# matthieugomez/LeastSquaresOptim.jl

Measured on AMD Instinct MI355X. Metric: lm_lsmr_outer_iterations_per_sec, higher is better.
Workload: dtype f64

## Files before the change

include/lsqhip.h:

```cpp
#ifndef LSQHIP_H
#define LSQHIP_H
#include <stddef.h>
#ifdef __cplusplus
extern "C" {
#endif

typedef enum {
    LSQ_OK = 0,
    LSQ_EDIM = 1,
    LSQ_ENOTPD = 2,
    LSQ_ERANK = 3,
    LSQ_ENONFINITE = 4,
    LSQ_EBOUNDS = 5,
    LSQ_EHIP = 6,
    LSQ_EARG = 7,
    LSQ_ECALLBACK = 8,
    LSQ_ERCCL = 9
} lsq_status;

typedef struct lsq_ctx lsq_ctx;
typedef struct lsq_mat lsq_mat;
typedef struct lsq_solver lsq_solver;
typedef struct lsq_model lsq_model;

// ... 16 lines not shown
int lsq_host_free(lsq_ctx *ctx, void *h_ptr);

int lsq_dense_create(lsq_ctx *ctx, int m, int n, lsq_mat **out);
int lsq_csc_create(lsq_ctx *ctx, int m, int n, const int *h_colptr, const int *h_rowval, lsq_mat **out);
int lsq_blockdiag_create(lsq_ctx *ctx, int nblocks, int mb, int nb, lsq_mat **out);
int lsq_mat_blockdiag_info(const lsq_mat *J, int *nblocks, int *mb, int *nb);
int lsq_blockdiag_bordered_create(lsq_ctx *ctx, int nblocks, int mb, int nb, int ng, lsq_mat **out);
int lsq_mat_bordered_info(const lsq_mat *J, int *nblocks, int *mb, int *nb, int *ng);
int lsq_mat_destroy(lsq_mat *J);
int lsq_mat_size(const lsq_mat *J, int *m, int *n, long long *nnz);
int lsq_mat_set_values(lsq_mat *J, const double *h_values);
int lsq_mat_get_values(const lsq_mat *J, double *h_values);
int lsq_mat_set_values_async(lsq_mat *J, const double *h_pinned_values);
int lsq_mat_upload_wait(lsq_mat *J);
double *lsq_mat_values(lsq_mat *J);
int lsq_mat_refresh(lsq_mat *J);

int lsq_mat_set_colscale(lsq_mat *J, const double *d_s);
int lsq_mat_colscale_changed(lsq_mat *J);

typedef int (*lsq_op_mul_callback)(int trans, const double *d_x, double *d_out, void *user);
typedef int (*lsq_op_colsum_callback)(double *d_out, void *user);
int lsq_op_create(lsq_ctx *ctx, int m, int n, lsq_op_mul_callback mul, lsq_op_colsum_callback colsumabs2,
                  void *user, lsq_mat **out);

int lsq_mul(lsq_mat *J, int trans, double alpha, const double *d_x, double beta, double *d_y);
int lsq_colsumabs2(lsq_mat *J, double *d_out);
int lsq_rowsumabs2(lsq_mat *J, double *d_out);

int lsq_axpy(lsq_ctx *ctx, int n, double a, const double *d_x, double *d_y);
int lsq_scal(lsq_ctx *ctx, int n, double a, double *d_x);
int lsq_copy(lsq_ctx *ctx, int n, const double *d_x, double *d_y);
int lsq_fill(lsq_ctx *ctx, int n, double a, double *d_x);
int lsq_sumsq(lsq_ctx *ctx, int n, const double *d_x, double *h_out);
int lsq_sum(lsq_ctx *ctx, int n, const double *d_x, double *h_out);
int lsq_dot(lsq_ctx *ctx, int n, const double *d_x, const double *d_y, double *h_out);
int lsq_emul(lsq_ctx *ctx, int n, const double *d_x, const double *d_y, double *d_out);
int lsq_nrm2(lsq_ctx *ctx, int n, const double *d_x, double *h_out);
int lsq_wdot(lsq_ctx *ctx, int n, const double *d_x, const double *d_y, const double *d_w,
             double *h_out);
int lsq_amax(lsq_ctx *ctx, int n, const double *d_x, double *h_out);
int lsq_amax_projected(lsq_ctx *ctx, int n, const double *d_g, const double *d_x,
                       const double *d_lower, const double *d_upper, double *h_out);
int lsq_clamp(lsq_ctx *ctx, int n, double lo, double hi, double *d_x);
int lsq_ediv(lsq_ctx *ctx, int n, const double *d_x, const double *d_y, double *d_out);
int lsq_box_clip(lsq_ctx *ctx, int n, double *d_dx, const double *d_x, const double *d_lower,
                 const double *d_upper);
int lsq_first_nonfinite(lsq_ctx *ctx, int n, const double *d_x, int *h_index);

int lsq_solver_create(lsq_ctx *ctx, lsq_mat *J, int solver_kind, int for_lm, lsq_solver **out);
int lsq_solver_destroy(lsq_solver *s);
int lsq_ldiv(lsq_solver *s, lsq_mat *J, const double *d_y, double *d_x, int *nmul);
int lsq_ldiv_damped(lsq_solver *s, lsq_mat *J, const double *d_y, double *d_damp, double *d_x,
                    int *nmul);
typedef int (*lsq_precond_callback)(double *d_P, lsq_mat *J, const double *d_damp, void *user);
int lsq_solver_set_preconditioner(lsq_solver *s, lsq_precond_callback cb, void *user);
typedef int (*lsq_precond_update_callback)(lsq_mat *J, const double *d_damp, void *user);
typedef int (*lsq_precond_ldiv_callback)(double *d_out, const double *d_in, void *user);
int lsq_solver_set_general_preconditioner(lsq_solver *s, lsq_precond_update_callback update, lsq_precond_ldiv_callback ldiv,
                                          void *user);
typedef int (*lsq_device_allreduce_callback)(double *d_buf, int count, void *hip_stream, void *user);

int lsq_solver_set_row_allreduce(lsq_solver *s, lsq_device_allreduce_callback cb, void *user, long long global_rows);
int lsq_solver_info(const lsq_solver *s, int *lsmr_iter, int *lsmr_istop, int *qr_rank);
int lsq_solver_qr_path(const lsq_solver *s, int *path);
int lsq_solver_qr_panel(const lsq_solver *s, int *kind);
int lsq_solver_chol_path(const lsq_solver *s, int *path);
int lsq_solver_lsmr_path(const lsq_solver *s, int *path);
int lsq_solver_blockdiag_path(const lsq_solver *s, int *path, int *block);
int lsq_solver_blockdiag_ranks(const lsq_solver *s, int *h_ranks);
int lsq_solver_covariance(lsq_solver *s, lsq_mat *J, const double *d_f, double *d_cov, double *d_stderr, int *h_info);
int lsq_dense_covariance(lsq_solver *s, lsq_mat *J, const double *d_f, double *d_cov, double *d_stderr, int *h_info);
int lsq_dense_qr_covariance(lsq_solver *s, lsq_mat *J, const double *d_f, double *d_cov, double *d_stderr, int *h_info);

int lsq_solver_stats(const lsq_solver *s, int h_giveups[4], int h_paused[4]);
int lsq_ctx_fallback_stats(const lsq_ctx *ctx, int h_giveups[4]);
int lsq_ctx_device_info(const lsq_ctx *ctx, int *num_cus, int *num_xcds, char *arch_name, int name_cap);

int lsq_ctx_tail_stats(const lsq_ctx *ctx, long long h_out[2]);
int lsq_ctx_commit_step_stats(const lsq_ctx *ctx, long long h_out[2]);

typedef int (*lsq_f_callback)(double *d_out, const double *d_x, void *user);
typedef int (*lsq_g_callback)(lsq_mat *J, const double *d_x, void *user);
typedef int (*lsq_allreduce_callback)(double *h_vals, int count, void *user);

typedef struct {
    double x_tol, f_tol, g_tol;
    int iterations;
    double delta;
    const double *h_lower;
    const double *h_upper;
    lsq_allreduce_callback allreduce;
    void *allreduce_user;
    int trace_cap;
    double *trace_ssr, *trace_gnorm, *trace_delta, *trace_rho;
    int *trace_inner, *trace_accept;
    double *trace_x;
    lsq_precond_callback preconditioner;
    void *preconditioner_user;
    lsq_device_allreduce_callback row_allreduce;
    void *row_allreduce_user;
    long long global_rows;
    lsq_precond_update_callback precond_update;
    lsq_precond_ldiv_callback precond_ldiv;
    void *precond_general_user;
} lsq_options;

typedef struct {
    int optimizer;
    double ssr;
    int iterations;
    int converged, x_converged, f_converged, g_converged;
    int f_calls, g_calls, mul_calls;
    int status;
    int bad_index;
    double seconds;
    long long lsmr_iterations;
    double ssr0;
} lsq_result;

void lsq_options_default(lsq_options *opt);
int lsq_optimize(lsq_ctx *ctx, int optimizer, int solver_kind, lsq_mat *J, double *d_x,
                 double *d_fcur, lsq_f_callback f, lsq_g_callback g, void *user,
                 const lsq_options *opt, lsq_result *res);
int lsq_fd_jacobian(lsq_ctx *ctx, lsq_mat *J, const double *d_x, lsq_f_callback f, void *user);

int lsq_csc_greedy_colouring(int m, int n, const int *h_colptr, const int *h_rowval, int *h_colour, int *h_ncolours);
int lsq_mat_set_fd_colouring(lsq_mat *J, const int *h_colour_or_null, int *h_ncolours);
int lsq_mat_fd_colouring(const lsq_mat *J, int *h_colour, int *h_ncolours);

typedef struct {
    double *ssr, *ssr0;
    int *iterations;
    int *converged, *x_converged, *f_converged, *g_converged;
    int *f_calls, *g_calls, *mul_calls;
    int *status, *info;
    int outer_iterations;
    double seconds;
    int trace_cap;
    double *trace_ssr, *trace_gnorm, *trace_delta, *trace_rho;
    int *trace_accept;
    double *trace_x;
} lsq_batched_result;
int lsq_optimize_batched(lsq_ctx *ctx, int optimizer, int solver_kind, lsq_mat *J, double *d_x,
                         double *d_fcur, lsq_f_callback f, lsq_g_callback g, void *user,
                         const lsq_options *opt, void *batched_result);

int lsq_model_tanh_create(lsq_ctx *ctx, lsq_mat *J, const double *h_Avalues, const double *h_b,
                          lsq_model **out);
int lsq_model_destroy(lsq_model *md);
lsq_f_callback lsq_model_f(void);
lsq_g_callback lsq_model_g(void);
int lsq_model_paths(const lsq_model *md, int *sliced_rows, int *sliced_cols, int *lsmr_path, long long *pair_tails);

int lsq_synth_sparse(int m, int n, int per_col, unsigned long long seed, int *h_colptr,
                     int *h_rowval, double *h_nzval);
int lsq_synth_dense(int m, int n, unsigned long long seed, double *h_values);
int lsq_synth_uniform(int n, unsigned long long seed, double lo, double hi, double *h_out);
int lsq_synth_normal(int n, unsigned long long seed, double *h_out);

int lsq_bench_mul(lsq_mat *J, int trans, int reps, const double *d_x, double *d_y, double beta,
                  float *h_ms_per_launch);

int lsq_bench_occupy(lsq_ctx *ctx, int workgroups, int lds_bytes, double milliseconds);
int lsq_bench_occupy_wait(lsq_ctx *ctx);

int lsq_set_exact(int on);

int lsq_debug_set(int launch_jitter_us, int serial);
int lsq_debug_get(int *launch_jitter_us, int *serial, long long *stalls);

int lsq_prof_begin(lsq_ctx *ctx, int max_samples);
int lsq_prof_select(lsq_ctx *ctx, int kernel_mask);
int lsq_prof_end(lsq_ctx *ctx, double h_avg_ms[2], int h_count[2]);
int lsq_prof_overhead(lsq_ctx *ctx, int pairs, double *h_ms);

#ifdef __cplusplus
}
#endif
#endif
```

leastsquaresoptim.jl_amd/_lib.py:

```python
import ctypes as C
import os
import re
import subprocess

_HERE = os.path.dirname(os.path.abspath(__file__))
ROOT = os.path.dirname(_HERE)
LIB_PATH = os.environ.get("LSQ_LIB_PATH") or os.path.join(_HERE, "liblsqhip.so")
HEADER = os.path.join(ROOT, "include", "lsqhip.h")

c_dp = C.POINTER(C.c_double)
c_ip = C.POINTER(C.c_int)

F_CALLBACK = C.CFUNCTYPE(C.c_int, C.c_void_p, C.c_void_p, C.c_void_p)
G_CALLBACK = C.CFUNCTYPE(C.c_int, C.c_void_p, C.c_void_p, C.c_void_p)
ALLREDUCE_CALLBACK = C.CFUNCTYPE(C.c_int, c_dp, C.c_int, C.c_void_p)
OP_MUL_CALLBACK = C.CFUNCTYPE(C.c_int, C.c_int, C.c_void_p, C.c_void_p, C.c_void_p)
OP_COLSUM_CALLBACK = C.CFUNCTYPE(C.c_int, C.c_void_p, C.c_void_p)
PRECOND_CALLBACK = C.CFUNCTYPE(C.c_int, C.c_void_p, C.c_void_p, C.c_void_p, C.c_void_p)
ROW_ALLREDUCE_CALLBACK = C.CFUNCTYPE(C.c_int, C.c_void_p, C.c_int, C.c_void_p, C.c_void_p)
PRECOND_UPDATE_CALLBACK = C.CFUNCTYPE(C.c_int, C.c_void_p, C.c_void_p, C.c_void_p)
PRECOND_LDIV_CALLBACK = C.CFUNCTYPE(C.c_int, C.c_void_p, C.c_void_p, C.c_void_p)

OK, EDIM, ENOTPD, ERANK, ENONFINITE, EBOUNDS, EHIP, EARG, ECALLBACK, ERCCL = range(10)
QR, CHOLESKY, LSMR, BLOCK_QR = 0, 1, 2, 3
DOGLEG, LEVENBERG_MARQUARDT = 0, 1


class Options(C.Structure):
    _fields_ = [("x_tol", C.c_double), ("f_tol", C.c_double), ("g_tol", C.c_double),
                ("iterations", C.c_int), ("delta", C.c_double), ("h_lower", c_dp), ("h_upper", c_dp),
                ("allreduce", ALLREDUCE_CALLBACK), ("allreduce_user", C.c_void_p),
                ("trace_cap", C.c_int), ("trace_ssr", c_dp), ("trace_gnorm", c_dp),
                ("trace_delta", c_dp), ("trace_rho", c_dp), ("trace_inner", c_ip),
                ("trace_accept", c_ip), ("trace_x", c_dp),
                ("preconditioner", PRECOND_CALLBACK), ("preconditioner_user", C.c_void_p),
                ("row_allreduce", ROW_ALLREDUCE_CALLBACK), ("row_allreduce_user", C.c_void_p),
                ("global_rows", C.c_longlong),
                ("precond_update", PRECOND_UPDATE_CALLBACK), ("precond_ldiv", PRECOND_LDIV_CALLBACK),
                ("precond_general_user", C.c_void_p)]


class Result(C.Structure):
    _fields_ = [("optimizer", C.c_int), ("ssr", C.c_double), ("iterations", C.c_int),
                ("converged", C.c_int), ("x_converged", C.c_int), ("f_converged", C.c_int),
                ("g_converged", C.c_int), ("f_calls", C.c_int), ("g_calls", C.c_int),
                ("mul_calls", C.c_int), ("status", C.c_int), ("bad_index", C.c_int),
                ("seconds", C.c_double), ("lsmr_iterations", C.c_longlong), ("ssr0", C.c_double)]


class BatchedResult(C.Structure):
    _fields_ = [("ssr", c_dp), ("ssr0", c_dp), ("iterations", c_ip),
                ("converged", c_ip), ("x_converged", c_ip), ("f_converged", c_ip), ("g_converged", c_ip),
                ("f_calls", c_ip), ("g_calls", c_ip), ("mul_calls", c_ip), ("status", c_ip), ("info", c_ip),
                ("outer_iterations", C.c_int), ("seconds", C.c_double), ("trace_cap", C.c_int),
                ("trace_ssr", c_dp), ("trace_gnorm", c_dp), ("trace_delta", c_dp), ("trace_rho", c_dp),
                ("trace_accept", c_ip), ("trace_x", c_dp)]


def build(verbose=False):
    cmd = ["make", "-C", os.path.join(_HERE, "csrc"), "-j8"]
    if not verbose:
        cmd.insert(1, "-s")
    subprocess.check_call(cmd)
    return LIB_PATH


def declared_symbols():
    txt = open(HEADER).read()
    txt = re.sub(r"/\*.*?\*/", "", txt, flags=re.S)
    names = re.findall(r"\b(lsq_[a-z0-9_]+)\s*\(", txt)
    skip = {"lsq_f_callback", "lsq_g_callback", "lsq_allreduce_callback", "lsq_device_allreduce_callback",
            "lsq_precond_update_callback", "lsq_precond_ldiv_callback"}
    return sorted(set(n for n in names if n not in skip))


_LIB = None


def lib():
    global _LIB
    if _LIB is not None:
        return _LIB
    if not os.path.exists(LIB_PATH):
        raise RuntimeError(
            "liblsqhip.so is not built (%s). Run __graft_entry__.build() or `make -C "
            "leastsquaresoptim.jl_amd/csrc`. There is no CPU fallback." % LIB_PATH)
    L = C.CDLL(LIB_PATH)
    vp, i, d, sz = C.c_void_p, C.c_int, C.c_double, C.c_size_t
    pvp = C.POINTER(C.c_void_p)
    sig = {
        "lsq_last_error": (C.c_char_p, []),
        "lsq_version": (i, []),
        "lsq_ctx_create": (i, [i, vp, pvp]),
        "lsq_ctx_destroy": (i, [vp]),
        "lsq_ctx_sync": (i, [vp]),
        "lsq_ctx_stream": (vp, [vp]),
        "lsq_malloc": (i, [vp, sz, pvp]),
        "lsq_free": (i, [vp, vp]),
        "lsq_h2d": (i, [vp, vp, vp, sz]),
        "lsq_d2h": (i, [vp, vp, vp, sz]),
        "lsq_d2d": (i, [vp, vp, vp, sz]),
        "lsq_dense_create": (i, [vp, i, i, pvp]),
        "lsq_csc_create": (i, [vp, i, i, c_ip, c_ip, pvp]),
        "lsq_blockdiag_create": (i, [vp, i, i, i, pvp]),
        "lsq_mat_blockdiag_info": (i, [vp, c_ip, c_ip, c_ip]),
        "lsq_blockdiag_bordered_create": (i, [vp, i, i, i, i, pvp]),
        "lsq_mat_bordered_info": (i, [vp, c_ip, c_ip, c_ip, c_ip]),
        "lsq_mat_destroy": (i, [vp]),
        "lsq_mat_size": (i, [vp, c_ip, c_ip, C.POINTER(C.c_longlong)]),
        "lsq_mat_set_values": (i, [vp, c_dp]),
        "lsq_mat_get_values": (i, [vp, c_dp]),
        "lsq_mat_set_values_async": (i, [vp, c_dp]),
        "lsq_mat_upload_wait": (i, [vp]),
        "lsq_host_alloc": (i, [vp, sz, pvp]),
        "lsq_host_free": (i, [vp, vp]),
        "lsq_dot": (i, [vp, i, vp, vp, c_dp]),
        "lsq_emul": (i, [vp, i, vp, vp, vp]),
        "lsq_mat_values": (vp, [vp]),
        "lsq_mat_refresh": (i, [vp]),
        "lsq_mat_set_colscale": (i, [vp, vp]),
        "lsq_mat_colscale_changed": (i, [vp]),
        "lsq_mul": (i, [vp, i, d, vp, d, vp]),
        "lsq_solver_set_preconditioner": (i, [vp, PRECOND_CALLBACK, vp]),
        "lsq_solver_set_general_preconditioner": (i, [vp, PRECOND_UPDATE_CALLBACK, PRECOND_LDIV_CALLBACK, vp]),
        "lsq_op_create": (i, [vp, i, i, OP_MUL_CALLBACK, OP_COLSUM_CALLBACK, vp, C.POINTER(vp)]),
        "lsq_colsumabs2": (i, [vp, vp]),
        "lsq_rowsumabs2": (i, [vp, vp]),
        "lsq_axpy": (i, [vp, i, d, vp, vp]),
        "lsq_scal": (i, [vp, i, d, vp]),
        "lsq_copy": (i, [vp, i, vp, vp]),
        "lsq_fill": (i, [vp, i, d, vp]),
        "lsq_sumsq": (i, [vp, i, vp, c_dp]),
        "lsq_sum": (i, [vp, i, vp, c_dp]),
        "lsq_nrm2": (i, [vp, i, vp, c_dp]),
        "lsq_wdot": (i, [vp, i, vp, vp, vp, c_dp]),
        "lsq_amax": (i, [vp, i, vp, c_dp]),
        "lsq_amax_projected": (i, [vp, i, vp, vp, vp, vp, c_dp]),
        "lsq_clamp": (i, [vp, i, d, d, vp]),
        "lsq_ediv": (i, [vp, i, vp, vp, vp]),
        "lsq_box_clip": (i, [vp, i, vp, vp, vp, vp]),
        "lsq_first_nonfinite": (i, [vp, i, vp, c_ip]),
        "lsq_solver_create": (i, [vp, vp, i, i, pvp]),
        "lsq_solver_destroy": (i, [vp]),
        "lsq_ldiv": (i, [vp, vp, vp, vp, c_ip]),
        "lsq_ldiv_damped": (i, [vp, vp, vp, vp, vp, c_ip]),
        "lsq_solver_set_row_allreduce": (i, [vp, ROW_ALLREDUCE_CALLBACK, vp, C.c_longlong]),
        "lsq_solver_info": (i, [vp, c_ip, c_ip, c_ip]),
        "lsq_solver_qr_path": (i, [vp, c_ip]),
        "lsq_solver_qr_panel": (i, [vp, c_ip]),
        "lsq_solver_chol_path": (i, [vp, c_ip]),
        "lsq_solver_lsmr_path": (i, [vp, c_ip]),
        "lsq_solver_blockdiag_path": (i, [vp, c_ip, c_ip]),
        "lsq_solver_blockdiag_ranks": (i, [vp, c_ip]),
        "lsq_solver_covariance": (i, [vp, vp, vp, vp, vp, c_ip]),
        "lsq_dense_covariance": (i, [vp, vp, vp, vp, vp, c_ip]),
        "lsq_dense_qr_covariance": (i, [vp, vp, vp, vp, vp, c_ip]),
        "lsq_solver_stats": (i, [vp, c_ip, c_ip]),
        "lsq_ctx_fallback_stats": (i, [vp, c_ip]),
        "lsq_ctx_device_info": (i, [vp, c_ip, c_ip, C.c_char_p, i]),
        "lsq_ctx_tail_stats": (i, [vp, C.POINTER(C.c_longlong)]),
        "lsq_ctx_commit_step_stats": (i, [vp, C.POINTER(C.c_longlong)]),
        "lsq_bench_occupy": (i, [vp, i, i, d]),
        "lsq_bench_occupy_wait": (i, [vp]),
        "lsq_options_default": (None, [C.POINTER(Options)]),
        "lsq_optimize": (i, [vp, i, i, vp, vp, vp, F_CALLBACK, G_CALLBACK, vp, C.POINTER(Options),
                             C.POINTER(Result)]),
        "lsq_optimize_batched": (i, [vp, i, i, vp, vp, vp, F_CALLBACK, G_CALLBACK, vp, C.POINTER(Options),
                                     C.POINTER(BatchedResult)]),
        "lsq_fd_jacobian": (i, [vp, vp, vp, F_CALLBACK, vp]),
        "lsq_csc_greedy_colouring": (i, [i, i, c_ip, c_ip, c_ip, c_ip]),
        "lsq_mat_set_fd_colouring": (i, [vp, c_ip, c_ip]),
        "lsq_mat_fd_colouring": (i, [vp, c_ip, c_ip]),
        "lsq_model_tanh_create": (i, [vp, vp, c_dp, c_dp, pvp]),
        "lsq_model_destroy": (i, [vp]),
        "lsq_model_f": (F_CALLBACK, []),
        "lsq_model_g": (G_CALLBACK, []),
        "lsq_model_paths": (i, [vp, c_ip, c_ip, c_ip, C.POINTER(C.c_longlong)]),
        "lsq_synth_sparse": (i, [i, i, i, C.c_ulonglong, c_ip, c_ip, c_dp]),
        "lsq_synth_dense": (i, [i, i, C.c_ulonglong, c_dp]),
        "lsq_synth_uniform": (i, [i, C.c_ulonglong, d, d, c_dp]),
        "lsq_synth_normal": (i, [i, C.c_ulonglong, c_dp]),
        "lsq_set_exact": (i, [i]),
        "lsq_debug_set": (i, [i, i]),
        "lsq_debug_get": (i, [c_ip, c_ip, C.POINTER(C.c_longlong)]),
        "lsq_prof_begin": (i, [vp, i]),
        "lsq_prof_select": (i, [vp, i]),
        "lsq_prof_end": (i, [vp, c_dp, c_ip]),
        "lsq_prof_overhead": (i, [vp, i, c_dp]),
        "lsq_bench_mul": (i, [vp, i, i, vp, vp, d, C.POINTER(C.c_float)]),
    }
    for name, (res, args) in sig.items():
        fn = getattr(L, name)
        fn.restype = res
        fn.argtypes = args
    L._signatures = sig
    _LIB = L
    return L


class LsqError(RuntimeError):

    def __init__(self, status, msg):
        super().__init__(msg)
        self.status = status


class DimensionMismatch(LsqError):
    pass


class PosDefException(LsqError):
    pass


class RankDeficientException(LsqError):
    pass


class IsFiniteException(LsqError):
    pass


class ArgumentError(LsqError):
    pass


class HipError(LsqError):
    pass


class PeerAborted(LsqError):
    """Sharded run: another rank left its loop with an error (LSQ_ERCCL)."""


_EXC = {EDIM: DimensionMismatch, ENOTPD: PosDefException, ERANK: RankDeficientException,
        ENONFINITE: IsFiniteException, EBOUNDS: ArgumentError, EHIP: HipError, EARG: ArgumentError,
        ECALLBACK: LsqError, ERCCL: PeerAborted}


def check(status):
    if status != OK:
        msg = lib().lsq_last_error().decode("utf-8", "replace")
        raise _EXC.get(status, LsqError)(status, msg or "lsq status %d" % status)
```

leastsquaresoptim.jl_amd/csrc/lsq_common.h:

```cpp
#pragma once
#include <hip/hip_runtime.h>
#include <atomic>

#include <cstdarg>
#include <cstdint>
#include <cstdio>
#include <unordered_map>
#include <vector>

#include "../../include/lsqhip.h"

void lsq_set_error(const char *fmt, ...);

#define LSQ_HIP(call)                                                                      \
    do {                                                                                   \
        hipError_t e__ = (call);                                                           \
        if (e__ != hipSuccess) {                                                           \
            lsq_set_error("%s failed: %s (%s:%d)", #call, hipGetErrorString(e__), __FILE__, \
                          __LINE__);                                                       \
            return LSQ_EHIP;                                                               \
        }                                                                                  \
    } while (0)

#define LSQ_TRY(call)                 \
// ... 169 lines not shown
    bool csc_fresh = true;
    bool upload_pending = false;
    const double *d_colscale = nullptr;
    const double *d_cs_user = nullptr;
    double *d_cs_base = nullptr;
    double *d_colsum_base = nullptr;
    unsigned long long base_version = 0;
    unsigned long long colsum_base_version = ~0ull;
    LsqSegs bcsc;
    int nwin = 0;
    int *d_bmap = nullptr;
    double *d_bpart = nullptr;
    double *d_dpart = nullptr;
    size_t dpart_cap = 0;
    LsqSell srows, scols;
    int (*op_mul)(int, const double *, double *, void *) = nullptr;
    int (*op_colsum)(double *, void *) = nullptr;
    void *op_user = nullptr;
    double *d_optmp = nullptr;
    unsigned long long version = 0;
    unsigned long long uid = lsq_next_mat_uid();
    double *d_colsum = nullptr;
    unsigned long long colsum_version = ~0ull;
    int bd_blocks = 0, bd_mb = 0, bd_nb = 0;
    int br_blocks = 0, br_mb = 0, br_nb = 0, br_ng = 0;
    double *d_fd = nullptr;
    struct LsqFdColouring *fdc = nullptr;
};

struct LsqFdColouring {
    int ncolours = 0;
    std::vector<int> colour;
    std::vector<int> bound;
    std::vector<int> ebound;
    int *d_colour = nullptr;
    int *d_cols = nullptr;
    int *d_off = nullptr;
};
void lsq_fd_colouring_free(lsq_mat *J);

#define LSQ_ZERO(ptr, val, bytes)                  \
    do {                                           \
        LSQ_HIP(hipMemset((ptr), (val), (bytes))); \
        LSQ_HIP(hipStreamSynchronize(nullptr));    \
    } while (0)

#define RLX_AGENT __ATOMIC_RELAXED, __HIP_MEMORY_SCOPE_AGENT

template <int CTRL>
__device__ __forceinline__ double lsq_dpp_mov_f64(double x) {
    int lo = __double2loint(x), hi = __double2hiint(x);
    lo = __builtin_amdgcn_update_dpp(0, lo, CTRL, 0xf, 0xf, false);
    hi = __builtin_amdgcn_update_dpp(0, hi, CTRL, 0xf, 0xf, false);
    return __hiloint2double(hi, lo);
}
__device__ __forceinline__ double lsq_readlane_f64(double x, int l) {
    return __hiloint2double(__builtin_amdgcn_readlane(__double2hiint(x), l), __builtin_amdgcn_readlane(__double2loint(x), l));
}
__device__ __forceinline__ double wave_sum(double v) {
    v += lsq_dpp_mov_f64<0x128>(v);
    v += lsq_dpp_mov_f64<0x124>(v);
    v += lsq_dpp_mov_f64<0x122>(v);
    v += lsq_dpp_mov_f64<0x121>(v);
    return (lsq_readlane_f64(v, 0) + lsq_readlane_f64(v, 16)) + (lsq_readlane_f64(v, 32) + lsq_readlane_f64(v, 48));
}
__device__ __forceinline__ double wave_max(double v) {
    v = fmax(v, lsq_dpp_mov_f64<0x128>(v));
    v = fmax(v, lsq_dpp_mov_f64<0x124>(v));
    v = fmax(v, lsq_dpp_mov_f64<0x122>(v));
    v = fmax(v, lsq_dpp_mov_f64<0x121>(v));
    return fmax(fmax(lsq_readlane_f64(v, 0), lsq_readlane_f64(v, 16)), fmax(lsq_readlane_f64(v, 32), lsq_readlane_f64(v, 48)));
}

__device__ __forceinline__ int lsq_xcd_block(int b, int G) {
    const int q = G >> 3, r = G & 7, x = b & 7;
    return x * q + (x < r ? x : r) + (b >> 3);
}

template <int NT>
__device__ __forceinline__ double block_sum(double v, double *sh ) {
    v = wave_sum(v);
    const int lane = threadIdx.x & 63, w = threadIdx.x >> 6;
    if (lane == 0) sh[w] = v;
    __syncthreads();
    double r = 0.0;
    if (threadIdx.x == 0) {
#pragma unroll
        for (int i = 0; i < NT / 64; ++i) r += sh[i];
    }
    __syncthreads();
    return r;
}
template <int NT>
__device__ __forceinline__ double block_max(double v, double *sh) {
    v = wave_max(v);
    const int lane = threadIdx.x & 63, w = threadIdx.x >> 6;
    if (lane == 0) sh[w] = v;
    __syncthreads();
    double r = 0.0;
    if (threadIdx.x == 0) {
        r = sh[0];
#pragma unroll
        for (int i = 1; i < NT / 64; ++i) r = fmax(r, sh[i]);
    }
    __syncthreads();
    return r;
}

constexpr int LSQ_RGROUPS = 8;
constexpr int LSQ_RFLAT = 64;
constexpr int LSQ_CTR_STRIDE = 32;
constexpr int LSQ_CTR_SLOT = (LSQ_RGROUPS + 1) * LSQ_CTR_STRIDE;
template <int NT, bool IS_MAX = false, class Fin>
__device__ __forceinline__ bool grid_reduce(double block_val, double *partials, unsigned *counter,
                                            int nblocks, double *sh, Fin fin) {
    __shared__ int s_last;
    const int b = blockIdx.x;
    if (threadIdx.x == 0) {
        __hip_atomic_store(&partials[b], block_val, RLX_AGENT);
        asm volatile("s_waitcnt vmcnt(0)" ::: "memory");
        const int g = b % LSQ_RGROUPS;
        const int ngroups = nblocks < LSQ_RGROUPS ? nblocks : LSQ_RGROUPS;
        const unsigned gsize = (unsigned)((nblocks - g + LSQ_RGROUPS - 1) / LSQ_RGROUPS);
        int last = 0;
        if (nblocks <= LSQ_RFLAT) {
            if (__hip_atomic_fetch_add(counter, 1u, RLX_AGENT) == (unsigned)(nblocks - 1)) {
                __hip_atomic_store(counter, 0u, RLX_AGENT);
                last = 1;
            }
        } else if (__hip_atomic_fetch_add(counter + (1 + g) * LSQ_CTR_STRIDE, 1u, RLX_AGENT) == gsize - 1) {
            __hip_atomic_store(counter + (1 + g) * LSQ_CTR_STRIDE, 0u, RLX_AGENT);
            unsigned t2 = __hip_atomic_fetch_add(counter, 1u, RLX_AGENT);
            if (t2 == (unsigned)(ngroups - 1)) {
                __hip_atomic_store(counter, 0u, RLX_AGENT);
                last = 1;
            }
        }
        s_last = last;
    }
    __syncthreads();
    if (!s_last) return false;
    if (threadIdx.x == 0) __builtin_amdgcn_fence(__ATOMIC_ACQUIRE, "agent");
    __syncthreads();
    double acc = 0.0;
    for (int i = threadIdx.x; i < nblocks; i += NT) {
        double p = __hip_atomic_load(&partials[i], RLX_AGENT);
        acc = IS_MAX ? fmax(acc, p) : acc + p;
    }
    double tot = IS_MAX ? block_max<NT>(acc, sh) : block_sum<NT>(acc, sh);
    if (threadIdx.x == 0) fin(tot);
    return true;
}

struct LsqSlotPublish {
    const double *src = nullptr;
    int count = 0;
    double *dst = nullptr;
    unsigned long long *seq_word = nullptr;
    unsigned long long seq = 0;
};
LsqSlotPublish lsq_slots_ticket(lsq_ctx *c, int first, int count);
int lsq_wait_slots(lsq_ctx *c, int first, int count, unsigned long long seq, double *h_out);
int lsq_first_nonfinite_to_slot(lsq_ctx *c, int n, const double *x, double *d_slot);
int lsq_read_ints(lsq_ctx *c, const int *d_a, const int *d_b, const int *d_c, const int *d_d, int h_out[4]);
LsqSlotPublish lsq_ints_ticket(lsq_ctx *c);
int lsq_wait_ints(lsq_ctx *c, unsigned long long seq, const int *d_a, const int *d_b, const int *d_c, const int *d_d, int h_out[4]);

static inline void lsq_run_idle_hook(lsq_ctx *c) {
    if (!c->idle_hook) return;
    int (*h)(void *) = c->idle_hook;
    c->idle_hook = nullptr;
    c->idle_status = h(c->idle_user);
}

static inline unsigned *lsq_ctr(const lsq_ctx *c, int k) { return c->d_counters + (size_t)k * LSQ_CTR_SLOT; }
static inline int lsq_div_up(long long a, long long b) { return (int)((a + b - 1) / b); }

constexpr int LSQ_EXACT_MAX_DIM = 2048;
constexpr long long LSQ_EXACT_MAX_NNZ = 1 << 18;
bool lsq_small_vec(long long n);
bool lsq_small_mat(const lsq_mat *J);
int lsq_exact_product(lsq_mat *J, int trans, const double *x, double *y);
int lsq_exact_colsumabs2(lsq_mat *J, double *out);
int lsq_exact_mul(lsq_mat *J, int trans, double alpha, const double *x, double beta, double *y);
int lsq_seq_reduce(lsq_ctx *c, int mode, int n, const double *x, const double *y, const double *w, double *d_out);
int lsq_exact_lm_damp(lsq_ctx *c, int n, const double *colsum, double inv_delta, double *dtd);

void lsq_workspace_free(void *workspace);

int lsq_sparse_mul(lsq_mat *J, int trans, double alpha, const double *d_x, double beta, double *d_y);
int lsq_dense_mul(lsq_mat *J, int trans, double alpha, const double *d_x, double beta, double *d_y);
static inline int lsq_dense_t_windows(const lsq_ctx *c, int m, int n) {
    if (n <= 0 || n >= c->num_cus || m < 8192) return 0;
    int nwin = (4 * c->num_cus + n - 1) / n;
    nwin = std::min(nwin, std::max(1, m / 2048));
    return nwin > 1 ? nwin : 0;
}
int lsq_dense_colsumabs2(lsq_mat *J, double *d_out);
int lsq_dense_part(lsq_mat *J, int nwin);
int lsq_dense_part_elems(lsq_mat *J, size_t need);
int lsq_sparse_colsumabs2(lsq_mat *J, double *d_out);
int lsq_ensure_csr(lsq_mat *J);
int lsq_ensure_csc(lsq_mat *J);
int lsq_mirror_rows(lsq_mat *J, const double *d_csc_vals, double *d_out);
int lsq_mirror_cols(lsq_mat *J, const double *d_csc_vals, double *d_out);
long long lsq_mirror_rows_len(const lsq_mat *J);
long long lsq_mirror_cols_len(const lsq_mat *J);
bool lsq_can_fuse_grad_colsum(const lsq_mat *J);
bool lsq_colscale_fusable(const lsq_mat *J);
int lsq_sparse_grad_colsum(lsq_mat *J, const double *f, double *g);
int lsq_sparse_grad_colsum_spec(lsq_mat *J, const double *f, double *g, const double *s_new, const int *gate);
void lsq_sparse_grad_colsum_adopt(lsq_mat *J);
void lsq_sparse_colsum_forget(lsq_mat *J);
const double *lsq_cached_colsum(lsq_mat *J);
struct LsqFdCall {
    lsq_f_callback f;
    void *user;
    int status;
};
int lsq_fd_check(const lsq_mat *J, const char *who);
int lsq_fd_values(lsq_mat *J, const double *x, lsq_f_callback f, void *user);
int lsq_fd_f_thunk(double *d_out, const double *d_x, void *user);
int lsq_fd_g_thunk(lsq_mat *J, const double *d_x, void *user);
int lsq_read_slots(lsq_ctx *ctx, int first, int count, double *h_out);
```

leastsquaresoptim.jl_amd/csrc/lsq_loop.h:

```cpp
#pragma once
#include "lsq_solver.h"

static constexpr double MIN_DELTA = 1e-16, MAX_DELTA = 1e16, MIN_STEP_QUALITY = 1e-3;
static constexpr double MIN_DIAGONAL = 1e-6, MAX_DIAGONAL = 1e32;
static constexpr double DECREASE_THRESHOLD = 0.25, INCREASE_THRESHOLD = 0.75;

enum { SL_GRAD = 8, SL_DX = 9, SL_NONFIN = 10, SL_TRIAL = 11, SL_PRED = 12, SL_SSR = 13, SL_W0 = 14, SL_W1 = 15,
       SL_W2 = 16, SL_SUM = 17 };

static inline int ngrid(const lsq_ctx *c, long long n) {
    long long g = (n + LSQ_NT - 1) / LSQ_NT;
    long long cap = (long long)c->num_cus * 8;
    if (g > cap) g = cap;
    return g < 1 ? 1 : (int)g;
}

bool model_is_builtin(lsq_f_callback f, lsq_g_callback g = nullptr);

int model_f_sumsq(void *user, double *out, const double *x, int ctr, double *d_out, LsqSlotPublish pub, bool *done,
                  const int *skip = nullptr, bool mirror = false);
int model_start_point(void *user, const double *x, double *d_nonfin, bool *done);
void model_forget_point(void *user);
struct SpecGrad {
    int *gate;
    double ssr;
    double *grad;
    bool launched;
    double xtol, ftol, gtol;
};
int model_pair_tail(void *user, lsq_mat *J, const double *dx, const double *fcur, double *ftrial, const double *xt,
                    double *slot_pred, double *slot_trial, LsqSlotPublish pub, const int *skip, bool *done,
                    SpecGrad *sg = nullptr);
void model_trial_buffers(void *user, const double *xt, double **t_out, double **s_out);

int lsq_workspace_lsmr_path(const lsq_ctx *c, const lsq_mat *J);
```

leastsquaresoptim.jl_amd/csrc/lsq_lsmr3.h:

```cpp
#pragma once

constexpr int LSQ_FUSED_UB_MAX = 4;
struct LsmrHandoff {
    unsigned long long w[8];
};
__device__ __forceinline__ void lsmr_handoff_write(LsmrHandoff *ho, unsigned tag, double vs, double cu, int done) {
    const unsigned long long t = (unsigned long long)tag << 32;
    const unsigned long long bv = (unsigned long long)__double_as_longlong(vs), bc = (unsigned long long)__double_as_longlong(cu);
    __hip_atomic_store(&ho->w[0], t | (bv & 0xffffffffull), __ATOMIC_RELAXED, __HIP_MEMORY_SCOPE_AGENT);
    __hip_atomic_store(&ho->w[1], t | (bv >> 32), __ATOMIC_RELAXED, __HIP_MEMORY_SCOPE_AGENT);
    __hip_atomic_store(&ho->w[2], t | (bc & 0xffffffffull), __ATOMIC_RELAXED, __HIP_MEMORY_SCOPE_AGENT);
    __hip_atomic_store(&ho->w[3], t | (bc >> 32), __ATOMIC_RELAXED, __HIP_MEMORY_SCOPE_AGENT);
    __hip_atomic_store(&ho->w[4], t | (unsigned)done, __ATOMIC_RELAXED, __HIP_MEMORY_SCOPE_AGENT);
}
__device__ __forceinline__ void lsmr_handoff_fail(LsmrHandoff *ho, unsigned tag) {
    __hip_atomic_store(&ho->w[6], (unsigned long long)tag, __ATOMIC_RELAXED, __HIP_MEMORY_SCOPE_AGENT);
}
struct LsmrHandoffWords { unsigned long long w[5]; };
__device__ __forceinline__ LsmrHandoffWords lsmr_handoff_request(const LsmrHandoff *ho) {
    LsmrHandoffWords r;
#pragma unroll
    for (int k = 0; k < 5; ++k) r.w[k] = __hip_atomic_load(&ho->w[k], __ATOMIC_RELAXED, __HIP_MEMORY_SCOPE_AGENT);
    return r;
}
// ... 34 lines not shown
    const double test2 = s.normAr / (s.normA * s.normr);
    const double test3 = 1.0 / s.condA;
    const double t1 = test1 / (1.0 + s.normA * s.normx / s.normb);
    const double rtol = s.btol + s.atol * s.normA * s.normx / s.normb;
    int istop = 0;
    if (s.iter >= s.maxiter) istop = 7;
    else if (1.0 + test3 <= 1.0) istop = 6;
    else if (1.0 + test2 <= 1.0) istop = 5;
    else if (1.0 + t1 <= 1.0) istop = 4;
    else if (test3 <= s.ctol) istop = 3;
    else if (test2 <= s.atol) istop = 2;
    else if (test1 <= rtol) istop = 1;
    s.istop = istop;
    if (istop) { s.done = 1; s.notdone = 0; }
}

constexpr long long LSQ_FUSED_SPIN_LIMIT = 1LL << 24;

__device__ __forceinline__ void publish_relaxed(LsqMailbox *mail, const LsmrState *st) {
    unsigned long long w = ((unsigned long long)(st->epoch & 0x7fffffu) << 41) |
                           ((unsigned long long)(st->done ? 1 : 0) << 40) |
                           ((unsigned long long)(st->istop & 0xff) << 32) | (unsigned)st->iter;
    __hip_atomic_store((unsigned long long *)mail, w, __ATOMIC_RELAXED, __HIP_MEMORY_SCOPE_SYSTEM);
}

__device__ __forceinline__ void ordered_sum512x3(const double *pa, const int *na, const double *pb, const int *nb,
                                                 const double *pc, const int *nc, double &ra, double &rb, double &rc) {
    __shared__ double s_w5[3][4];
    __shared__ double s_tot5[3];
    const int tid = threadIdx.x;
    if (tid < 256) {
        const double a0 = pa ? pa[tid] : 0.0, b0 = pb ? pb[tid] : 0.0, c0 = pc ? pc[tid] : 0.0;
        const double a1 = pa ? pa[tid + 256] : 0.0, b1 = pb ? pb[tid + 256] : 0.0, c1 = pc ? pc[tid + 256] : 0.0;
        const int ca = pa ? *na : 0, cb = pb ? *nb : 0, cc = pc ? *nc : 0;
        double a = tid < ca ? a0 : 0.0, b = tid < cb ? b0 : 0.0, c = tid < cc ? c0 : 0.0;
        if (tid + 256 < ca) a += a1;
        if (tid + 256 < cb) b += b1;
        if (tid + 256 < cc) c += c1;
        for (int i = tid + 512; i < ca; i += 256) a += pa[i];
        for (int i = tid + 512; i < cb; i += 256) b += pb[i];
        for (int i = tid + 512; i < cc; i += 256) c += pc[i];
        a = wave_sum(a);
        b = wave_sum(b);
        c = wave_sum(c);
        if ((tid & 63) == 0) {
            s_w5[0][tid >> 6] = a;
            s_w5[1][tid >> 6] = b;
            s_w5[2][tid >> 6] = c;
        }
    }
    __syncthreads();
    if (tid < 3) s_tot5[tid] = ((s_w5[tid][0] + s_w5[tid][1]) + s_w5[tid][2]) + s_w5[tid][3];
    __syncthreads();
    ra = s_tot5[0];
    rb = s_tot5[1];
    rc = s_tot5[2];
    __syncthreads();
}

__device__ __forceinline__ void lsq_lds_barrier() { asm volatile("s_waitcnt lgkmcnt(0)\n\ts_barrier" ::: "memory"); }
template <bool IS_MAX>
__device__ __forceinline__ double lsq_block_reduce_lds(double v, double *sh ) {
    v = IS_MAX ? wave_max(v) : wave_sum(v);
    const int lane = threadIdx.x & 63, w = threadIdx.x >> 6;
    if (lane == 0) sh[w] = v;
    lsq_lds_barrier();
    double r = 0.0;
    if (threadIdx.x == 0) {
        r = sh[0];
#pragma unroll
        for (int i = 1; i < LSQ_BIG_NT / 64; ++i) r = IS_MAX ? fmax(r, sh[i]) : r + sh[i];
    }
    lsq_lds_barrier();
    return r;
}

template <bool STEP, int NU>
__device__ __forceinline__ void lsmr_update_groups(const LsmrFused &a, const LsmrStepDesc &sd, const int gstride, double *sh,
                                                   LsmrState &ns) {
    const int tid = threadIdx.x;
    const int n = a.n;
    static_assert(sizeof(LsmrState) % 8 == 0 && sizeof(LsmrState) / 8 <= LSQ_BIG_NT, "state copy: one 8-byte word per thread");
    constexpr int NQ = (LSQ_LDS_X_MAX + LSQ_BIG_NT - 1) / LSQ_BIG_NT;
    double xi[NQ], hbi[NQ], hi[NQ];
#pragma unroll
    for (int q = 0; q < NQ; ++q) {
        const int j = min(tid + q * LSQ_BIG_NT, n - 1);
        xi[q] = a.x_in[j];
        hbi[q] = a.hbar_in[j];
        hi[q] = a.h_in[j];
    }
    if (tid < (int)(sizeof(LsmrState) / 8)) ((unsigned long long *)&ns)[tid] = ((const unsigned long long *)a.st_in)[tid];
    const bool prev_failed = a.tag_prev != 0u &&
                             (unsigned)__hip_atomic_load(&a.ho->w[6], __ATOMIC_RELAXED, __HIP_MEMORY_SCOPE_AGENT) == a.tag_prev;
    double beta2, betax2, alpha2;
    ordered_sum512x3(a.pu_in, a.npu_in, a.px_in, a.npx_in, a.pv, a.npv, beta2, betax2, alpha2);
    if (ns.done) {
        if (blockIdx.x == 0) {
            if (tid < (int)(sizeof(LsmrState) / 8)) ((unsigned long long *)a.st_out)[tid] = ((const unsigned long long *)&ns)[tid];
            if (tid == 0) {
                lsmr_handoff_write(a.ho, a.tag, 1.0, 0.0, 1);
                publish_relaxed(a.mail, &ns);
            }
        }
        return;
    }
    const bool was_first = ns.first != 0;
    if (tid == 0) lsmr_scalars(ns, beta2, betax2, alpha2, a.dg != nullptr, a.px_in != nullptr);
    __syncthreads();
    if (!was_first) {
        const double c1 = ns.c1, c2 = ns.c2;
        double acc = 0.0;
#pragma unroll
        for (int q = 0; q < NQ; ++q) {
            const double hb = hbi[q] * c1 + hi[q];
            const double xj = xi[q] + c2 * hb;
            acc += (tid + q * LSQ_BIG_NT < n) ? xj * xj : 0.0;
        }
        const double total = block_sum<LSQ_BIG_NT>(acc, sh);
        if (tid == 0) lsmr_decide(ns, total);
    } else if (tid == 0) {
        ns.first = 0;
        if (!(ns.normAr != 0.0)) { ns.done = 1; ns.notdone = 0; }
    }
    if (tid == 0 && prev_failed) { ns.istop = 99; ns.done = 1; ns.notdone = 0; }
    __syncthreads();
    const bool done_now = ns.done != 0;
    const double vs = ns.vscale, cu = ns.cu, c1 = ns.c1, c2 = ns.c2, c3 = ns.c3;
    if constexpr (STEP) {
        if (!done_now) {
            if (blockIdx.x == 0 && tid == 0) {
                if (!was_first) {
                    __hip_atomic_store((double *)&a.mail->test1, ns.normr / ns.normb, __ATOMIC_RELAXED, __HIP_MEMORY_SCOPE_SYSTEM);
                    __hip_atomic_store((double *)&a.mail->test2, ns.normAr / (ns.normA * ns.normr), __ATOMIC_RELAXED, __HIP_MEMORY_SCOPE_SYSTEM);
                }
                publish_relaxed(a.mail, &ns);
            }
            return;
        }
    }
    if (blockIdx.x == 0) {
        if (tid == 0 && !a.test_no_record) lsmr_handoff_write(a.ho, a.tag, vs, cu, done_now ? 1 : 0);
        if (tid < (int)(sizeof(LsmrState) / 8)) ((unsigned long long *)a.st_out)[tid] = ((const unsigned long long *)&ns)[tid];
        if (tid == 0) {
            if (!was_first) {
                __hip_atomic_store((double *)&a.mail->test1, ns.normr / ns.normb, __ATOMIC_RELAXED, __HIP_MEMORY_SCOPE_SYSTEM);
                __hip_atomic_store((double *)&a.mail->test2, ns.normAr / (ns.normA * ns.normr), __ATOMIC_RELAXED, __HIP_MEMORY_SCOPE_SYSTEM);
            }
            publish_relaxed(a.mail, &ns);
        }
    }
    double e_vt[NU], e_P[NU], e_dg[NU], e_ux[NU], e_h[NU], e_hb[NU], e_x[NU];
    double e_s[NU];
#pragma unroll
    for (int k = 0; k < NU; ++k) {
        const int j = min((int)(blockIdx.x + k * gstride) * LSQ_BIG_NT + tid, n - 1);
        e_vt[k] = a.vt[j];
        e_P[k] = a.P ? a.P[j] : 1.0;
        e_dg[k] = a.dg ? a.dg[j] : 0.0;
        e_ux[k] = a.dg ? a.ux[j] : 0.0;
        e_h[k] = a.h_in[j];
        e_hb[k] = a.hbar_in[j];
        e_x[k] = a.x_in[j];
        if constexpr (STEP) e_s[k] = sd.x[j];
    }
    double aux = 0.0;
    double mx = 0.0, code = 0.0;
#pragma unroll
    for (int k = 0; k < NU; ++k) {
        const int j = (int)(blockIdx.x + k * gstride) * LSQ_BIG_NT + tid;
        if (j >= n) continue;
        const double Pj = e_P[k];
        const double vj = e_vt[k] * vs;
        a.v[j] = vj;
        double dj = 0.0;
        if (was_first) {
            a.h_out[j] = vj;
            a.hbar_out[j] = 0.0;
            a.x_out[j] = 0.0;
            a.xout[j] = 0.0;
        } else {
            const double hj = e_h[k];
            const double hb = e_hb[k] * c1 + hj;
            a.hbar_out[j] = hb;
            const double xj = e_x[k] + c2 * hb;
            a.x_out[j] = xj;
            a.h_out[j] = hj * c3 + vj;
            dj = a.P ? xj * Pj : xj;
            a.xout[j] = dj;
        }
        if constexpr (STEP) {
            const double v = e_s[k] + -1.0 * dj;
            sd.xt[j] = v;
            if (sd.t_out) {
                const double th = tanh(v);
                sd.t_out[j] = th;
                sd.s_out[j] = 1.0 - th * th;
            }
            double ad = fabs(dj);
            if (isnan(ad)) ad = INFINITY;
            mx = fmax(mx, ad);
            if (!isfinite(v) && code == 0.0) code = 1e15 - (double)(j + 1);
        }
        if (a.dg && !done_now) {
            const double tj = a.P ? vj * Pj : vj;
            const double un = tj * e_dg[k] - cu * e_ux[k];
            a.ux[j] = un;
            aux += un * un;
        }
    }
    if constexpr (STEP) {
        const double b2 = lsq_block_reduce_lds<true>(code, sh);
        if (tid == 0) __hip_atomic_store(&sd.partials[LSQ_MAX_GRID + blockIdx.x], b2, RLX_AGENT);
        const double b1 = lsq_block_reduce_lds<true>(mx, sh);
        const int nb = gridDim.x;
        double *const out_dx = sd.out_dx;
        if (grid_reduce<LSQ_BIG_NT, true>(b1, sd.partials, sd.counter, nb, sh, [=](double t) { *out_dx = t; })) {
            double acc = 0.0;
            for (int i = tid; i < nb; i += LSQ_BIG_NT) acc = fmax(acc, __hip_atomic_load(&sd.partials[LSQ_MAX_GRID + i], RLX_AGENT));
            const double t = block_max<LSQ_BIG_NT>(acc, sh);
            if (tid == 0) *sd.out_nonfin = (t == 0.0) ? -1.0 : (1e15 - t) - 1.0;
        }
        return;
    }
    if (done_now) return;
    const double bux = lsq_block_reduce_lds<false>(aux, sh);
    if (tid == 0) {
        a.px_out[blockIdx.x] = bux;
        if (blockIdx.x == 0) *a.npx_out = gstride;
    }
}

template <int = 0>
__global__ void __launch_bounds__(LSQ_BIG_NT) k_lsmr_fused(SellDev S, int wrows, int m, int nxpad, LsmrFused a) {
    extern __shared__ __attribute__((aligned(16))) double smem[];
    __shared__ double sh[LSQ_BIG_NT / 64];
    __shared__ LsmrState ns;
    __shared__ double s_vs, s_cu;
    __shared__ int s_done;
    double *xl = smem;
    double *yw = smem + nxpad;
    const int tid = threadIdx.x, lane = tid & 63, wv = tid >> 6;
    const int n = a.n;
    const bool upd = (int)blockIdx.x < a.ub;

    if (upd) {
        constexpr int NQ = (LSQ_LDS_X_MAX + LSQ_BIG_NT - 1) / LSQ_BIG_NT;
        lsmr_update_groups<false, (NQ + 2) / 3>(a, LsmrStepDesc{}, a.ub, sh, ns);
        return;
    }

    constexpr int XR = (LSQ_LDS_X_MAX + LSQ_BIG_NT - 1) / LSQ_BIG_NT;
    {
        double xr[XR];
#pragma unroll
        for (int q = 0; q < XR; ++q) xr[q] = a.w[min(tid + q * LSQ_BIG_NT, n - 1)];
        const int dflag = a.st_in->done;
#pragma unroll
        for (int q = 0; q < XR; ++q)
            if (tid + q * LSQ_BIG_NT < n) xl[tid + q * LSQ_BIG_NT] = xr[q];
        if (dflag) return;
    }
    constexpr int Q = LSQ_SELL_ROWS_MAX / LSQ_BIG_NT;
    const int pb = (int)blockIdx.x - a.ub, npb = (int)gridDim.x - a.ub;
    double racc = 0.0;
    bool have_scalars = false;
    if (a.cautious) {
        if (tid == 0) {
            LsmrHandoffWords rec = lsmr_handoff_request(a.ho);
            long long spins = 0;
            while (!lsmr_handoff_valid(rec, a.tag)) {
                if (++spins > (a.test_no_record ? 4096 : LSQ_FUSED_SPIN_LIMIT)) break;
                __builtin_amdgcn_s_sleep(8);
                rec = lsmr_handoff_request(a.ho);
            }
            const bool ok = spins <= (a.test_no_record ? 4096 : LSQ_FUSED_SPIN_LIMIT);
            s_vs = __longlong_as_double((long long)((rec.w[0] & 0xffffffffull) | (rec.w[1] << 32)));
            s_cu = __longlong_as_double((long long)((rec.w[2] & 0xffffffffull) | (rec.w[3] << 32)));
            s_done = ok ? (int)(rec.w[4] & 0xffffffffull) : 2;
            if (!ok) lsmr_handoff_fail(a.ho, a.tag);
        }
        __syncthreads();
        if (s_done) return;
        have_scalars = true;
    }
    for (int w = pb; w < S.nblocks; w += npb) {
        const int base = w * wrows, rows = min(wrows, m - base);
        const int s0 = w * S.spw, s1 = s0 + S.spw;
        double pre[Q];
#pragma unroll
        for (int q = 0; q < Q; ++q) pre[q] = a.uold[base + min(tid + q * LSQ_BIG_NT, rows - 1)];
        LsmrHandoffWords rec;
#pragma unroll
        for (int k = 0; k < 5; ++k) rec.w[k] = 0ull;
        {
            constexpr int NW = LSQ_BIG_NT / 64;
            int sidx = s0 + wv;
            SellSliceRef A = sell_slice_ref(S, sidx, s1, lane);
            __syncthreads();
            unsigned long long poll = 0ull;
            for (; sidx < s1; sidx += NW) {
                if (!have_scalars && (unsigned)(poll >> 32) == a.tag && (poll & 1ull)) break;
                if (!have_scalars) poll = __hip_atomic_load(&a.ho->w[4], __ATOMIC_RELAXED, __HIP_MEMORY_SCOPE_AGENT);
                const SellSliceRef r = A;
                A = sell_slice_ref(S, sidx + NW, s1, lane);
                if (!have_scalars && tid == 0 && sidx + NW >= s1) rec = lsmr_handoff_request(a.ho);
                const size_t oa = (size_t)r.sm.x + lane * 2;
                const unsigned pos = r.inf & LSQ_SELL_POS_MASK;
                double sum = 0.0, sq = 0.0;
                sell_lane_sum<false>(S.val + oa, S.idx16 + oa, r.sm.y, (int)(r.inf >> LSQ_SELL_POS_BITS), xl, sum, sq, lane);
                if (pos != LSQ_SELL_POS_MASK) yw[pos] = sum;
            }
        }
        if (!have_scalars && tid == 0) {
            long long spins = 0;
            while (!lsmr_handoff_valid(rec, a.tag)) {
                if (++spins > (a.test_no_record ? 4096 : LSQ_FUSED_SPIN_LIMIT)) break;
                __builtin_amdgcn_s_sleep(8);
                rec = lsmr_handoff_request(a.ho);
            }
            const bool ok = spins <= (a.test_no_record ? 4096 : LSQ_FUSED_SPIN_LIMIT);
            s_vs = __longlong_as_double((long long)((rec.w[0] & 0xffffffffull) | (rec.w[1] << 32)));
            s_cu = __longlong_as_double((long long)((rec.w[2] & 0xffffffffull) | (rec.w[3] << 32)));
            s_done = ok ? (int)(rec.w[4] & 0xffffffffull) : 2;
            if (!ok) lsmr_handoff_fail(a.ho, a.tag);
        }
        have_scalars = true;
        __syncthreads();
        if (s_done) return;
        const double vs = s_vs, cu = s_cu;
#pragma unroll
        for (int q = 0; q < Q; ++q) {
            const int i = tid + q * LSQ_BIG_NT;
            if (i < rows) {
                const double un = vs * yw[i] - cu * pre[q];
                a.unew[base + i] = un;
                racc += un * un;
            }
        }
    }
    const double bv = block_sum<LSQ_BIG_NT>(racc, sh);
    if (tid == 0) {
        a.pu_out[pb] = bv;
        if (pb == 0) *a.npu_out = npb;
    }
}

template <int = 0>
__global__ void __launch_bounds__(LSQ_BIG_NT) k_lsmr_commit_step(LsmrFused a, LsmrStepDesc sd) {
    __shared__ double sh[LSQ_BIG_NT / 64];
// ... 4 lines not shown
```

leastsquaresoptim.jl_amd/csrc/lsq_model.hip:

```cpp
#include <algorithm>

#include "lsq_loop.h"
#include "lsq_spmv.h"

struct lsq_model {
    lsq_ctx *ctx;
    lsq_mat *J;
    bool fused = false;
    double *d_Acsc = nullptr;
    double *d_Acsr = nullptr;
    double *d_Ab = nullptr;
    double *d_b = nullptr;
    double *d_t = nullptr;
    double *d_s = nullptr;
    double *d_sspec = nullptr;
    const double *tanh_x = nullptr;
    const double *sfac_x = nullptr;
    double *d_b_perm = nullptr;
    double *d_perm[2] = {nullptr, nullptr};
    const double *perm_of[2] = {nullptr, nullptr};
    long long pair_tails = 0;
};
static void model_perm_invalidate(lsq_model *md, const double *vec) {
    for (int k = 0; k < 2; ++k)
        if (!vec || md->perm_of[k] == vec) md->perm_of[k] = nullptr;
}

__global__ void __launch_bounds__(LSQ_NT) k_tanh(int n, const double *__restrict__ x, double *__restrict__ t) {
    for (int i = blockIdx.x * LSQ_NT + threadIdx.x; i < n; i += gridDim.x * LSQ_NT) t[i] = tanh(x[i]);
}

struct EpiResidual {
    static constexpr bool REDUCE = false;
    const int *done;
    int extra_blocks;
    const double *b;
    double *out;
    double *partials;
    unsigned *counter;
    __device__ void seg(int i, double dot, double &) const { out[i] = dot - b[i]; }
    using has_pre = void;
    __device__ double pre(int i) const { return b[i]; }
    __device__ void seg_pre(int i, double dot, double bi, double &) const { out[i] = dot - bi; }
    __device__ void extra(int, double &) const {}
    __device__ void finalize(double) const {}
};

struct EpiResidualSq {
    static constexpr bool REDUCE = true;
    const int *done;
    int extra_blocks;
    const double *b;
    double *out;
    double *partials;
    unsigned *counter;
    double *slot;
    LsqSlotPublish pub;
    __device__ void seg(int i, double dot, double &racc) const { seg_pre(i, dot, b[i], racc); }
    using has_pre = void;
    __device__ double pre(int i) const { return b[i]; }
    __device__ void seg_pre(int i, double dot, double bi, double &racc) const {
        const double v = dot - bi;
        out[i] = v;
        racc += v * v;
    }
    __device__ void extra(int, double &) const {}
    __device__ void finalize(double t) const {
        *slot = t;
        if (pub.count > 0) {
            for (int i = 0; i < pub.count; ++i)
                __hip_atomic_store(pub.dst + i, pub.src + i == slot ? t : pub.src[i], __ATOMIC_RELAXED, __HIP_MEMORY_SCOPE_SYSTEM);
            __hip_atomic_store(pub.seq_word, pub.seq, __ATOMIC_RELEASE, __HIP_MEMORY_SCOPE_SYSTEM);
        }
    }
};

struct EpiResidualSqPerm : EpiResidualSq {
    const double *b_perm;
    double *out_perm;
    using has_slice_out = void;
    __device__ double slice_pre(size_t pidx) const { return b_perm[pidx]; }
    __device__ void slice_post(size_t pidx, double dot, double bi) const { out_perm[pidx] = dot - bi; }
};

__global__ void __launch_bounds__(LSQ_NT)
k_scale_cols(int n, const int *__restrict__ colptr, int m_dense, const double *__restrict__ A,
             const double *__restrict__ x, double *__restrict__ out) {
    for (int j = blockIdx.x; j < n; j += gridDim.x) {
        double t = tanh(x[j]);
        double s = 1.0 - t * t;
        long long k0 = colptr ? colptr[j] : (long long)j * m_dense;
        long long k1 = colptr ? colptr[j + 1] : (long long)(j + 1) * m_dense;
        for (long long k = k0 + threadIdx.x; k < k1; k += LSQ_NT) out[k] = A[k] * s;
    }
}
__global__ void __launch_bounds__(LSQ_NT)
k_scale_dense(int m, const double *__restrict__ A, const double *__restrict__ x, double *__restrict__ out) {
    const int j = blockIdx.x;
    const double t = tanh(x[j]);
    const double sfac = 1.0 - t * t;
    const size_t base = (size_t)j * m;
    for (int i = blockIdx.y * LSQ_NT + threadIdx.x; i < m; i += gridDim.y * LSQ_NT) out[base + i] = A[base + i] * sfac;
}
__global__ void __launch_bounds__(LSQ_NT)
k_scale_csr(long long nnz, const int *__restrict__ colidx, const double *__restrict__ A, const double *__restrict__ sfac,
            double *__restrict__ out) {
    for (long long k = blockIdx.x * (long long)LSQ_NT + threadIdx.x; k < nnz; k += (long long)gridDim.x * LSQ_NT)
        out[k] = A[k] * sfac[colidx[k]];
}
__global__ void __launch_bounds__(LSQ_NT) k_tanh_sfac(int n, const double *__restrict__ x, double *__restrict__ t,
                                                      double *__restrict__ s, double *partials, unsigned *counter,
                                                      double *out_nonfin) {
    __shared__ double sh[LSQ_NT / 64];
    double code = 0.0;
    for (int i = blockIdx.x * LSQ_NT + threadIdx.x; i < n; i += gridDim.x * LSQ_NT) {
        const double xi = x[i];
        const double v = tanh(xi);
        t[i] = v;
        s[i] = 1.0 - v * v;
        if (!isfinite(xi) && code == 0.0) code = 1e15 - (double)(i + 1);
    }
    const double bv = block_max<LSQ_NT>(code, sh);
    grid_reduce<LSQ_NT, true>(bv, partials, counter, gridDim.x, sh, [=](double m) {
        *out_nonfin = (m == 0.0) ? -1.0 : (1e15 - m) - 1.0;
    });
}
__global__ void __launch_bounds__(LSQ_NT) k_sfac(int n, const double *__restrict__ x, double *__restrict__ s) {
    for (int i = blockIdx.x * LSQ_NT + threadIdx.x; i < n; i += gridDim.x * LSQ_NT) {
        double t = tanh(x[i]);
        s[i] = 1.0 - t * t;
    }
}

__global__ void __launch_bounds__(LSQ_NT)
k_scale_bcsc(int nseg, int n, const int *__restrict__ ptr, const double *__restrict__ A, const double *__restrict__ sfac,
             double *__restrict__ out) {
    const int lane = threadIdx.x & 63, per = LSQ_NT / 64;
    for (int s = blockIdx.x * per + (threadIdx.x >> 6); s < nseg; s += gridDim.x * per) {
        const double f = sfac[s % n];
        const int k1 = ptr[s + 1];
        for (int k = ptr[s] + lane; k < k1; k += 64) out[k] = A[k] * f;
    }
}

typedef double lsq_d2 __attribute__((ext_vector_type(2)));
template <bool NT>
__global__ void __launch_bounds__(1024)
k_scale_lds(long long nnz4, const unsigned short *__restrict__ col16, const double *__restrict__ A,
            const double *__restrict__ sfac, int n, double *__restrict__ out) {
    extern __shared__ double sf[];
    for (int i = threadIdx.x; i < n; i += 1024) sf[i] = sfac[i];
    __syncthreads();
    for (long long q = blockIdx.x * 1024LL + threadIdx.x; q < nnz4; q += (long long)gridDim.x * 1024) {
        const long long k = 4 * q;
        const lsq_d2 a0 = *reinterpret_cast<const lsq_d2 *>(A + k);
        const lsq_d2 a1 = *reinterpret_cast<const lsq_d2 *>(A + k + 2);
        const uint2 c = *reinterpret_cast<const uint2 *>(col16 + k);
        lsq_d2 o0, o1;
        o0.x = a0.x * sf[c.x & 0xffffu];
        o0.y = a0.y * sf[c.x >> 16];
        o1.x = a1.x * sf[c.y & 0xffffu];
        o1.y = a1.y * sf[c.y >> 16];
        if constexpr (NT) {
            __builtin_nontemporal_store(o0, reinterpret_cast<lsq_d2 *>(out + k));
            __builtin_nontemporal_store(o1, reinterpret_cast<lsq_d2 *>(out + k + 2));
        } else {
            *reinterpret_cast<lsq_d2 *>(out + k) = o0;
            *reinterpret_cast<lsq_d2 *>(out + k + 2) = o1;
        }
    }
}

__global__ void __launch_bounds__(LSQ_NT)
k_scale_bcsc_thread(int nseg, int n, const int *__restrict__ ptr, const double *__restrict__ A,
                    const double *__restrict__ sfac, double *__restrict__ out) {
    for (int s = blockIdx.x * LSQ_NT + threadIdx.x; s < nseg; s += gridDim.x * LSQ_NT) {
        const double f = sfac[s % n];
        const int k1 = ptr[s + 1];
        for (int k = ptr[s]; k < k1; ++k) out[k] = A[k] * f;
    }
}

static int model_f(double *out, const double *x, void *user) {
    lsq_model *md = (lsq_model *)user;
    lsq_ctx *c = md->ctx;
    lsq_mat *J = md->J;
    const bool have_tanh = md->tanh_x == x;
    md->tanh_x = nullptr;
    model_perm_invalidate(md, out);
    if (!have_tanh) {
        md->sfac_x = nullptr;
        LSQ_LAUNCH(k_tanh, dim3(ngrid(c, J->n)), dim3(LSQ_NT), 0, c->stream, J->n, x, md->d_t);
    }
    EpiResidual e{nullptr, 0, md->d_b, out, nullptr, nullptr};
    if (J->kind == LSQ_MAT_CSC && J->srows.active) {
        if (launch_sell_rows(J, nullptr, md->d_t, e, md->fused ? nullptr : md->d_Acsr) != LSQ_OK) return 1;
    } else if (J->kind == LSQ_MAT_CSC) {
        LsqSegs A = J->csr;
        A.d_val = md->d_Acsr;
        if (launch_segs<false>(c, A, md->d_t, e) != LSQ_OK) return 1;
    } else {
        lsq_mat tmp = *J;
        tmp.d_dense = md->d_Acsc;
        if (launch_product(&tmp, 0, md->d_t, e) != LSQ_OK) return 1;
    }
    return hipGetLastError() == hipSuccess ? 0 : 1;
}

void model_trial_buffers(void *user, const double *xt, double **t_out, double **s_out) {
    lsq_model *md = (lsq_model *)user;
    md->tanh_x = md->sfac_x = nullptr;
    if ((md->J->kind == LSQ_MAT_CSC && md->J->srows.active) || md->J->kind == LSQ_MAT_DENSE) {
        *t_out = md->d_t;
        *s_out = md->d_sspec;
        md->tanh_x = md->sfac_x = xt;
    }
}

int model_start_point(void *user, const double *x, double *d_nonfin, bool *done) {
    lsq_model *md = (lsq_model *)user;
    lsq_ctx *c = md->ctx;
    lsq_mat *J = md->J;
    *done = false;
    md->tanh_x = md->sfac_x = nullptr;
    if (!(J->kind == LSQ_MAT_CSC && J->srows.active) || J->n <= 0) return 0;
    LSQ_LAUNCH(k_tanh_sfac, dim3(ngrid(c, J->n)), dim3(LSQ_NT), 0, c->stream, J->n, x, md->d_t, md->d_sspec, c->d_partials,
               lsq_ctr(c, 0), d_nonfin);
    if (hipGetLastError() != hipSuccess) return 1;
    md->tanh_x = md->sfac_x = x;
    *done = true;
    return 0;
}
void model_forget_point(void *user) {
    lsq_model *md = (lsq_model *)user;
    md->tanh_x = md->sfac_x = nullptr;
}

static bool model_pair_applies(const lsq_model *md, const lsq_mat *J) {
    return md->fused && J == md->J && J->kind == LSQ_MAT_CSC && J->srows.active && J->srows.ncw == 1 && J->d_colscale &&
           J->n <= LSQ_PAIR_X_MAX && !getenv("LSQ_NO_PAIR_TAIL");
}
static bool model_perm_ready(lsq_model *md) {
    if (md->d_b_perm) return true;
    lsq_ctx *c = md->ctx;
    const LsqSell &S = md->J->srows;
    const size_t plen = (size_t)S.nslices * 64;
    const int pgrid = std::max(1, std::min(lsq_div_up((long long)plen, LSQ_NT), c->num_cus * 8));
    double *pb = nullptr, *p0 = nullptr, *p1 = nullptr;
    if (hipMalloc(&pb, plen * sizeof(double)) != hipSuccess || hipMalloc(&p0, plen * sizeof(double)) != hipSuccess ||
        hipMalloc(&p1, plen * sizeof(double)) != hipSuccess) {
        (void)hipGetLastError();
        hipFree(pb); hipFree(p0); hipFree(p1);
        return false;
    }
    md->d_b_perm = pb; md->d_perm[0] = p0; md->d_perm[1] = p1;
    LSQ_LAUNCH(k_sell_perm_rows<0>, dim3(pgrid), dim3(LSQ_NT), 0, c->stream, sell_dev(S), S.wrows, S.nslices, (const double *)md->d_b,
               md->d_b_perm);
    return true;
}

int model_f_sumsq(void *user, double *out, const double *x, int ctr, double *d_out, LsqSlotPublish pub, bool *done,
                         const int *skip, bool mirror) {
    lsq_model *md = (lsq_model *)user;
    lsq_ctx *c = md->ctx;
    lsq_mat *J = md->J;
    *done = false;
    if (!(J->kind == LSQ_MAT_CSC && J->srows.active)) return model_f(out, x, user);
    model_perm_invalidate(md, out);
    EpiResidualSq e{skip, 0, md->d_b, out, c->d_partials, lsq_ctr(c, ctr), d_out, pub};
    const bool have_tanh = md->tanh_x == x;
    md->tanh_x = nullptr;
    if (!have_tanh) {
        md->sfac_x = nullptr;
        LSQ_LAUNCH(k_tanh, dim3(ngrid(c, J->n)), dim3(LSQ_NT), 0, c->stream, J->n, x, md->d_t);
    }
    if (mirror && !skip && model_pair_applies(md, J) && model_perm_ready(md)) {
        EpiResidualSqPerm ep;
        static_cast<EpiResidualSq &>(ep) = e;
        ep.b_perm = md->d_b_perm;
        ep.out_perm = md->d_perm[0];
        if (launch_sell_rows(J, nullptr, md->d_t, ep, nullptr) != LSQ_OK) return 1;
        md->perm_of[0] = out;
    } else if (launch_sell_rows(J, nullptr, md->d_t, e, md->fused ? nullptr : md->d_Acsr) != LSQ_OK) return 1;
    *done = true;
    return hipGetLastError() == hipSuccess ? 0 : 1;
}

int model_pair_tail(void *user, lsq_mat *J, const double *dx, const double *fcur, double *ftrial, const double *xt,
                           double *slot_pred, double *slot_trial, LsqSlotPublish pub, const int *skip, bool *done, SpecGrad *sg) {
    lsq_model *md = (lsq_model *)user;
    lsq_ctx *c = md->ctx;
    *done = false;
    if (!(model_pair_applies(md, J) && md->tanh_x == xt)) return 0;
    const LsqSell &S = J->srows;
    const int nxpad = (J->n + 1) & ~1;
    const size_t lds = (size_t)std::max(2 * nxpad, LSQ_SELL_ROWS_MAX) * sizeof(double);
    if (lsq_set_lds(c, (const void *)k_sell_rows_pair<0>, (size_t)2 * LSQ_PAIR_X_MAX * sizeof(double)) != LSQ_OK) return 0;
    const size_t plen = (size_t)S.nslices * 64;
    const int pgrid = std::max(1, std::min(lsq_div_up((long long)plen, LSQ_NT), c->num_cus * 8));
    if (!model_perm_ready(md)) return 0;
    int k = md->perm_of[0] == fcur ? 0 : (md->perm_of[1] == fcur ? 1 : -1);
    if (k < 0) {
        k = 0;
        LSQ_LAUNCH(k_sell_perm_rows<0>, dim3(pgrid), dim3(LSQ_NT), 0, c->stream, sell_dev(S), S.wrows, S.nslices, fcur, md->d_perm[k]);
        md->perm_of[k] = fcur;
    }
    md->perm_of[1 - k] = ftrial;
    md->tanh_x = nullptr;
    const int grid = std::max(1, std::min(S.nblocks, c->num_cus));
    const bool spec = sg && sg->gate && md->sfac_x == xt;
    SellPairEpi e{skip, md->d_perm[k], md->d_b_perm, ftrial, md->d_perm[1 - k], c->d_partials, c->d_partials + 4096, lsq_ctr(c, 7),
                  slot_pred, slot_trial, pub, spec ? sg->gate : nullptr, spec ? sg->ssr : 0.0, MIN_STEP_QUALITY,
                  c->d_slots + SL_SSR, c->d_slots + SL_DX, c->d_slots + SL_GRAD, spec ? sg->xtol : 0.0, spec ? sg->ftol : 0.0,
                  spec ? sg->gtol : 0.0};
    LSQ_LAUNCH(k_sell_rows_pair<0>, dim3(grid), dim3(LSQ_BIG_NT), lds, c->stream, sell_dev(S), S.wrows, J->m, dx, J->d_colscale,
               (const double *)md->d_t, J->n, nxpad, e);
    *done = true;
    ++md->pair_tails;
    if (hipGetLastError() != hipSuccess) return 1;
    if (spec) {
        const int st = lsq_sparse_grad_colsum_spec(J, ftrial, sg->grad, md->d_sspec, sg->gate);
        if (st == LSQ_OK) sg->launched = true;
        else if (st != LSQ_EARG) return 1;
    }
    return 0;
}

static int model_g(lsq_mat *J, const double *x, void *user) {
    lsq_model *md = (lsq_model *)user;
    lsq_ctx *c = md->ctx;
    if (J->kind == LSQ_MAT_DENSE) {}
    else if (md->sfac_x == x) std::swap(md->d_s, md->d_sspec);
    else LSQ_LAUNCH(k_sfac, dim3(ngrid(c, J->n)), dim3(LSQ_NT), 0, c->stream, J->n, x, md->d_s);
    md->sfac_x = nullptr;
    md->tanh_x = nullptr;
    if (md->fused) {
        if (lsq_mat_set_colscale(J, md->d_s) != LSQ_OK) return 1;
        return hipGetLastError() == hipSuccess ? 0 : 1;
    }
    if (J->kind == LSQ_MAT_CSC) {
        const bool have_cols = J->scols.active || J->nwin > 1;
        const unsigned short *rcol = J->srows.active ? J->srows.d_idx16 : J->csr.d_idx16;
        const unsigned short *ccol = J->scols.active ? J->scols.d_col16 : J->bcsc.d_col16;
        double *rval = J->srows.active ? J->srows.d_val : J->csr.d_val;
        double *cval = J->scols.active ? J->scols.d_val : J->bcsc.d_val;
        const long long rlen = lsq_mirror_rows_len(J), clen = lsq_mirror_cols_len(J);
        const bool lds_ok = J->n <= 12000 && J->nnz >= (1 << 20) && J->srows.ncw == 1;
        const bool lazy_csc = lds_ok && rcol && have_cols && ccol && lsq_can_fuse_grad_colsum(J);
        if (!lazy_csc) {
            int grid = J->n < c->num_cus * 16 ? (J->n > 0 ? J->n : 1) : c->num_cus * 16;
            LSQ_LAUNCH(k_scale_cols, dim3(grid), dim3(LSQ_NT), 0, c->stream, J->n, J->csc.d_ptr, 0, md->d_Acsc,
                               x, J->csc.d_val);
        }
        J->csc_fresh = !lazy_csc;
        const size_t lds = (size_t)J->n * sizeof(double);
        if (lds_ok) {
            LSQ_TRY(lsq_set_lds(c, (const void *)k_scale_lds<true>, 12000 * 8));
            LSQ_TRY(lsq_set_lds(c, (const void *)k_scale_lds<false>, 12000 * 8));
        }
        if (J->nnz > 0) {
            if (lds_ok && rcol) {
                LSQ_LAUNCH(k_scale_lds<true>, dim3(c->num_cus), dim3(1024), lds, c->stream, (rlen + 3) / 4, rcol,
                                   md->d_Acsr, md->d_s, J->n, rval);
            } else if (!J->srows.active) {
                long long g2 = std::min<long long>((J->nnz + LSQ_NT - 1) / LSQ_NT, (long long)c->num_cus * 16);
                LSQ_LAUNCH(k_scale_csr, dim3((int)g2), dim3(LSQ_NT), 0, c->stream, J->nnz, J->csr.d_idx,
                                   md->d_Acsr, md->d_s, J->csr.d_val);
            } else {
                if (lazy_csc) return 1;
                if (lsq_mirror_rows(J, J->csc.d_val, rval) != LSQ_OK) return 1;
            }
        }
        if (have_cols) {
            if (lds_ok && ccol) {
                LSQ_LAUNCH(k_scale_lds<false>, dim3(c->num_cus), dim3(1024), lds, c->stream, (clen + 3) / 4,
                                   ccol, md->d_Ab, md->d_s, J->n, cval);
            } else if (J->scols.active) {
                if (lazy_csc) return 1;
                if (lsq_mirror_cols(J, J->csc.d_val, cval) != LSQ_OK) return 1;
            } else if (J->nnz < 16LL * J->bcsc.nseg) {
                int nsegs = J->bcsc.nseg;
                int g3 = std::min(lsq_div_up(nsegs, LSQ_NT), c->num_cus * 16);
                LSQ_LAUNCH(k_scale_bcsc_thread, dim3(g3), dim3(LSQ_NT), 0, c->stream, nsegs, J->n,
                                   J->bcsc.d_ptr, md->d_Ab, md->d_s, J->bcsc.d_val);
            } else {
                int nsegs = J->bcsc.nseg;
                int g3 = std::min(lsq_div_up(nsegs, LSQ_NT / 64), c->num_cus * 16);
                LSQ_LAUNCH(k_scale_bcsc, dim3(g3), dim3(LSQ_NT), 0, c->stream, nsegs, J->n, J->bcsc.d_ptr,
                                   md->d_Ab, md->d_s, J->bcsc.d_val);
            }
        }
        J->csr_fresh = true;
    } else {
        const long long tot = (long long)J->m * J->n;
        const int chunks = std::max(1, (int)std::min<long long>((J->m + 4 * LSQ_NT - 1) / (4 * LSQ_NT),
                                                               std::max<long long>(1, (long long)c->num_cus * 16 / std::max(1, J->n))));
        if (tot > 0)
            LSQ_LAUNCH(k_scale_dense, dim3(J->n, chunks), dim3(LSQ_NT), 0, c->stream, J->m, md->d_Acsc, x, J->d_dense);
    }
    J->version++;
    return hipGetLastError() == hipSuccess ? 0 : 1;
}

bool model_is_builtin(lsq_f_callback f, lsq_g_callback g) { return f == model_f && (!g || g == model_g); }

extern "C" lsq_f_callback lsq_model_f(void) { return model_f; }
extern "C" lsq_g_callback lsq_model_g(void) { return model_g; }

extern "C" int lsq_model_tanh_create(lsq_ctx *c, lsq_mat *J, const double *hA, const double *hb, lsq_model **out) {
    if (!c || !J || !hA || !hb || !out) return LSQ_EARG;
    LSQ_HIP(hipSetDevice(c->device));
    lsq_model *md = new lsq_model();
    md->ctx = c;
    md->J = J;
    const size_t nb = (size_t)(J->n > 0 ? J->n : 1) * sizeof(double);
    LSQ_HIP(hipMalloc(&md->d_b, (size_t)(J->m > 0 ? J->m : 1) * sizeof(double)));
    LSQ_HIP(hipMemcpy(md->d_b, hb, (size_t)J->m * sizeof(double), hipMemcpyHostToDevice));
    LSQ_HIP(hipMalloc(&md->d_t, nb));
    LSQ_HIP(hipMalloc(&md->d_s, nb));
    LSQ_HIP(hipMalloc(&md->d_sspec, nb));
    if (lsq_colscale_fusable(J)) {
        LSQ_TRY(lsq_mat_set_values(J, hA));
        LSQ_TRY(lsq_fill(c, J->n, 1.0, md->d_s));
        LSQ_TRY(lsq_mat_set_colscale(J, md->d_s));
        md->fused = true;
        LSQ_HIP(hipStreamSynchronize(c->stream));
        *out = md;
        return LSQ_OK;
    }
    size_t vb = (size_t)(J->nnz + 8) * sizeof(double);
    LSQ_HIP(hipMalloc(&md->d_Acsc, vb));
    LSQ_ZERO(md->d_Acsc, 0, vb);
    LSQ_HIP(hipMemcpy(md->d_Acsc, hA, (size_t)J->nnz * sizeof(double), hipMemcpyHostToDevice));
    if (J->kind == LSQ_MAT_CSC) {
        const size_t rb = (size_t)(lsq_mirror_rows_len(J) + 1024) * sizeof(double);
        LSQ_HIP(hipMalloc(&md->d_Acsr, rb));
        LSQ_ZERO(md->d_Acsr, 0, rb);
        LSQ_TRY(lsq_mirror_rows(J, md->d_Acsc, md->d_Acsr));
        if (lsq_mirror_cols_len(J) > 0) {
            const size_t cbytes = (size_t)(lsq_mirror_cols_len(J) + 1024) * sizeof(double);
            LSQ_HIP(hipMalloc(&md->d_Ab, cbytes));
            LSQ_ZERO(md->d_Ab, 0, cbytes);
            LSQ_TRY(lsq_mirror_cols(J, md->d_Acsc, md->d_Ab));
        }
        LSQ_HIP(hipStreamSynchronize(c->stream));
    }
    *out = md;
    return LSQ_OK;
}

extern "C" int lsq_model_paths(const lsq_model *md, int *sliced_rows, int *sliced_cols, int *lsmr_path, long long *pair_tails) {
    if (!md || !sliced_rows || !sliced_cols || !lsmr_path || !pair_tails) {
        lsq_set_error("lsq_model_paths: null argument");
        return LSQ_EARG;
    }
    const lsq_mat *J = md->J;
    *sliced_rows = J->kind == LSQ_MAT_CSC && J->srows.active;
    *sliced_cols = J->kind == LSQ_MAT_CSC && J->scols.active;
    *lsmr_path = lsq_workspace_lsmr_path(md->ctx, J);
    *pair_tails = md->pair_tails;
    return LSQ_OK;
}

extern "C" int lsq_model_destroy(lsq_model *md) {
    if (!md) return LSQ_OK;
    hipStreamSynchronize(md->ctx->stream);
    if (md->fused && md->J) lsq_mat_set_colscale(md->J, nullptr);
    hipFree(md->d_Acsc); hipFree(md->d_Acsr); hipFree(md->d_Ab); hipFree(md->d_b); hipFree(md->d_t); hipFree(md->d_s); hipFree(md->d_sspec);
    hipFree(md->d_b_perm); hipFree(md->d_perm[0]); hipFree(md->d_perm[1]);
    delete md;
    return LSQ_OK;
}
```

leastsquaresoptim.jl_amd/csrc/lsq_optimize.hip:

```cpp
#include <chrono>
#include <cmath>
#include <cstring>

#include "lsq_loop.h"
#include "lsq_spmv.h"

__global__ void __launch_bounds__(1024)
k_lm_damp(int n, const double *__restrict__ colsum, double inv_delta, double *__restrict__ dtd) {
    __shared__ double sh[16];
    __shared__ double s_mean;
    double acc = 0.0;
    for (int i = threadIdx.x; i < n; i += 1024) acc += colsum[i];
    acc = wave_sum(acc);
    if ((threadIdx.x & 63) == 0) sh[threadIdx.x >> 6] = acc;
    __syncthreads();
    if (threadIdx.x == 0) {
        double t = 0.0;
        for (int w = 0; w < 16; ++w) t += sh[w];
        s_mean = t / n;
    }
    __syncthreads();
    const double lo = MIN_DIAGONAL * s_mean, hi = MAX_DIAGONAL * s_mean;
    for (int i = threadIdx.x; i < n; i += 1024) {
        double v = colsum[i];
        v = v > hi ? hi : (v < lo ? lo : v);
        dtd[i] = v * inv_delta;
    }
}

constexpr int LSQ_ONE_WG_N = 16384;

__global__ void __launch_bounds__(1024)
k_lm_damp_grad(int n, const double *__restrict__ colsum, double inv_delta, double *__restrict__ dtd,
               const double *__restrict__ g, const double *__restrict__ x, const double *__restrict__ lo,
               const double *__restrict__ hi, double *out_grad) {
    constexpr int R = LSQ_ONE_WG_N / 1024;
    __shared__ double sh[16];
    __shared__ double s_mean;
    double cs[R], gv[R];
#pragma unroll
    for (int k = 0; k < R; ++k) {
        const int i = threadIdx.x + k * 1024;
        cs[k] = i < n ? colsum[i] : 0.0;
        gv[k] = i < n ? g[i] : 0.0;
    }
    double acc = 0.0, mg = 0.0;
#pragma unroll
    for (int k = 0; k < R; ++k) {
        const int i = threadIdx.x + k * 1024;
        if (i < n) {
            acc += cs[k];
            double gi = gv[k];
            if (lo && x[i] <= lo[i] && gi > 0.0) gi = 0.0;
            else if (hi && x[i] >= hi[i] && gi < 0.0) gi = 0.0;
            double a = fabs(gi);
            if (isnan(a)) a = INFINITY;
            mg = fmax(mg, a);
        }
    }
    acc = wave_sum(acc);
    mg = wave_max(mg);
    __shared__ double shm[16];
    if ((threadIdx.x & 63) == 0) {
        sh[threadIdx.x >> 6] = acc;
        shm[threadIdx.x >> 6] = mg;
    }
    __syncthreads();
    if (threadIdx.x == 0) {
        double t = 0.0, tm = shm[0];
        for (int w = 0; w < 16; ++w) t += sh[w];
        for (int w = 1; w < 16; ++w) tm = fmax(tm, shm[w]);
        s_mean = t / n;
        *out_grad = tm;
    }
    __syncthreads();
    const double lo_d = MIN_DIAGONAL * s_mean, hi_d = MAX_DIAGONAL * s_mean;
#pragma unroll
    for (int k = 0; k < R; ++k) {
        const int i = threadIdx.x + k * 1024;
        if (i < n) {
            double v = cs[k];
            v = v > hi_d ? hi_d : (v < lo_d ? lo_d : v);
            dtd[i] = v * inv_delta;
        }
    }
}

__global__ void __launch_bounds__(LSQ_NT)
k_dl_scale(int n, const double *__restrict__ colsum, double *__restrict__ dtd) {
    for (int i = blockIdx.x * LSQ_NT + threadIdx.x; i < n; i += gridDim.x * LSQ_NT) {
        double v = colsum[i];
        dtd[i] = v > MAX_DIAGONAL ? MAX_DIAGONAL : (v < MIN_DIAGONAL ? MIN_DIAGONAL : v);
    }
}

struct EpiGrad {
    static constexpr bool REDUCE = false;
    const int *done;
    int extra_blocks;
    double *g;
    double *partials;
    unsigned *counter;
    __device__ void seg(int j, double dot, double &) const { g[j] = dot; }
    __device__ void extra(int, double &) const {}
    __device__ void finalize(double) const {}
};

struct EpiPredict {
    static constexpr bool REDUCE = true;
    const int *done;
    int extra_blocks;
    const double *f;
    double *out;
    double *partials;
    unsigned *counter;
    __device__ void seg(int i, double dot, double &racc) const { seg_pre(i, dot, f[i], racc); }
    using has_pre = void;
    __device__ double pre(int i) const { return f[i]; }
    __device__ void seg_pre(int, double dot, double fi, double &racc) const {
        double r = dot - fi;
        racc += r * r;
    }
    __device__ void extra(int, double &) const {}
    LsqSlotPublish pub;
    __device__ void finalize(double t) const {
        *out = t;
        if (pub.count > 0) {
            for (int i = 0; i < pub.count; ++i)
                __hip_atomic_store(pub.dst + i, pub.src + i == out ? t : pub.src[i], __ATOMIC_RELAXED,
                                   __HIP_MEMORY_SCOPE_SYSTEM);
            __hip_atomic_store(pub.seq_word, pub.seq, __ATOMIC_RELEASE, __HIP_MEMORY_SCOPE_SYSTEM);
        }
    }
};

struct EpiSumsq {
    static constexpr bool REDUCE = true;
    const int *done;
    int extra_blocks;
    double *out;
    double *partials;
    unsigned *counter;
    __device__ void seg(int, double dot, double &racc) const { racc += dot * dot; }
    __device__ void extra(int, double &) const {}
    __device__ void finalize(double t) const { *out = t; }
};

__global__ void __launch_bounds__(LSQ_NT)
k_step(int n, const double *__restrict__ x, const double *__restrict__ dx, double *__restrict__ xt,
       double *partials, unsigned *counters, double *out_dx, double *out_nonfin, double *__restrict__ t_out,
       double *__restrict__ s_out, const int *skip = nullptr) {
    __shared__ double sh[LSQ_NT / 64];
    if (skip && *skip) return;
    double mx = 0.0, code = 0.0;
    for (int i = blockIdx.x * LSQ_NT + threadIdx.x; i < n; i += gridDim.x * LSQ_NT) {
        double d = dx[i];
        double v = x[i] + -1.0 * d;
        xt[i] = v;
        if (t_out) {
            const double th = tanh(v);
            t_out[i] = th;
            s_out[i] = 1.0 - th * th;
        }
        double a = fabs(d);
        if (isnan(a)) a = INFINITY;
        mx = fmax(mx, a);
        if (!isfinite(v) && code == 0.0) code = 1e15 - (double)(i + 1);
    }
    double b2 = block_max<LSQ_NT>(code, sh);
    if (threadIdx.x == 0) __hip_atomic_store(&partials[LSQ_MAX_GRID + blockIdx.x], b2, RLX_AGENT);
    double b1 = block_max<LSQ_NT>(mx, sh);
    const int nb = gridDim.x;
    if (grid_reduce<LSQ_NT, true>(b1, partials, counters, nb, sh, [=](double t) { *out_dx = t; })) {
        double acc = 0.0;
        for (int i = threadIdx.x; i < nb; i += LSQ_NT) acc = fmax(acc, __hip_atomic_load(&partials[LSQ_MAX_GRID + i], RLX_AGENT));
        double t = block_max<LSQ_NT>(acc, sh);
        if (threadIdx.x == 0) *out_nonfin = (t == 0.0) ? -1.0 : (1e15 - t) - 1.0;
    }
}

__global__ void __launch_bounds__(LSQ_NT)
k_revert(int n, const double *__restrict__ xt, const double *__restrict__ dx, double *__restrict__ x) {
    for (int i = blockIdx.x * LSQ_NT + threadIdx.x; i < n; i += gridDim.x * LSQ_NT)
        x[i] = xt[i] + 1.0 * dx[i];
}

__global__ void __launch_bounds__(LSQ_NT)
k_gradnorm(int n, const double *__restrict__ g, const double *__restrict__ x, const double *__restrict__ lo,
           const double *__restrict__ hi, double *partials, unsigned *counter, double *out) {
    __shared__ double sh[LSQ_NT / 64];
    double m = 0.0;
    for (int i = blockIdx.x * LSQ_NT + threadIdx.x; i < n; i += gridDim.x * LSQ_NT) {
        double gi = g[i];
        if (lo && x[i] <= lo[i] && gi > 0.0) gi = 0.0;
        else if (hi && x[i] >= hi[i] && gi < 0.0) gi = 0.0;
        double a = fabs(gi);
        if (isnan(a)) a = INFINITY;
        m = fmax(m, a);
    }
    double b = block_max<LSQ_NT>(m, sh);
    grid_reduce<LSQ_NT, true>(b, partials, counter, gridDim.x, sh, [=](double t) { *out = t; });
}

__global__ void __launch_bounds__(LSQ_NT)
k_sumsq_slot(long long n, const double *__restrict__ x, double *partials, unsigned *counter, double *out,
             LsqSlotPublish pub) {
    __shared__ double sh[LSQ_NT / 64];
    double acc = 0.0;
    const long long stride = (long long)gridDim.x * LSQ_NT;
    long long i = blockIdx.x * (long long)LSQ_NT + threadIdx.x;
    for (; i + 3 * stride < n; i += 4 * stride) {
        const double v0 = x[i], v1 = x[i + stride], v2 = x[i + 2 * stride], v3 = x[i + 3 * stride];
        acc += v0 * v0;
        acc += v1 * v1;
        acc += v2 * v2;
        acc += v3 * v3;
    }
    for (; i < n; i += stride) {
        double v = x[i];
        acc += v * v;
    }
    double b = block_sum<LSQ_NT>(acc, sh);
    grid_reduce<LSQ_NT>(b, partials, counter, gridDim.x, sh, [=](double t) {
        *out = t;
        if (pub.count > 0) {
            for (int i = 0; i < pub.count; ++i)
                __hip_atomic_store(pub.dst + i, pub.src + i == out ? t : pub.src[i], __ATOMIC_RELAXED,
                                   __HIP_MEMORY_SCOPE_SYSTEM);
            __hip_atomic_store(pub.seq_word, pub.seq, __ATOMIC_RELEASE, __HIP_MEMORY_SCOPE_SYSTEM);
        }
    });
}

__global__ void __launch_bounds__(LSQ_NT)
k_wdot_slot(int n, const double *__restrict__ x, const double *__restrict__ y, const double *__restrict__ w,
            double *partials, unsigned *counter, double *out) {
    __shared__ double sh[LSQ_NT / 64];
    double acc = 0.0;
    for (int i = blockIdx.x * LSQ_NT + threadIdx.x; i < n; i += gridDim.x * LSQ_NT) acc += w[i] * x[i] * y[i];
    double b = block_sum<LSQ_NT>(acc, sh);
    grid_reduce<LSQ_NT>(b, partials, counter, gridDim.x, sh, [=](double t) { *out = t; });
}

__global__ void __launch_bounds__(LSQ_NT)
k_lincomb(int n, double a, const double *__restrict__ p, double b, const double *__restrict__ q,
          double *__restrict__ out) {
    for (int i = blockIdx.x * LSQ_NT + threadIdx.x; i < n; i += gridDim.x * LSQ_NT) {
        double v = p[i] * a;
        if (q) v += b * q[i];
        out[i] = v;
    }
}

static int sumsq_to_slot(lsq_ctx *c, bool exact, long long n, const double *x, int ctr, double *d_out,
                         LsqSlotPublish pub = LsqSlotPublish()) {
    if (exact) return lsq_seq_reduce(c, 1, (int)n, x, nullptr, nullptr, d_out);
    long long g = (n + LSQ_NT - 1) / LSQ_NT, cap = (long long)c->num_cus * 2;
    if (g > cap) g = cap;
    if (g < 1) g = 1;
    LSQ_LAUNCH(k_sumsq_slot, dim3((int)g), dim3(LSQ_NT), 0, c->stream, n, x, c->d_partials, lsq_ctr(c, ctr), d_out,
                       pub);
    return LSQ_OK;
}
static int f_then_sumsq(lsq_ctx *c, bool exact, lsq_f_callback f, void *user, long long m, double *out, const double *x, int ctr,
                        double *d_out, LsqSlotPublish pub = LsqSlotPublish(), const int *skip = nullptr, bool mirror = false) {
    if (!exact && model_is_builtin(f)) {
        bool fused = false;
        if (model_f_sumsq(user, out, x, ctr, d_out, pub, &fused, skip, mirror) != 0) {
            lsq_set_error("user callback reported failure");
            return LSQ_ECALLBACK;
        }
        if (fused) return LSQ_OK;
    } else if (f(out, x, user) != 0) {
        lsq_set_error("user callback reported failure");
        return LSQ_ECALLBACK;
    }
    return sumsq_to_slot(c, exact, m, out, ctr, d_out, pub);
}
static int predicted_to_slot(lsq_ctx *c, bool exact, lsq_mat *J, const double *d, const double *f, double *scratch,
                             int ctr, double *d_out, LsqSlotPublish pub = LsqSlotPublish(), const int *skip = nullptr) {
    if (exact) {
        LSQ_TRY(lsq_exact_product(J, 0, d, scratch));
        return lsq_seq_reduce(c, f ? 3 : 1, J->m, scratch, f, nullptr, d_out);
    }
    if (f) {
        EpiPredict ep{skip, 0, f, d_out, c->d_partials, lsq_ctr(c, ctr), pub};
        return launch_product(J, 0, d, ep);
    }
    EpiSumsq es{nullptr, 0, d_out, c->d_partials, lsq_ctr(c, ctr)};
    return launch_product(J, 0, d, es);
}
static int wdot_to_slot(lsq_ctx *c, bool exact, int n, const double *x, const double *y, const double *w, int ctr,
                        double *d_out) {
    if (exact) return lsq_seq_reduce(c, 2, n, x, y, w, d_out);
    int g = lsq_div_up(n > 0 ? n : 1, LSQ_NT), cap = c->num_cus * 8;
    LSQ_LAUNCH(k_wdot_slot, dim3(g > cap ? cap : g), dim3(LSQ_NT), 0, c->stream, n, x, y, w, c->d_partials,
                       lsq_ctr(c, ctr), d_out);
    return LSQ_OK;
}
static int gradient_into(lsq_ctx *c, bool exact, lsq_mat *J, const double *f, double *g) {
    (void)c;
    if (exact) return lsq_exact_product(J, 1, f, g);
    EpiGrad eg{nullptr, 0, g, nullptr, nullptr};
    return launch_product(J, 1, f, eg);
}

struct LoopBuffers {
    lsq_ctx *c;
    int m, n;
    double *dx = nullptr, *dtd = nullptr, *xt = nullptr, *ftrial = nullptr;
    double *dgn = nullptr, *dgr = nullptr, *grad = nullptr, *fpred = nullptr;
    double *lo = nullptr, *hi = nullptr;
    int *gate_ring = nullptr;
    int gate_next = 0;
    static constexpr int GATE_RING = 1024;
// ... 50 lines not shown
    }
    LSQ_HIP(hipStreamSynchronize(c->stream));
    return LSQ_OK;
}

static bool assess(double maxabs_dx, double maxabs_gr, double ssr, double trial_ssr, double xtol, double ftol,
                   double gtol, bool accepted, int *xc, int *fc, int *gc) {
    *xc = *fc = *gc = 0;
    if (accepted && std::fabs(trial_ssr - ssr) <= ftol * (std::fabs(ssr) + ftol)) *fc = 1;
    else if (maxabs_dx <= xtol) *xc = 1;
    else if (maxabs_gr <= gtol) *gc = 1;
    return *xc || *fc || *gc;
}

static void record(const lsq_options *o, lsq_ctx *c, int it, int n, double ssr, double g, double delta, double rho,
                   int inner, int acc, const double *d_x) {
    if (it > o->trace_cap) return;
    int k = it - 1;
    if (o->trace_ssr) o->trace_ssr[k] = ssr;
    if (o->trace_gnorm) o->trace_gnorm[k] = g;
    if (o->trace_delta) o->trace_delta[k] = delta;
    if (o->trace_rho) o->trace_rho[k] = rho;
    if (o->trace_inner) o->trace_inner[k] = inner;
    if (o->trace_accept) o->trace_accept[k] = acc;
    if (o->trace_x) {
        hipMemcpyAsync(o->trace_x + (size_t)k * n, d_x, (size_t)n * sizeof(double), hipMemcpyDeviceToHost, c->stream);
        hipStreamSynchronize(c->stream);
    }
}

extern "C" void lsq_options_default(lsq_options *o) {
    memset(o, 0, sizeof(*o));
    o->x_tol = o->f_tol = o->g_tol = 1e-8;
    o->iterations = 1000;
    o->delta = -1.0;
}

static int check_start(const double *hx, int n, const lsq_options *o) {
    for (int i = 0; i < n; ++i) {
        if (o->h_lower && !(hx[i] >= o->h_lower[i])) return LSQ_EBOUNDS;
        if (o->h_upper && !(hx[i] <= o->h_upper[i])) return LSQ_EBOUNDS;
    }
    return LSQ_OK;
}

static int *next_gate(lsq_ctx *c, LoopBuffers &b) {
    if (!b.gate_ring) return nullptr;
    if (b.gate_next >= LoopBuffers::GATE_RING) {
        if (hipMemsetAsync(b.gate_ring, 1, LoopBuffers::GATE_RING * sizeof(int), c->stream) != hipSuccess) return nullptr;
        b.gate_next = 0;
    }
    return b.gate_ring + b.gate_next++;
}

static thread_local int t_xchg_issued = 0;
static thread_local bool t_xchg_hook_failed = false;
static int global_exchange(const lsq_options *o, double *ssr, double *gnorm, int *all_converged) {
    if (!o->allreduce) return LSQ_OK;
    double v[3] = {*ssr, *gnorm, (double)*all_converged};
    t_xchg_issued++;
    const int rc = o->allreduce(v, 3, o->allreduce_user);
    if (rc == 2 || (rc == 0 && v[2] < -0.5)) {
        lsq_set_error("sharded run: a peer rank left its loop with an error");
        return LSQ_ERCCL;
    }
    if (rc != 0) {
        t_xchg_hook_failed = true;
        lsq_set_error("allreduce callback failed");
        return LSQ_ECALLBACK;
    }
    *ssr = v[0];
    *gnorm = v[1];
    *all_converged = v[2] > 0.5 ? 1 : 0;
    return LSQ_OK;
}

struct ShardedExit {
    lsq_ctx *c;
    const lsq_options *o;
    ShardedExit(lsq_ctx *c_, const lsq_options *o_) : c(c_), o(o_) {
        t_xchg_issued = 0;
        t_xchg_hook_failed = false;
    }
    int finish(int st) {
        c->idle_hook = nullptr;
        c->idle_user = nullptr;
        if (st != LSQ_OK && st != LSQ_ERCCL && o->allreduce && !t_xchg_hook_failed && t_xchg_issued < o->iterations) {
            double v[3] = {0.0, 0.0, -1.0};
            (void)o->allreduce(v, 3, o->allreduce_user);
        }
        return st;
    }
};

#define CB(call)                                          \
    do {                                                  \
        if ((call) != 0) {                                \
            lsq_set_error("user callback reported failure"); \
            return LSQ_ECALLBACK;                         \
        }                                                 \
    } while (0)

static int call_g(lsq_g_callback g, lsq_mat *J, const double *x, void *user) {
    J->version++;
    if (J->kind == LSQ_MAT_CSC && !J->d_cs_user) J->csr_fresh = false;
    CB(g(J, x, user));
    return lsq_ensure_csr(J);
}
int lsq_call_g(lsq_g_callback g, lsq_mat *J, const double *x, void *user) { return call_g(g, J, x, user); }

struct IterateGuard {
    lsq_ctx *c;
    double *&x, *&fcur;
    double *x_user, *fcur_user;
    int m, n;
    ~IterateGuard() {
        if (x != x_user) lsq_d2d(c, x_user, x, (size_t)n * sizeof(double));
        if (fcur != fcur_user) lsq_d2d(c, fcur_user, fcur, (size_t)m * sizeof(double));
    }
};

struct StartAhead {
    int (*fn)(void *);
    void *user;
};
static int start_residual(lsq_ctx *c, lsq_mat *J, lsq_f_callback f, void *user, double *fcur, const double *x, double *ssr,
                          int *nonfinite_at, bool pair_next = false, const StartAhead *ahead = nullptr) {
    const int m = J->m, n = J->n;
    if (lsq_small_mat(J) || lsq_small_vec(m) || m <= 0) {
        CB(f(fcur, x, user));
        LSQ_TRY(lsq_sumsq(c, m, fcur, ssr));
        return lsq_first_nonfinite(c, n, x, nonfinite_at);
    }
    static_assert(SL_TRIAL == SL_NONFIN + 1, "the two scalars of the loop head travel together");
    bool head = false;
    if (model_is_builtin(f) && model_start_point(user, x, c->d_slots + SL_NONFIN, &head) != 0) return LSQ_EHIP;
    if (!head) LSQ_TRY(lsq_first_nonfinite_to_slot(c, n, x, c->d_slots + SL_NONFIN));
    const LsqSlotPublish pub = lsq_slots_ticket(c, SL_NONFIN, 2);
    double sl[2];
    int st = f_then_sumsq(c, false, f, user, m, fcur, x, 7, c->d_slots + SL_TRIAL, pub, nullptr, pair_next);
    if (st == LSQ_OK && head && ahead) st = ahead->fn(ahead->user);
    if (st == LSQ_OK) st = lsq_wait_slots(c, SL_NONFIN, 2, pub.seq, sl);
    if (st != LSQ_OK || (int)sl[0] >= 0) {
        if (head) model_forget_point(user);
        if (st != LSQ_OK) return st;
    }
    *nonfinite_at = (int)sl[0];
    *ssr = sl[1];
    return LSQ_OK;
}

static int launch_step(lsq_ctx *c, bool model, void *user, int gn, int n, const double *x, const double *dx, double *xt,
                       const int *skip = nullptr) {
    double *t_out = nullptr, *s_out = nullptr;
    if (model) model_trial_buffers(user, xt, &t_out, &s_out);
    LSQ_LAUNCH(k_step, dim3(gn), dim3(LSQ_NT), 0, c->stream, n, x, dx, xt, c->d_partials, lsq_ctr(c, 5), c->d_slots + SL_DX,
               c->d_slots + SL_NONFIN, t_out, s_out, skip);
    LSQ_HIP(hipGetLastError());
    return LSQ_OK;
}

static int frozen_turn(const lsq_options *o, double ssr, double maxabs_gr, double *gssr, double *ggr, bool *all) {
    int a = 1;
    *gssr = ssr; *ggr = maxabs_gr;
    LSQ_TRY(global_exchange(o, gssr, ggr, &a));
    *all = a != 0;
    return LSQ_OK;
}

static int nonfinite_exit(lsq_result *r, int nonfinite_at, int iter) {
    r->bad_index = nonfinite_at;
    r->iterations = iter - 1;
    lsq_set_error("IsFiniteException: non-finite x at index %d", nonfinite_at);
    return LSQ_ENONFINITE;
}

struct LoopTally {
    int f_calls = 0, g_calls = 0, mul_calls = 0, xc = 0, fc = 0, gc = 0;
    long long inner_total = 0;
};
static int finish_result(lsq_ctx *c, lsq_result *r, int optimizer, double ssr, int iter, bool converged, const LoopTally &t) {
    LSQ_HIP(hipStreamSynchronize(c->stream));
    r->optimizer = optimizer;
    r->ssr = ssr;
    r->iterations = iter;
    r->converged = converged; r->x_converged = t.xc; r->f_converged = t.fc; r->g_converged = t.gc;
    r->f_calls = t.f_calls; r->g_calls = t.g_calls; r->mul_calls = t.mul_calls;
    r->lsmr_iterations = t.inner_total;
    return LSQ_OK;
}

static int rows_sum(lsq_ctx *c, const lsq_options *o, double *d_buf, int count) {
    if (o->row_allreduce(d_buf, count, (void *)c->stream, o->row_allreduce_user) != 0) {
        lsq_set_error("row all-reduce callback reported failure");
        return LSQ_ECALLBACK;
    }
    return LSQ_OK;
}

struct LmAhead {
    lsq_g_callback g; lsq_mat *J; const double *x; void *user; const double *fcur; double *grad;
    bool g_done, grad_done;
};
static int lm_ahead(void *p) {
    LmAhead &a = *(LmAhead *)p;
    LSQ_TRY(call_g(a.g, a.J, a.x, a.user));
    a.g_done = true;
    if (a.J->colsum_version != a.J->version && lsq_can_fuse_grad_colsum(a.J)) {
        LSQ_TRY(lsq_sparse_grad_colsum(a.J, a.fcur, a.grad));
        a.grad_done = true;
    }
    return LSQ_OK;
}

namespace {
struct SpecGuard {
    lsq_mat *J;
    bool &ready, &pending;
    ~SpecGuard() { if (ready || pending) lsq_sparse_colsum_forget(J); }
};
}

struct LmXchg { const lsq_options *o; double *gssr, *ggr; };
static int lm_idle_exchange(void *p) {
    LmXchg *q = (LmXchg *)p;
    int all = 0;
    return global_exchange(q->o, q->gssr, q->ggr, &all);
}

struct LmTail {
    lsq_ctx *c; lsq_mat *J; LoopBuffers *b; lsq_f_callback f; void *user; const lsq_options *o;
    const double *x, *fcur; double *xt, *ftrial;
    int m, n, gn;
    bool is_model;
    bool want_spec;
    double ssr;
    bool *spec_pending;
    LsqSlotPublish pub;
    bool spec_launched;
    bool step_taken = false;
};
static int lm_tail(const int *skip, void *u) {
    LmTail &t = *(LmTail *)u;
    lsq_ctx *c = t.c;
    if (!t.step_taken) LSQ_TRY(launch_step(c, t.is_model, t.user, t.gn, t.n, t.x, t.b->dx, t.xt, skip));
    t.pub = lsq_slots_ticket(c, SL_GRAD, 6);
    bool pair = false;
    SpecGrad sg{t.want_spec ? next_gate(c, *t.b) : nullptr, t.ssr, t.b->grad, false, t.o->x_tol, t.o->f_tol, t.o->g_tol};
    if (t.is_model && model_pair_tail(t.user, t.J, t.b->dx, t.fcur, t.ftrial, t.xt, c->d_slots + SL_PRED, c->d_slots + SL_TRIAL,
                                      t.pub, skip, &pair, &sg) != 0) {
        lsq_set_error("user callback reported failure");
        return LSQ_ECALLBACK;
    }
    t.spec_launched = sg.launched;
    if (sg.launched) *t.spec_pending = true;
    if (!pair) {
        LSQ_TRY(predicted_to_slot(c, false, t.J, t.b->dx, t.fcur, t.b->fpred, 8, c->d_slots + SL_PRED, LsqSlotPublish(), skip));
        LSQ_TRY(f_then_sumsq(c, false, t.f, t.user, t.m, t.ftrial, t.xt, 7, c->d_slots + SL_TRIAL, t.pub, skip));
    }
    LSQ_HIP(hipGetLastError());
    return LSQ_OK;
}

static int optimize_lm_loop(lsq_ctx *c, lsq_solver *sv, LoopBuffers &b, lsq_mat *J, double *x_user, double *fcur_user,
                            lsq_f_callback f, lsq_g_callback g, void *user, const lsq_options *o, lsq_result *r) {
    const int m = J->m, n = J->n;
    double *x = x_user, *fcur = fcur_user, *xt = b.xt, *ftrial = b.ftrial;
    IterateGuard guard{c, x, fcur, x_user, fcur_user, m, n};
    double delta = o->delta > 0 ? o->delta : 10.0;
    double decrease_factor = 2.0;
    int f_calls = 0, g_calls = 0, mul_calls = 0, xc = 0, fc = 0, gc = 0;
    bool converged = false;
    double ssr;
    int iter = 0, nonfinite_at = -1;
    const bool sharded = o->row_allreduce != nullptr;
    const bool model_fg = model_is_builtin(f, g);
    LmAhead ah{g, J, x, user, fcur, b.grad, false, false};
    const StartAhead ahead{lm_ahead, &ah};
    const bool ahead_ok = model_fg && sv->kind == LSQ_LSMR && o->iterations > 0;
    if (sharded) CB(f(fcur, x, user));
    else {
        const int st = start_residual(c, J, f, user, fcur, x, &ssr, &nonfinite_at,
                                      sv->kind == LSQ_LSMR && !o->h_lower && !o->h_upper && !lsq_small_mat(J),
                                      ahead_ok ? &ahead : nullptr);
        if (ah.g_done && (st != LSQ_OK || nonfinite_at >= 0)) lsq_sparse_colsum_forget(J);
        LSQ_TRY(st);
    }
    f_calls++;
    if (sharded) {
        LSQ_TRY(sumsq_to_slot(c, false, m, fcur, 7, c->d_slots + SL_TRIAL));
        LSQ_TRY(rows_sum(c, o, c->d_slots + SL_TRIAL, 1));
        LSQ_TRY(lsq_read_slots(c, SL_TRIAL, 1, &ssr));
        LSQ_TRY(lsq_first_nonfinite(c, n, x, &nonfinite_at));
    }
    r->ssr0 = ssr;
    double maxabs_gr = INFINITY;
    bool need_jac = true;
    const int gn = ngrid(c, n);
    const bool exact = lsq_small_mat(J) && !sharded && !(sv->kind == LSQ_LSMR && sv->gen_ldiv);
    const bool is_model = !exact && model_is_builtin(f);
    int last_inner = 0;
    const bool no_spec_grad = getenv("LSQ_NO_SPEC_GRADIENT") != nullptr;
    bool spec_launched = false, spec_grad_ready = false, spec_pending = false;
    SpecGuard spec_guard{J, spec_grad_ready, spec_pending};
    double gssr = ssr, ggr = maxabs_gr;
    LmXchg xchg{o, &gssr, &ggr};
    long long inner_total = 0;
    while (iter < o->iterations) {
        if (converged) {
            if (!o->allreduce) break;
            bool all;
            LSQ_TRY(frozen_turn(o, ssr, maxabs_gr, &gssr, &ggr, &all));
            if (all) break;
            ++iter;
            continue;
        }
        iter++;
        if (nonfinite_at >= 0) return nonfinite_exit(r, nonfinite_at, iter);
        if (need_jac) {
            if (!ah.g_done) LSQ_TRY(call_g(g, J, x, user));
            ah.g_done = false;
            g_calls++;
            need_jac = false;
        }
        bool have_grad = ah.grad_done;
        ah.grad_done = false;
        if (spec_grad_ready) {
            lsq_sparse_grad_colsum_adopt(J);
            have_grad = true;
            spec_grad_ready = false;
        }
        const bool spec_ok = !no_spec_grad && !exact && !sharded && sv->kind == LSQ_LSMR && model_fg && iter < o->iterations &&
                             !lsq_dbg_serial;
        spec_launched = false;
        if (!exact && J->colsum_version != J->version && lsq_can_fuse_grad_colsum(J)) {
            LSQ_TRY(lsq_sparse_grad_colsum(J, fcur, b.grad));
            have_grad = true;
        }
        const double *cs = nullptr;
        LSQ_TRY(lsq_rowshard_colsum(sv, J, &cs));
        const bool one_wg = !exact && n <= LSQ_ONE_WG_N;
        const bool lm_prep = one_wg && sv->kind == LSQ_LSMR && ssr >= 0.0 && lsq_lsmr_takes_lm_prep(sv, J);
        if (exact) LSQ_TRY(lsq_exact_lm_damp(c, n, cs, 1.0 / delta, b.dtd));
        else if (!one_wg) LSQ_LAUNCH(k_lm_damp, dim3(1), dim3(1024), 0, c->stream, n, cs, 1.0 / delta, b.dtd);
        {
            if (!have_grad) LSQ_TRY(gradient_into(c, exact, J, fcur, b.grad));
            if (sharded) LSQ_TRY(rows_sum(c, o, b.grad, n));
            if (lm_prep) {}
            else if (one_wg)
                LSQ_LAUNCH(k_lm_damp_grad, dim3(1), dim3(1024), 0, c->stream, n, cs, 1.0 / delta, b.dtd, b.grad,
                                   x, b.lo, b.hi, c->d_slots + SL_GRAD);
            else
                LSQ_LAUNCH(k_gradnorm, dim3(gn), dim3(LSQ_NT), 0, c->stream, n, b.grad, x, b.lo, b.hi,
                                   c->d_partials, lsq_ctr(c, 4), c->d_slots + SL_GRAD);
            mul_calls++;
        }
        if (o->allreduce) {
            gssr = ssr; ggr = maxabs_gr;
            c->idle_hook = lm_idle_exchange;
            c->idle_user = &xchg;
            c->idle_status = 0;
            if (sv->kind != LSQ_LSMR || exact) lsq_run_idle_hook(c);
        }
        int lmiter = 0;
        LmTail tc{c, J, &b, f, user, o, x, fcur, xt, ftrial, m, n, gn, is_model, spec_ok, ssr, &spec_pending, LsqSlotPublish(), false};
        const bool tail_ok = !exact && !sharded && sv->kind == LSQ_LSMR && !b.lo && !b.hi;
        bool tail_done = false;
        if (sv->kind == LSQ_LSMR) {
            const LsmrLmPrep prep{cs, 1.0 / delta, MIN_DIAGONAL, MAX_DIAGONAL, x, b.lo, b.hi, c->d_slots + SL_GRAD};
            static const bool no_spec = getenv("LSQ_NO_TAIL_SPECULATION") != nullptr;
            const bool guardable = tc.is_model && J->kind == LSQ_MAT_CSC && J->srows.active && !no_spec && !lsq_dbg_serial;
            LsmrTail tail{guardable ? last_inner : 0, lm_tail, &tc, guardable};
            LsmrStepDesc sd{x, xt, nullptr, nullptr, c->d_partials, lsq_ctr(c, 5), c->d_slots + SL_DX, c->d_slots + SL_NONFIN};
            if (tail_ok && guardable) {
                if (is_model) model_trial_buffers(user, xt, &sd.t_out, &sd.s_out);
                tail.step = &sd;
                tail.step_taken = &tc.step_taken;
            }
            LSQ_TRY(lsq_lsmr_solve(sv, J, fcur, b.dtd, b.dx, &lmiter, b.grad, ssr, lm_prep ? &prep : nullptr,
                                   tail_ok ? &tail : nullptr));
            tail_done = tail_ok;
            last_inner = lmiter / 2;
        }
        else LSQ_TRY(lsq_ldiv_damped(sv, J, fcur, b.dtd, b.dx, &lmiter));
        lsq_run_idle_hook(c);
        if (o->allreduce && c->idle_status != LSQ_OK) return c->idle_status;
        mul_calls += lmiter;
        inner_total += lmiter / 2;
        double sl[6] = {0, 0, 0, 0, 0, 0};
        if (!tail_done && !exact && !sharded) {
            LSQ_TRY(lsq_box_clip(c, n, b.dx, x, b.lo, b.hi));
            LSQ_TRY(lm_tail(nullptr, &tc));
            tail_done = true;
        }
        if (tail_done) {
            f_calls++;
            spec_launched = tc.spec_launched;
            LSQ_TRY(lsq_wait_slots(c, SL_GRAD, 6, tc.pub.seq, sl));
        } else {
            LSQ_TRY(lsq_box_clip(c, n, b.dx, x, b.lo, b.hi));
            LSQ_TRY(launch_step(c, is_model, user, gn, n, x, b.dx, xt));
            if (exact) {
                CB(f(ftrial, xt, user));
                f_calls++;
                LSQ_TRY(sumsq_to_slot(c, exact, m, ftrial, 7, c->d_slots + SL_TRIAL));
                LSQ_TRY(predicted_to_slot(c, exact, J, b.dx, fcur, b.fpred, 8, c->d_slots + SL_PRED));
                LSQ_HIP(hipGetLastError());
                LSQ_TRY(lsq_read_slots(c, SL_GRAD, 5, sl));
            } else {
                static_assert(SL_PRED == SL_TRIAL + 1, "trial and predicted ssr travel together");
                LSQ_TRY(predicted_to_slot(c, exact, J, b.dx, fcur, b.fpred, 8, c->d_slots + SL_PRED));
                LSQ_TRY(f_then_sumsq(c, exact, f, user, m, ftrial, xt, 7, c->d_slots + SL_TRIAL));
                f_calls++;
                LSQ_TRY(rows_sum(c, o, c->d_slots + SL_TRIAL, 2));
                LSQ_TRY(lsq_read_slots(c, SL_GRAD, 5, sl));
            }
        }
        mul_calls++;
        maxabs_gr = sl[0];
        const double maxabs_dx = sl[1];
        const int trial_nonfinite = (int)sl[2];
        const double trial_ssr = sl[3], predicted_ssr = sl[4];
        const double pred_red = std::fabs(ssr - predicted_ssr);
        const double rho = pred_red > 0 ? (ssr - trial_ssr) / pred_red : 0.0;
        const bool accepted = rho > MIN_STEP_QUALITY;
        converged = assess(maxabs_dx, maxabs_gr, ssr, trial_ssr, o->x_tol, o->f_tol, o->g_tol, accepted, &xc, &fc, &gc);
        const bool dev_ran = spec_launched && sl[5] != 0.0;
        const bool host_goes_on = accepted && !converged;
        spec_grad_ready = dev_ran && host_goes_on;
        if (dev_ran && !host_goes_on) lsq_sparse_colsum_forget(J);
        spec_pending = false;
        if (accepted) {
            std::swap(fcur, ftrial);
            std::swap(x, xt);
            ssr = trial_ssr;
            double q = 1.0 - (2.0 * rho - 1.0) * (2.0 * rho - 1.0) * (2.0 * rho - 1.0);
            delta = std::min(delta / std::max(1.0 / 3.0, q), MAX_DELTA);
            decrease_factor = 2.0;
            need_jac = true;
            nonfinite_at = trial_nonfinite;
        } else {
            LSQ_LAUNCH(k_revert, dim3(gn), dim3(LSQ_NT), 0, c->stream, n, xt, b.dx, x);
            nonfinite_at = trial_nonfinite;
            delta = std::max(delta / decrease_factor, MIN_DELTA);
            decrease_factor *= 2.0;
        }
        record(o, c, iter, n, ssr, maxabs_gr, delta, rho, lmiter, accepted ? 1 : 0, x);
    }
    return finish_result(c, r, LSQ_LEVENBERG_MARQUARDT, o->allreduce ? gssr : ssr, iter, converged,
                         LoopTally{f_calls, g_calls, mul_calls, xc, fc, gc, inner_total});
}
static int optimize_lm(lsq_ctx *c, lsq_solver *sv, LoopBuffers &b, lsq_mat *J, double *x_user, double *fcur_user,
                       lsq_f_callback f, lsq_g_callback g, void *user, const lsq_options *o, lsq_result *r) {
    ShardedExit ex{c, o};
    return ex.finish(optimize_lm_loop(c, sv, b, J, x_user, fcur_user, f, g, user, o, r));
}

static int optimize_dogleg_loop(lsq_ctx *c, lsq_solver *sv, LoopBuffers &b, lsq_mat *J, double *x_user, double *fcur_user,
                                lsq_f_callback f, lsq_g_callback g, void *user, const lsq_options *o, lsq_result *r) {
    const int m = J->m, n = J->n;
    double *x = x_user, *fcur = fcur_user, *xt = b.xt, *ftrial = b.ftrial;
    IterateGuard guard{c, x, fcur, x_user, fcur_user, m, n};
    double delta = o->delta > 0 ? o->delta : 1.0;
    bool reuse = false, converged = false;
    double wnorm_dgn = 0.0, wnorm_dgr = 0.0, alpha = 0.0, wdot_gr_gn = 0.0;
    int f_calls = 0, g_calls = 0, mul_calls = 0, xc = 0, fc = 0, gc = 0;
    double ssr;
    int iter = 0, nonfinite_at = -1;
    LSQ_TRY(start_residual(c, J, f, user, fcur, x, &ssr, &nonfinite_at));
    f_calls++;
    r->ssr0 = ssr;
    double maxabs_gr = INFINITY;
    const int gn = ngrid(c, n);
    const bool exact = lsq_small_mat(J);
    const bool is_model = !exact && model_is_builtin(f);
    double gssr = ssr, ggr = maxabs_gr;
    long long inner_total = 0;
    while (iter < o->iterations) {
        if (converged) {
            if (!o->allreduce) break;
            bool all;
            LSQ_TRY(frozen_turn(o, ssr, maxabs_gr, &gssr, &ggr, &all));
            if (all) break;
            ++iter;
            continue;
        }
        iter++;
        if (nonfinite_at >= 0) return nonfinite_exit(r, nonfinite_at, iter);
        int ls_iter = 0;
        bool exchanged = false;
        if (!reuse) {
            LSQ_TRY(call_g(g, J, x, user));
            g_calls++;
            bool have_grad = false;
            if (!exact && J->colsum_version != J->version && lsq_can_fuse_grad_colsum(J)) {
                LSQ_TRY(lsq_sparse_grad_colsum(J, fcur, b.dgr));
                have_grad = true;
            }
            const double *cs = lsq_cached_colsum(J);
            if (!cs) return LSQ_EHIP;
            LSQ_LAUNCH(k_dl_scale, dim3(gn), dim3(LSQ_NT), 0, c->stream, n, cs, b.dtd);
            if (iter == 1) {
                double wx2;
                LSQ_TRY(lsq_wdot(c, n, x, x, b.dtd, &wx2));
                double wx = std::sqrt(wx2);
                if (wx > 0) delta *= wx;
            }
            if (!have_grad) LSQ_TRY(gradient_into(c, exact, J, fcur, b.dgr));
            mul_calls++;
            LSQ_LAUNCH(k_gradnorm, dim3(gn), dim3(LSQ_NT), 0, c->stream, n, b.dgr, x, b.lo, b.hi,
                               c->d_partials, lsq_ctr(c, 4), c->d_slots + SL_GRAD);
            LSQ_TRY(lsq_ediv(c, n, b.dgr, b.dtd, b.dgr));
            LSQ_TRY(wdot_to_slot(c, exact, n, b.dgr, b.dgr, b.dtd, 5, c->d_slots + SL_W0));
            LSQ_TRY(predicted_to_slot(c, exact, J, b.dgr, nullptr, b.fpred, 6, c->d_slots + SL_SUM));
            mul_calls++;
            LSQ_TRY(lsq_fill(c, n, 0.0, b.dgn));
            if (o->allreduce) {
                int all = 0;
                gssr = ssr; ggr = maxabs_gr;
                LSQ_TRY(global_exchange(o, &gssr, &ggr, &all));
                exchanged = true;
            }
            if (sv->kind == LSQ_LSMR) LSQ_TRY(lsq_lsmr_solve(sv, J, fcur, nullptr, b.dgn, &ls_iter));
            else LSQ_TRY(lsq_ldiv(sv, J, fcur, b.dgn, &ls_iter));
            mul_calls += ls_iter;
            inner_total += ls_iter / 2;
            LSQ_TRY(wdot_to_slot(c, exact, n, b.dgn, b.dgn, b.dtd, 5, c->d_slots + SL_W1));
            LSQ_TRY(wdot_to_slot(c, exact, n, b.dgr, b.dgn, b.dtd, 5, c->d_slots + SL_W2));
// ... 167 lines not shown
```

leastsquaresoptim.jl_amd/csrc/lsq_sell.h:

```cpp
#pragma once

constexpr int LSQ_SELL_POS_BITS = 13;
constexpr unsigned LSQ_SELL_POS_MASK = (1u << LSQ_SELL_POS_BITS) - 1u;
constexpr int LSQ_SELL_ROWS_MAX = 4096;
constexpr int LSQ_SELL_CW_AUTO = 6;
constexpr int LSQ_SELL_CW_MAX = 32;
constexpr int LSQ_SELL_GROWS_MAX = 16384;
constexpr int LSQ_SELL_CCOLS_MAX = 2560;

struct SellDev {
    const int2 *smeta;
    const unsigned *info;
    const unsigned short *idx16;
    const double *val;
    int nblocks;
    int spw;
};

template <int U>
struct SellBatch {
    double2 a[U];
    unsigned c[U];
};
template <int U, bool CLAMP>
// ... 230 lines not shown
    __device__ __forceinline__ void post(size_t, double, double) const {}
};
template <bool SQ, class Out, class Hook = SellNoSliceHook, class Before = SellNoBeforeBarrier>
__device__ __forceinline__ bool sell_wave_slices(const SellDev &S, int s0, int s1, int wv, int lane, const double *xl, Out out,
                                                 Hook hook = Hook(), Before before_barrier = Before(), int stop = 0,
                                                 bool have_first = false, SellSliceRef first = SellSliceRef()) {
    constexpr int NW = LSQ_BIG_NT / 64;
    int s = s0 + wv;
    SellSliceRef A;
    A.sm = make_int2(0, 0);
    A.inf = LSQ_SELL_POS_MASK;
    if (!have_first) A = sell_slice_ref(S, s, s1, lane);
    SellHead H;
    double hp0 = 0.0;
    const int2 smv = have_first ? first.sm : A.sm;
    const int2 sm0 = make_int2(__builtin_amdgcn_readfirstlane(smv.x), __builtin_amdgcn_readfirstlane(smv.y));
    if (s < s1) {
        sell_head_load(H, S.val, S.idx16, sm0.x, sm0.y, lane);
        hp0 = hook.pre((size_t)s * 64 + lane);
    }
    before_barrier();
    __syncthreads();
    asm volatile("" : "+v"(stop));
    if (stop) return true;
    if (s < s1) {
        SellSliceRef a;
        a.sm = sm0;
        unsigned inf1 = first.inf;
        asm volatile("" : "+v"(inf1));
        a.inf = have_first ? inf1 : A.inf;
        A = sell_slice_ref(S, s + NW, s1, lane);
        const size_t oa = (size_t)a.sm.x + lane * 2;
        const unsigned pos = a.inf & LSQ_SELL_POS_MASK;
        const size_t pidx = (size_t)s * 64 + lane;
        double sum = 0.0, sq = 0.0;
        sell_lane_sum_head<SQ>(H, S.val + oa, S.idx16 + oa, a.sm.y, (int)(a.inf >> LSQ_SELL_POS_BITS), xl, sum, sq, lane);
        if (pos != LSQ_SELL_POS_MASK) {
            out(pos, sum, sq);
            hook.post(pidx, sum, hp0);
        }
        s += NW;
    }
    for (; s < s1; s += NW) {
        const SellSliceRef a = A;
        A = sell_slice_ref(S, s + NW, s1, lane);
        const size_t oa = (size_t)a.sm.x + lane * 2;
        const unsigned pos = a.inf & LSQ_SELL_POS_MASK;
        const size_t pidx = (size_t)s * 64 + lane;
        const double hp = hook.pre(pidx);
        double sum = 0.0, sq = 0.0;
        sell_lane_sum<SQ>(S.val + oa, S.idx16 + oa, a.sm.y, (int)(a.inf >> LSQ_SELL_POS_BITS), xl, sum, sq, lane);
        if (pos != LSQ_SELL_POS_MASK) {
            out(pos, sum, sq);
            hook.post(pidx, sum, hp);
        }
    }
    return false;
}
template <class Epi>
struct SellEpiSliceHook {
    const Epi &epi;
    __device__ __forceinline__ double pre(size_t pidx) const { return epi.slice_pre(pidx); }
    __device__ __forceinline__ void post(size_t pidx, double sum, double p) const { epi.slice_post(pidx, sum, p); }
};

template <class Epi>
__global__ void __launch_bounds__(LSQ_BIG_NT) k_sell_rows(SellDev S, int wrows, int m, const double *__restrict__ x,
                                                          const double *__restrict__ xscale, int nx, int nxpad, Epi epi) {
    extern __shared__ __attribute__((aligned(16))) double smem[];
    __shared__ double sh[LSQ_BIG_NT / 64];
    double *xl = smem;
    double *yw = smem + nxpad;
    const int tid = threadIdx.x, lane = tid & 63, wv = tid >> 6;
    constexpr int XR = (LSQ_LDS_X_MAX + LSQ_BIG_NT - 1) / LSQ_BIG_NT;
    SellStageTail xtail;
    xtail.v = 0.0;
    xtail.at = -1;
    const bool dma = !xscale && sell_stage_dma_ok(x);
    const SellSliceRef ref0 = sell_slice_ref(S, (int)blockIdx.x * S.spw + wv, (int)blockIdx.x < S.nblocks ? ((int)blockIdx.x + 1) * S.spw : 0, lane);
    int dflag;
    if (dma) {
        xtail = sell_stage_dma<(XR + 1) / 2>(x, xl, nx, tid);
        dflag = epi.done ? *epi.done : 0;
        if constexpr (EpiHasBlockPrepare<Epi>::value) epi.block_prepare();
        if constexpr (EpiHasPrepare<Epi>::value) epi.prepare();
    } else {
        double xr[XR];
#pragma unroll
        for (int q = 0; q < XR; ++q) xr[q] = x[min(tid + q * LSQ_BIG_NT, nx - 1)];
        if (xscale) {
            double sr[XR];
#pragma unroll
            for (int q = 0; q < XR; ++q) sr[q] = xscale[min(tid + q * LSQ_BIG_NT, nx - 1)];
#pragma unroll
            for (int q = 0; q < XR; ++q) xr[q] *= sr[q];
        }
        dflag = epi.done ? *epi.done : 0;

        if constexpr (EpiHasBlockPrepare<Epi>::value) epi.block_prepare();
        if constexpr (EpiHasPrepare<Epi>::value) epi.prepare();
#pragma unroll
        for (int q = 0; q < XR; ++q)
            if (tid + q * LSQ_BIG_NT < nx) xl[tid + q * LSQ_BIG_NT] = xr[q];
        sell_stage_wait();
    }
    if ((int)blockIdx.x >= S.nblocks) {
        sell_stage_wait();
        int d = dflag;
        asm volatile("" : "+v"(d));
        if (d) return;
    }
    bool pending = dma;
    constexpr int Q = LSQ_SELL_ROWS_MAX / LSQ_BIG_NT;
    double racc = 0.0;
    for (int w = blockIdx.x; w < S.nblocks; w += gridDim.x) {
        const int base = w * wrows, rows = min(wrows, m - base);
        const int s0 = w * S.spw, s1 = s0 + S.spw;
        double pre[Q];
        if constexpr (EpiHasPre<Epi>::value) {
#pragma unroll
            for (int q = 0; q < Q; ++q) pre[q] = epi.pre(base + min(tid + q * LSQ_BIG_NT, rows - 1));
        }
        auto staged = [&]() {
            sell_stage_tail_write(xtail, xl);
            if (pending) sell_stage_wait();
        };
        bool stopped;
        if constexpr (EpiHasSliceOut<Epi>::value)
            stopped = sell_wave_slices<false>(S, s0, s1, wv, lane, xl, [&](unsigned pos, double sum, double) { yw[pos] = sum; },
                                              SellEpiSliceHook<Epi>{epi}, staged, dflag, w == (int)blockIdx.x, ref0);
        else
            stopped = sell_wave_slices<false>(S, s0, s1, wv, lane, xl, [&](unsigned pos, double sum, double) { yw[pos] = sum; },
                                              SellNoSliceHook(), staged, dflag, w == (int)blockIdx.x, ref0);
        if (stopped) return;
        xtail.at = -1;
        pending = false;
        __syncthreads();
#pragma unroll
        for (int q = 0; q < Q; ++q) {
            const int i = tid + q * LSQ_BIG_NT;
            if (i < rows) {
                if constexpr (EpiHasPre<Epi>::value) epi.seg_pre(base + i, yw[i], pre[q], racc);
                else epi.seg(base + i, yw[i], racc);
            }
        }
        sell_stage_wait();
    }
    for (int e = blockIdx.x; e < epi.extra_blocks; e += gridDim.x)
        if (tid < LSQ_NT) epi.extra(e, racc);
    finish_block_nt<LSQ_BIG_NT>(epi, racc, sh);
}

template <int U, bool CLAMP>
__device__ __forceinline__ void sell_batch_sum2(SellBatch<U> &B, int p0, int np, int len, const double *xa, const double *xb,
                                                double &sa, double &sb) {
#pragma unroll
    for (int u = 0; u < U; ++u) {
        const unsigned i0 = B.c[u] & 0xffffu, i1 = B.c[u] >> 16;
        double a0 = B.a[u].x * xa[i0], a1 = B.a[u].y * xa[i1], b0 = B.a[u].x * xb[i0], b1 = B.a[u].y * xb[i1];
        asm volatile("" : "+v"(a0), "+v"(a1), "+v"(b0), "+v"(b1));
        const int j = 2 * (p0 + u);
        const bool pin = !CLAMP || p0 + u < np;
        const bool in0 = pin && j < len, in1 = pin && j + 1 < len;
        const double ta0 = sa + a0;
        sa = in0 ? ta0 : sa;
        const double ta1 = sa + a1;
        sa = in1 ? ta1 : sa;
        const double tb0 = sb + b0;
        sb = in0 ? tb0 : sb;
        const double tb1 = sb + b1;
        sb = in1 ? tb1 : sb;
    }
}
__device__ __forceinline__ void sell_lane_sum2(const double *__restrict__ vp, const unsigned short *__restrict__ ip, int L, int len,
                                               const double *xa, const double *xb, double &sa, double &sb, int lane) {
    const int np = L >> 1;
    int p0 = 0;
    SellTail tail;
    tail.a = 0.0;
    tail.c = 0;
    if (L & 1) tail = sell_tail_load(vp, ip, L, lane);
    for (; p0 + 8 <= np; p0 += 8) {
        SellBatch<8> B;
        sell_batch_load<8, false>(B, vp, ip, p0, np);
        sell_batch_sum2<8, false>(B, p0, np, len, xa, xb, sa, sb);
    }
    const int rem = np - p0;
    if (rem > 4) {
        SellBatch<8> B;
        sell_batch_load<8, true>(B, vp, ip, p0, np);
        sell_batch_sum2<8, true>(B, p0, np, len, xa, xb, sa, sb);
    } else if (rem > 2) {
        SellBatch<4> B;
        sell_batch_load<4, true>(B, vp, ip, p0, np);
        sell_batch_sum2<4, true>(B, p0, np, len, xa, xb, sa, sb);
    } else if (rem > 0) {
        SellBatch<2> B;
        sell_batch_load<2, true>(B, vp, ip, p0, np);
        sell_batch_sum2<2, true>(B, p0, np, len, xa, xb, sa, sb);
    }
    if (L & 1) {
        double pa = tail.a * xa[tail.c], pb = tail.a * xb[tail.c];
        asm volatile("" : "+v"(pa), "+v"(pb));
        const bool in = L - 1 < len;
        const double ta = sa + pa, tb = sb + pb;
        sa = in ? ta : sa;
        sb = in ? tb : sb;
    }
}
constexpr int LSQ_PAIR_X_MAX = 10200;
struct SellPairEpi {
    const int *done;
    const double *fa;
    const double *fb;
    double *out_b;
    double *out_b_perm;
    double *part_a, *part_b;
    unsigned *counter;
    double *slot_a, *slot_b;
    LsqSlotPublish pub;
    int *gate;
    double ssr, min_quality;
    double *slot_gate;
    const double *slot_dx, *slot_gr;
    double xtol, ftol, gtol;
};
template <int = 0>
__global__ void __launch_bounds__(LSQ_NT) k_sell_perm_rows(SellDev S, int wrows, int nslices, const double *__restrict__ src,
                                                           double *__restrict__ dst) {
    for (long long i = blockIdx.x * (long long)LSQ_NT + threadIdx.x; i < (long long)nslices * 64; i += (long long)gridDim.x * LSQ_NT) {
        const unsigned inf = S.info[i];
        const unsigned pos = inf & LSQ_SELL_POS_MASK;
        const int w = (int)(i >> 6) / S.spw;
        dst[i] = pos != LSQ_SELL_POS_MASK ? src[(size_t)w * wrows + pos] : 0.0;
    }
}
template <int = 0>
__global__ void __launch_bounds__(LSQ_BIG_NT) k_sell_rows_pair(SellDev S, int wrows, int m, const double *__restrict__ xa,
                                                               const double *__restrict__ sa_scale, const double *__restrict__ xb,
                                                               int nx, int nxpad, SellPairEpi e) {
    extern __shared__ __attribute__((aligned(16))) double smem[];
    __shared__ double sh[LSQ_BIG_NT / 64];
    double *la = smem, *lb = smem + nxpad;
    constexpr int NW = LSQ_BIG_NT / 64;
    const int tid = threadIdx.x, lane = tid & 63, wv = tid >> 6;
    constexpr int XR = (LSQ_PAIR_X_MAX + LSQ_BIG_NT - 1) / LSQ_BIG_NT;
    {
        double ra[XR], rs[XR], rb[XR];
#pragma unroll
        for (int q = 0; q < XR; ++q) {
            const int i = min(tid + q * LSQ_BIG_NT, nx - 1);
            ra[q] = xa[i];
            rs[q] = sa_scale ? sa_scale[i] : 1.0;
            rb[q] = xb[i];
        }
        const int dflag = e.done ? *e.done : 0;
#pragma unroll
        for (int q = 0; q < XR; ++q)
            if (tid + q * LSQ_BIG_NT < nx) {
                la[tid + q * LSQ_BIG_NT] = ra[q] * rs[q];
                lb[tid + q * LSQ_BIG_NT] = rb[q];
            }
        if (dflag) return;
    }
    constexpr int G = LSQ_SELL_ROWS_MAX / 64 / NW;
    double acc_a = 0.0, acc_b = 0.0;
    for (int w = blockIdx.x; w < S.nblocks; w += gridDim.x) {
        const int base = w * wrows, rows = min(wrows, m - base);
        const int s0 = w * S.spw, s1 = s0 + S.spw;
        if (w != (int)blockIdx.x) {
            __syncthreads();
            for (int i = tid; i < nx; i += LSQ_BIG_NT) {
                la[i] = xa[i] * (sa_scale ? sa_scale[i] : 1.0);
                lb[i] = xb[i];
            }
        }
        int s = s0 + wv;
        SellSliceRef A = sell_slice_ref(S, s, s1, lane);
        __syncthreads();
        double keep[G];
        unsigned kpos[G];
#pragma unroll
        for (int g = 0; g < G; ++g) {
            kpos[g] = LSQ_SELL_POS_MASK;
            keep[g] = 0.0;
            if (s < s1) {
                const SellSliceRef a = A;
                A = sell_slice_ref(S, s + NW, s1, lane);
                const unsigned pos = a.inf & LSQ_SELL_POS_MASK;
                const bool valid = pos != LSQ_SELL_POS_MASK;
                const size_t pidx = (size_t)s * 64 + lane;
                const double fa = e.fa[pidx], fb = e.fb[pidx];
                const size_t oa = (size_t)a.sm.x + lane * 2;
                double sum_a = 0.0, sum_b = 0.0;
                sell_lane_sum2(S.val + oa, S.idx16 + oa, a.sm.y, (int)(a.inf >> LSQ_SELL_POS_BITS), la, lb, sum_a, sum_b, lane);
                if (valid) {
                    const double r_a = sum_a - fa, r_b = sum_b - fb;
                    e.out_b_perm[pidx] = r_b;
                    keep[g] = r_b;
                    kpos[g] = pos;
                    acc_a += r_a * r_a;
                    acc_b += r_b * r_b;
                }
                s += NW;
            }
        }
        __syncthreads();
#pragma unroll
        for (int g = 0; g < G; ++g)
            if (kpos[g] != LSQ_SELL_POS_MASK) smem[kpos[g]] = keep[g];
        __syncthreads();
        for (int i = tid; i < rows; i += LSQ_BIG_NT) e.out_b[base + i] = smem[i];
    }
    const double ba = block_sum<LSQ_BIG_NT>(acc_a, sh);
    const double bb = block_sum<LSQ_BIG_NT>(acc_b, sh);
    if (tid == 0) __hip_atomic_store(&e.part_b[blockIdx.x], bb, RLX_AGENT);
    double total_a = 0.0;
    const bool last = grid_reduce<LSQ_BIG_NT>(ba, e.part_a, e.counter, gridDim.x, sh, [&](double t) { total_a = t; });
    if (!last) return;
    double pb = 0.0;
    for (int i = tid; i < (int)gridDim.x; i += LSQ_BIG_NT) pb += __hip_atomic_load(&e.part_b[i], RLX_AGENT);
    const double total_b = block_sum<LSQ_BIG_NT>(pb, sh);
    if (tid == 0) {
        *e.slot_a = total_a;
        *e.slot_b = total_b;
        if (e.gate) {
            const double pred_red = fabs(e.ssr - total_a);
            const double rho = pred_red > 0 ? (e.ssr - total_b) / pred_red : 0.0;
            const bool acc = rho > e.min_quality;
            const bool conv = (acc && fabs(total_b - e.ssr) <= e.ftol * (fabs(e.ssr) + e.ftol)) || *e.slot_dx <= e.xtol ||
                              *e.slot_gr <= e.gtol;
            const bool go = acc && !conv;
            *e.gate = go ? 0 : 1;
            *e.slot_gate = go ? 1.0 : 0.0;
        }
        if (e.pub.count > 0) {
            for (int i = 0; i < e.pub.count; ++i) {
                const double *src = e.pub.src + i;
                const double v = src == e.slot_a ? total_a : (src == e.slot_b ? total_b : *src);
                __hip_atomic_store(e.pub.dst + i, v, __ATOMIC_RELAXED, __HIP_MEMORY_SCOPE_SYSTEM);
            }
            __hip_atomic_store(e.pub.seq_word, e.pub.seq, __ATOMIC_RELEASE, __HIP_MEMORY_SCOPE_SYSTEM);
        }
    }
}

constexpr int LSQ_WIDE_NT = 512;
constexpr int LSQ_SELL_WIDE_X_MAX = 12544;
constexpr int LSQ_SELL_WIDE_G = LSQ_SELL_ROWS_MAX / 64 / (LSQ_WIDE_NT / 64);

template <class Epi>
__global__ void __launch_bounds__(LSQ_WIDE_NT) k_sell_rows_wide(SellDev S, int wrows, int m, int ncw, int cwidth,
                                                                const double *__restrict__ x, int nx, Epi epi) {
    extern __shared__ __attribute__((aligned(16))) double smem[];
    __shared__ double sh[LSQ_WIDE_NT / 64];
    constexpr int NW = LSQ_WIDE_NT / 64, G = LSQ_SELL_WIDE_G;
    double *xl = smem;
    double *yw = smem + cwidth;
    const int tid = threadIdx.x, lane = tid & 63, wv = tid >> 6;
    const int nrb = S.nblocks / ncw;
    constexpr int XR = (LSQ_SELL_WIDE_X_MAX + LSQ_WIDE_NT - 1) / LSQ_WIDE_NT;
    constexpr int Q = LSQ_SELL_ROWS_MAX / LSQ_WIDE_NT;
    SellSliceRef A[G];
    double xr[XR];
    auto refs_at = [&](int w, int cw) {
        const int sb = (w * ncw + cw) * S.spw;
#pragma unroll
        for (int g = 0; g < G; ++g) A[g] = sell_slice_ref(S, sb + wv + g * NW, sb + S.spw, lane);
    };
    auto fetch_x = [&](int cw) {
        const int c0 = cw * cwidth;
#pragma unroll
        for (int q = 0; q < XR; ++q) xr[q] = x[min(c0 + tid + q * LSQ_WIDE_NT, nx - 1)];
    };
    if ((int)blockIdx.x < nrb) refs_at(blockIdx.x, 0);
    const int dflag = epi.done ? *epi.done : 0;
    if constexpr (EpiHasBlockPrepare<Epi>::value) epi.block_prepare();
    if constexpr (EpiHasPrepare<Epi>::value) epi.prepare();
    if (dflag) return;
    double racc = 0.0;
    for (int w = blockIdx.x; w < nrb; w += gridDim.x) {
        const int base = w * wrows, rows = min(wrows, m - base);
        for (int cw = 0; cw < ncw; ++cw) {
            fetch_x(cw);
            SellSliceRef a[G];
            SellBatch<2> B[G];
#pragma unroll
            for (int g = 0; g < G; ++g) {
                a[g] = A[g];
                const size_t oa = (size_t)a[g].sm.x + lane * 2;
                sell_batch_load<2, true>(B[g], S.val + oa, S.idx16 + oa, 0, max(a[g].sm.y >> 1, 1));
            }
            const bool more = cw + 1 < ncw, next_block = w + (int)gridDim.x < nrb;
            if (more) refs_at(w, cw + 1);
            else if (next_block) refs_at(w + gridDim.x, 0);
            __syncthreads();
#pragma unroll
            for (int q = 0; q < XR; ++q)
                if (tid + q * LSQ_WIDE_NT < cwidth) xl[tid + q * LSQ_WIDE_NT] = xr[q];
            if (cw == 0) {
#pragma unroll
                for (int q = 0; q < Q; ++q) yw[tid + q * LSQ_WIDE_NT] = 0.0;
            }
            __syncthreads();
#pragma unroll
            for (int g = 0; g < G; ++g) {
                const int np = a[g].sm.y >> 1, len = (int)(a[g].inf >> LSQ_SELL_POS_BITS);
                const unsigned pos = a[g].inf & LSQ_SELL_POS_MASK;
                if (np == 0) continue;
                double sum = pos != LSQ_SELL_POS_MASK ? yw[pos] : 0.0, sq = 0.0;
                sell_batch_sum<2, true, false>(B[g], 0, np, len, xl, sum, sq);
                if (pos != LSQ_SELL_POS_MASK) yw[pos] = sum;
            }
#pragma unroll
            for (int g = 0; g < G; ++g) {
                if (a[g].sm.y <= 4) continue;
                const unsigned pos = a[g].inf & LSQ_SELL_POS_MASK;
                const size_t oa = (size_t)a[g].sm.x + lane * 2;
                double sum = pos != LSQ_SELL_POS_MASK ? yw[pos] : 0.0, sq = 0.0;
                sell_lane_sum_from<false, false>(S.val + oa, S.idx16 + oa, 2, a[g].sm.y, (int)(a[g].inf >> LSQ_SELL_POS_BITS), xl, sum, sq, lane);
                if (pos != LSQ_SELL_POS_MASK) yw[pos] = sum;
            }
        }
        double pre[Q];
        if constexpr (EpiHasPre<Epi>::value) {
#pragma unroll
            for (int q = 0; q < Q; ++q) pre[q] = epi.pre(base + min(tid + q * LSQ_WIDE_NT, rows - 1));
        }
        __syncthreads();
#pragma unroll
        for (int q = 0; q < Q; ++q) {
            const int i = tid + q * LSQ_WIDE_NT;
            if (i < rows) {
                if constexpr (EpiHasPre<Epi>::value) epi.seg_pre(base + i, yw[i], pre[q], racc);
                else epi.seg(base + i, yw[i], racc);
            }
        }
    }
    for (int e = blockIdx.x; e < epi.extra_blocks; e += gridDim.x)
        if (tid < LSQ_NT) epi.extra(e, racc);
    finish_block_nt<LSQ_WIDE_NT>(epi, racc, sh);
}

template <int = 0>
__global__ void __launch_bounds__(LSQ_NT) k_sell_vmul(int n, const double *__restrict__ a, const double *__restrict__ b,
                                                      double *__restrict__ out) {
    for (int i = blockIdx.x * LSQ_NT + threadIdx.x; i < n; i += gridDim.x * LSQ_NT) out[i] = a[i] * b[i];
}

__device__ __forceinline__ SellStageTail sell_cols_stage_y(int b, int ncb, int grows, int m, const double *__restrict__ y, double *yl,
                                                          int tid) {
    constexpr int YR = LSQ_SELL_GROWS_MAX / LSQ_BIG_NT;
    const int gw = b / ncb, gbase = gw * grows, rows = min(grows, m - gbase);
    SellStageTail t;
    t.v = 0.0;
    t.at = -1;
    if (sell_stage_dma_ok(y + gbase)) {
        if (rows < grows) {
#pragma unroll
            for (int j = 0; j < YR; ++j) {
                const int i = tid + j * LSQ_BIG_NT;
                if (i >= rows && i < grows) yl[i] = 0.0;
            }
        }
        return sell_stage_dma<YR / 2>(y + gbase, yl, rows, tid);
    }
    double yr[YR];
#pragma unroll
    for (int j = 0; j < YR; ++j) yr[j] = y[gbase + min(tid + j * LSQ_BIG_NT, rows - 1)];
#pragma unroll
    for (int j = 0; j < YR; ++j)
        if (tid + j * LSQ_BIG_NT < grows) yl[tid + j * LSQ_BIG_NT] = (tid + j * LSQ_BIG_NT < rows) ? yr[j] : 0.0;
    sell_stage_wait();
    return t;
}
__device__ __forceinline__ int sell_cols_wg() { return lsq_xcd_block((int)blockIdx.x, (int)gridDim.x); }
__device__ __forceinline__ int sell_cols_first(int nblocks) {
    const int per = (nblocks + (int)gridDim.x - 1) / (int)gridDim.x;
    return sell_cols_wg() * per;
}
template <bool SQ>
__device__ __forceinline__ void sell_cols_pass(const SellDev &S, int ncb, int ccols, int grows, int m, int n,
                                               const double *__restrict__ y, double *__restrict__ part, double *smem,
                                               SellStageTail ytail, int dflag, const SellSliceRef &ref0) {
// ... 50 lines not shown
```

leastsquaresoptim.jl_amd/csrc/lsq_solver.h:

```cpp
#pragma once
#include "lsq_common.h"

struct LsmrState {
    double alpha, beta, rho, rhobar, cbar, sbar, zeta, zetabar, alphabar;
    double betadd, betad, rhodold, tautildeold, thetatilde, d;
    double normA2, maxrbar, minrbar, normb, normr, normAr, normA, condA, normx;
    double cu;
    double inv_beta;
    double vscale;
    double c1, c2, c3;
    double atol, btol, ctol;
    int iter, istop, done, maxiter;
    int beta_zero;
    int first;
    unsigned epoch;
    int notdone;
};

struct LsqFallback {
    int giveups = 0;
    int cooldown = 0;
    int next_pause = 16;
    bool exchange = true;
    bool off() const { return cooldown > 0 || (exchange && lsq_dbg_serial >= 2); }
    void gave_up(lsq_ctx *c, int which) {
        giveups++;
        c->fallback_giveups[which]++;
        cooldown = next_pause;
        next_pause = next_pause < 4096 ? next_pause * 4 : 4096;
    }
    void solve_done(bool used_and_clean) {
        if (cooldown > 0) --cooldown;
        else if (used_and_clean) next_pause = 16;
    }
};
enum { LSQ_FB_CHOL_TILES = 0, LSQ_FB_TRI_PIPE = 1, LSQ_FB_QR_EXCHANGE = 2, LSQ_FB_CHOLQR = 3 };

struct lsq_solver {
    lsq_ctx *ctx;
    int kind;
    int for_lm;
    int m, n;
    LsmrState *d_state = nullptr;
    double *d_u = nullptr;
    double *d_ux = nullptr;
    double *d_v = nullptr, *d_h = nullptr, *d_hbar = nullptr, *d_t = nullptr;
    double *d_P = nullptr;
    double *d_dg = nullptr;
    double *d_red = nullptr;
    double *d_f3 = nullptr;
    size_t f3_elems = 0;
    unsigned f3_tag = 0;
    unsigned epoch = 0;
    int last_iter = 0, last_istop = 0;
    int last_lsmr_path = 0;
    int (*row_cb)(double *, int, void *, void *) = nullptr;
    void *row_user = nullptr;
    long long global_rows = 0;
    double *d_xbuf = nullptr;
    double lsmr_ratio2 = 0.1;
    double *d_colsum_g = nullptr;
    unsigned long long colsum_g_uid = 0;
    unsigned long long colsum_g_version = ~0ull;
    int *d_one = nullptr;
    double *d_chol = nullptr;
    double *d_Ds = nullptr;
    double *d_rhs = nullptr;
    int *d_info = nullptr;
    int last_qr_path = 0;
    int last_qr_panel = 0;
    double *d_qr = nullptr;
    double *d_qu = nullptr;
    double *d_tau = nullptr;
    double *d_T = nullptr;
    double *d_work = nullptr;
    size_t work_elems = 0;
    std::vector<double> h_R;
    int last_rank = -1;
    const double *qr_R = nullptr, *qr_X = nullptr;
    int qr_ldr = 0;
    int (*precond_cb)(double *, lsq_mat *, const double *, void *) = nullptr;
    void *precond_user = nullptr;
    int (*gen_update)(lsq_mat *, const double *, void *) = nullptr;
    int (*gen_ldiv)(double *, const double *, void *) = nullptr;
    void *gen_user = nullptr;
    void *qr2 = nullptr;
    void (*qr2_free)(void *) = nullptr;
    void *tripipe = nullptr;
    void (*tripipe_free)(void *) = nullptr;
    double *tri_X = nullptr, *tri_T = nullptr, *tri_fro = nullptr, *tri_hfro = nullptr;
    int last_chol_path = 0;
    LsqFallback fb_pipe;
    bool chol_have_diaginv = false;
    unsigned *d_chol_flags = nullptr;
    unsigned chol_epoch = 0;
    LsqFallback fb_tiles;
    LsqFallback fb_qrx;
    LsqFallback fb_cholqr{0, 0, 16, false};
    bool last_chol_tiles = false;
    bool pub_want = false;
    unsigned long long pub_seq = 0;
    int bd_blocks = 0, bd_mb = 0, bd_nb = 0;
    int last_bd_path = 0;
    int last_bd_block = -1;
    bool bq_solved = false;
    int br_blocks = 0, br_mb = 0, br_nb = 0, br_ng = 0;
    int *d_cov_info = nullptr;
    double *d_cov_buf = nullptr;
};
int lsq_tri_chol_solve(lsq_solver *s, const double *U, int n, double *d_bx);
int lsq_tri_chol_fwd_operands(lsq_solver *s, int n, double **z, unsigned long long **slot, unsigned long long *epoch, int **err);
double *lsq_tri_chol_diagbuf(lsq_solver *s, int n);

#ifdef __HIPCC__
__device__ inline void lsmr_rotate_inline(LsmrState &s, double alpha, double beta) {
    const double lambda = 0.0;
    double alphahat = sqrt(s.alphabar * s.alphabar + lambda * lambda);
    double chat = s.alphabar / alphahat, shat = lambda / alphahat;
    double rhoold = s.rho;
    double rho = sqrt(alphahat * alphahat + beta * beta);
    double c = alphahat / rho, sn = beta / rho;
    double thetanew = sn * alpha;
    s.alphabar = c * alpha;
    double rhobarold = s.rhobar, zetaold = s.zeta;
    double thetabar = s.sbar * rho;
    double rhotemp = s.cbar * rho;
    double rhobar = sqrt((s.cbar * rho) * (s.cbar * rho) + thetanew * thetanew);
    s.cbar = s.cbar * rho / rhobar;
    s.sbar = thetanew / rhobar;
    s.zeta = s.cbar * s.zetabar;
    s.zetabar = -s.sbar * s.zetabar;
    s.rho = rho;
    s.rhobar = rhobar;
    s.c1 = -thetabar * rho / (rhoold * rhobarold);
    s.c2 = s.zeta / (rho * rhobar);
    s.c3 = -thetanew / rho;
    double betaacute = chat * s.betadd, betacheck = -shat * s.betadd;
    double betahat = c * betaacute;
    s.betadd = -sn * betaacute;
    double thetatildeold = s.thetatilde;
    double rhotildeold = sqrt(s.rhodold * s.rhodold + thetabar * thetabar);
    double ctildeold = s.rhodold / rhotildeold, stildeold = thetabar / rhotildeold;
    s.thetatilde = stildeold * rhobar;
    s.rhodold = ctildeold * rhobar;
    s.betad = -stildeold * s.betad + ctildeold * betahat;
    s.tautildeold = (zetaold - thetatildeold * s.tautildeold) / rhotildeold;
    double taud = (s.zeta - s.thetatilde * s.tautildeold) / s.rhodold;
    s.d = s.d + betacheck * betacheck;
    s.normr = sqrt(s.d + (s.betad - taud) * (s.betad - taud) + s.betadd * s.betadd);
    s.normA2 = s.normA2 + beta * beta;
    s.normA = sqrt(s.normA2);
    s.normA2 = s.normA2 + alpha * alpha;
    s.maxrbar = fmax(s.maxrbar, rhobarold);
    if (s.iter + 1 > 1) s.minrbar = fmin(s.minrbar, rhobarold);
    s.condA = fmax(s.maxrbar, rhotemp) / fmin(s.minrbar, rhotemp);
    s.normAr = fabs(s.zetabar);
}

#endif

int lsq_lsmr_alloc(lsq_solver *s);
void lsq_lsmr_free(lsq_solver *s);
struct LsmrLmPrep {
    const double *colsum;
    double inv_delta, min_diag, max_diag;
    const double *x, *lo, *hi;
    double *out_grad;
};
constexpr int LSMR_LM_PREP_MAX_N = 16384;
struct LsmrStepDesc {
    const double *x = nullptr;
    double *xt = nullptr, *t_out = nullptr, *s_out = nullptr;
    double *partials = nullptr;
    unsigned *counter = nullptr;
    double *out_dx = nullptr, *out_nonfin = nullptr;
};
struct LsmrTail {
    int predict = 0;
    int (*fn)(const int *skip, void *user) = nullptr;
    void *user = nullptr;
    bool dynamic = false;
    const LsmrStepDesc *step = nullptr;
    bool *step_taken = nullptr;
};
int lsq_rowshard_colsum(lsq_solver *s, lsq_mat *J, const double **out);
int lsq_lsmr_solve(lsq_solver *s, lsq_mat *J, const double *d_y, double *d_damp, double *d_x, int *nmul,
                   const double *d_Jty = nullptr, double y_sumsq = -1.0, const LsmrLmPrep *lm = nullptr,
                   const LsmrTail *tail = nullptr);
bool lsq_lsmr_takes_lm_prep(const lsq_solver *s, const lsq_mat *J);
int lsq_lsmr_general_solve(lsq_solver *s, lsq_mat *J, const double *d_y, double *d_damp, double *d_x, int *nmul);
int lsq_lsmr_exact_solve(lsq_solver *s, lsq_mat *J, const double *d_y, double *d_damp, double *d_x, int *nmul);
int lsq_dense_solver_alloc(lsq_solver *s);
void lsq_dense_solver_free(lsq_solver *s);
int lsq_cholesky_solve(lsq_solver *s, lsq_mat *J, const double *d_y, const double *d_damp, double *d_x, int *nmul);
int lsq_qr_solve(lsq_solver *s, lsq_mat *J, const double *d_y, const double *d_damp, double *d_x, int *nmul);
bool lsq_cholesky_takes_blocked(int m, int n);
int lsq_cholesky_small_factor(lsq_solver *s, lsq_mat *J);
int lsq_tri_inv_enqueue(lsq_solver *s, const double *U, int n);
int lsq_blockdiag_solver_alloc(lsq_solver *s, const lsq_mat *J);
int lsq_blockdiag_solve(lsq_solver *s, lsq_mat *J, const double *d_y, const double *d_damp, double *d_x, int *nmul);
int lsq_blockdiag_solve_blocks(lsq_ctx *c, lsq_mat *J, bool pivot, const double *d_y, const double *d_delta, double *d_x,
                               const int *d_active, int *d_binfo, double *d_r, double *d_diag);
int lsq_bordered_solver_alloc(lsq_solver *s, const lsq_mat *J);
int lsq_bordered_solve(lsq_solver *s, lsq_mat *J, const double *d_y, const double *d_damp, double *d_x, int *nmul);
int lsq_bordered_covariance(lsq_solver *s, lsq_mat *J, const double *d_f, double *d_cov, double *d_stderr, int *h_info);
int lsq_blockqr_solver_alloc(lsq_solver *s, const lsq_mat *J);
int lsq_blockqr_solve(lsq_solver *s, lsq_mat *J, const double *d_y, const double *d_damp, double *d_x, int *nmul);
int lsq_blockqr_solve_blocks(lsq_ctx *c, lsq_mat *J, bool lm, const double *d_y, const double *d_delta, double *d_x,
                             const int *d_active, int *d_ranks, double *d_r, double *d_diag);
int lsq_call_g(lsq_g_callback g, lsq_mat *J, const double *x, void *user);
```

leastsquaresoptim.jl_amd/synthetic.py:

```python
import ctypes as C

import numpy as np

from . import _lib
from ._lib import check, lib
from .api import (DeviceVector, LeastSquaresResult, _run_native, _run_native_batched, default_context)

BASE_SEED = 20260928


def sparse_inputs(m, n, per_col, seed):
    nnz = n * per_col
    colptr = np.zeros(n + 1, dtype=np.int32)
    rowval = np.zeros(nnz, dtype=np.int32)
    nzval = np.zeros(nnz)
    check(lib().lsq_synth_sparse(m, n, per_col, seed, colptr.ctypes.data_as(_lib.c_ip),
                                 rowval.ctypes.data_as(_lib.c_ip), nzval.ctypes.data_as(_lib.c_dp)))
    return colptr, rowval, nzval


def dense_inputs(m, n, seed):
    v = np.zeros(m * n)
    check(lib().lsq_synth_dense(m, n, seed, v.ctypes.data_as(_lib.c_dp)))
    return v


def blockdiag_inputs(nblocks, mb, nb, seed):
    return dense_inputs(mb, nblocks * nb, seed)


def bordered_inputs(nblocks, mb, nb, ng, seed):
    return np.concatenate([blockdiag_inputs(nblocks, mb, nb, seed), dense_inputs(nblocks * mb, ng, seed + 1)])


def uniform(n, seed, lo=-1.0, hi=1.0):
    v = np.zeros(n)
    check(lib().lsq_synth_uniform(n, seed, lo, hi, v.ctypes.data_as(_lib.c_dp)))
    return v


def normal(n, seed):
    v = np.zeros(n)
    check(lib().lsq_synth_normal(n, seed, v.ctypes.data_as(_lib.c_dp)))
    return v


def rhs_for(matvec, m, n, seed, noise=1e-3):
    x_true = uniform(n, seed + 101)
    b = matvec(np.tanh(x_true)) + noise * normal(m, seed + 202)
    return x_true, b


def csc_matvec(m, colptr, rowval, nzval, t):
    n = len(colptr) - 1
    cols = np.repeat(np.arange(n), np.diff(colptr))
    return np.bincount(rowval, weights=nzval * t[cols], minlength=m)


class _Handle:
    __slots__ = ("h",)

    def __init__(self, h):
        self.h = h


class TanhProblem:

    def __init__(self, m, n, sparse=True, per_col=None, seed=BASE_SEED, ctx=None, inputs=None, b=None, blockdiag=None,
                 bordered=None):
        self.ctx = ctx or default_context()
        self.m, self.n, self.sparse = m, n, sparse
        self.blockdiag = None
        self.bordered = None
        L = lib()
        h = C.c_void_p()
        if bordered is not None:
            B, mb, nb, ng = (int(v) for v in bordered)
            if (m, n) != (B * mb, B * nb + ng):
                raise ValueError("bordered=(%d, %d, %d, %d) is a %d x %d problem, not %d x %d"
                                 % (B, mb, nb, ng, B * mb, B * nb + ng, m, n))
            self.bordered, self.sparse = (B, mb, nb, ng), True
            if inputs is None:
                inputs = bordered_inputs(B, mb, nb, ng, seed)
            self.A = inputs
            check(L.lsq_blockdiag_bordered_create(self.ctx.h, B, mb, nb, ng, C.byref(h)))
            self.nnz = len(self.A)
            A3 = self.A[:B * mb * nb].reshape((B, nb, mb))
            Cg = self.A[B * mb * nb:].reshape((m, ng), order="F")
            mv = lambda t: np.einsum("bjr,bj->br", A3, t[:B * nb].reshape((B, nb))).reshape(-1) + Cg @ t[B * nb:]
        elif blockdiag is not None:
            B, mb, nb = (int(v) for v in blockdiag)
            if (m, n) != (B * mb, B * nb):
                raise ValueError("blockdiag=(%d, %d, %d) is a %d x %d problem, not %d x %d" % (B, mb, nb, B * mb, B * nb, m, n))
            self.blockdiag, self.sparse = (B, mb, nb), True
            if inputs is None:
                inputs = blockdiag_inputs(B, mb, nb, seed)
            self.A = inputs
            check(L.lsq_blockdiag_create(self.ctx.h, B, mb, nb, C.byref(h)))
            self.nnz = len(self.A)
            A3 = self.A.reshape((B, nb, mb))
            mv = lambda t: np.einsum("bjr,bj->br", A3, t.reshape((B, nb))).reshape(-1)
        elif sparse:
            if inputs is None:
                inputs = sparse_inputs(m, n, per_col, seed)
            colptr, rowval, nzval = inputs
            self.colptr, self.rowval, self.A = colptr, rowval, nzval
            check(L.lsq_csc_create(self.ctx.h, m, n, colptr.ctypes.data_as(_lib.c_ip),
                                   rowval.ctypes.data_as(_lib.c_ip), C.byref(h)))
            self.nnz = len(nzval)
            mv = lambda t: csc_matvec(m, colptr, rowval, nzval, t)
        else:
            if inputs is None:
                inputs = dense_inputs(m, n, seed)
            self.A = inputs
            check(L.lsq_dense_create(self.ctx.h, m, n, C.byref(h)))
            self.nnz = m * n
            Amat = self.A.reshape((m, n), order="F")
            mv = lambda t: Amat @ t
        self.J = h
        if b is None:
            self.x_true, self.b = rhs_for(mv, m, n, seed)
        else:
            self.x_true, self.b = None, np.ascontiguousarray(b, dtype=np.float64)
        md = C.c_void_p()
        check(L.lsq_model_tanh_create(self.ctx.h, self.J, self.A.ctypes.data_as(_lib.c_dp),
                                      self.b.ctypes.data_as(_lib.c_dp), C.byref(md)))
        self.model = md
        self.x = DeviceVector(self.ctx, n)
        self.fcur = DeviceVector(self.ctx, m)
        self._Jd = None
        self._fg = None

    def reset(self, x0=None):
        if x0 is None:
            check(lib().lsq_fill(self.ctx.h, self.n, 0.0, self.x.ptr))
        else:
            self.x.set(x0)

    def optimize(self, optimizer_kind, solver_kind, x_tol=1e-8, f_tol=1e-8, g_tol=1e-8, iterations=1000,
                 delta=None, trace=False, allreduce=None, fetch_x=True, row_allreduce=None, row_allreduce_user=None,
                 global_rows=0):
        if self._Jd is None:
            L = lib()
            self._Jd = _Handle(self.J)
            self._fg = (L.lsq_model_f(), L.lsq_model_g())
        Jd = self._Jd
        st, res, tr = _run_native(self.ctx, optimizer_kind, solver_kind, Jd, self.x, self.fcur,
                                  self._fg[0], self._fg[1], self.model, x_tol, f_tol, g_tol,
                                  iterations, delta, None, None, trace, self.n, allreduce=allreduce,
                                  row_allreduce=row_allreduce, row_allreduce_user=row_allreduce_user, global_rows=global_rows)
        check(st)
        r = LeastSquaresResult()
        r.optimizer = "LevenbergMarquardt" if res.optimizer == _lib.LEVENBERG_MARQUARDT else "Dogleg"
        r.ssr, r.iterations = float(res.ssr), res.iterations
        r.converged = bool(res.converged)
        r.x_converged, r.f_converged, r.g_converged = bool(res.x_converged), bool(res.f_converged), bool(res.g_converged)
        r.x_tol, r.f_tol, r.g_tol = x_tol, f_tol, g_tol
        r.f_calls, r.g_calls, r.mul_calls = res.f_calls, res.g_calls, res.mul_calls
        r.seconds, r.lsmr_iterations = res.seconds, int(res.lsmr_iterations)
        r.trace = tr
        r.minimizer = self.x.get() if fetch_x else None
        return r

    def optimize_batched(self, optimizer_kind=_lib.LEVENBERG_MARQUARDT, solver_kind=_lib.CHOLESKY, x_tol=1e-8, f_tol=1e-8,
                         g_tol=1e-8, iterations=1000, delta=None, lower=None, upper=None, trace=False, fetch_x=True):
        if self.blockdiag is None:
            raise _lib.ArgumentError(_lib.EARG, "optimize_batched needs a problem built with blockdiag=(nblocks, mb, nb)")
        if self._fg is None:
            L = lib()
            self._Jd = _Handle(self.J)
            self._fg = (L.lsq_model_f(), L.lsq_model_g())
        name = "LevenbergMarquardt" if optimizer_kind == _lib.LEVENBERG_MARQUARDT else "Dogleg"
        st, r = _run_native_batched(self.ctx, optimizer_kind, solver_kind, self.J, self.blockdiag, self.x, self.fcur,
                                    self._fg[0], self._fg[1], self.model, x_tol, f_tol, g_tol, iterations, delta, lower, upper,
                                    trace, name)
        check(st)
        r.minimizer = self.x.get() if fetch_x else None
        return r

    def paths(self):
        rows, cols, lpath, pairs = C.c_int(), C.c_int(), C.c_int(), C.c_longlong()
        check(lib().lsq_model_paths(self.model, C.byref(rows), C.byref(cols), C.byref(lpath), C.byref(pairs)))
        return dict(sliced_rows=bool(rows.value), sliced_cols=bool(cols.value), pair_tails=pairs.value,
                    lsmr_path={0: None, 1: "reference-order", 2: "four-launch", 3: "three-launch", 4: "general"}[lpath.value])

    def close(self):
        L = lib()
        if self.model:
            L.lsq_model_destroy(self.model)
            self.model = None
        if self.J:
            L.lsq_mat_destroy(self.J)
            self.J = None
```

Before: 4302.

## Interleave trial step and tanh vectors for pair SpMV and fuse grid reductions

The step kernels now also write an interleaved double2 vector of scaled step and tanh values, so the paired SELL row kernel can stage both operands into LDS with a single async global-to-LDS copy and gather both from one 16-byte load per column index. The two grid reductions in the pair kernel are merged into one two-value reduction, and the first chunk's staging overlaps the slice metadata loads and done-flag reads. This adds a device buffer of size 2n plus an extra store in the step kernel, in exchange for fewer gather loads and less staging arithmetic in the hot tail kernel.

```diff
diff --git a/include/lsqhip.h b/include/lsqhip.h
--- a/include/lsqhip.h
+++ b/include/lsqhip.h
@@ -192,6 +192,7 @@
 lsq_f_callback lsq_model_f(void);
 lsq_g_callback lsq_model_g(void);
 int lsq_model_paths(const lsq_model *md, int *sliced_rows, int *sliced_cols, int *lsmr_path, long long *pair_tails);
+int lsq_model_pair_vector_tails(const lsq_model *md, long long *out);
 
 int lsq_synth_sparse(int m, int n, int per_col, unsigned long long seed, int *h_colptr,
                      int *h_rowval, double *h_nzval);
diff --git a/leastsquaresoptim.jl_amd/_lib.py b/leastsquaresoptim.jl_amd/_lib.py
--- a/leastsquaresoptim.jl_amd/_lib.py
+++ b/leastsquaresoptim.jl_amd/_lib.py
@@ -176,6 +176,7 @@
         "lsq_model_f": (F_CALLBACK, []),
         "lsq_model_g": (G_CALLBACK, []),
         "lsq_model_paths": (i, [vp, c_ip, c_ip, c_ip, C.POINTER(C.c_longlong)]),
+        "lsq_model_pair_vector_tails": (i, [vp, C.POINTER(C.c_longlong)]),
         "lsq_synth_sparse": (i, [i, i, i, C.c_ulonglong, c_ip, c_ip, c_dp]),
         "lsq_synth_dense": (i, [i, i, C.c_ulonglong, c_dp]),
         "lsq_synth_uniform": (i, [i, C.c_ulonglong, d, d, c_dp]),
diff --git a/leastsquaresoptim.jl_amd/csrc/lsq_common.h b/leastsquaresoptim.jl_amd/csrc/lsq_common.h
--- a/leastsquaresoptim.jl_amd/csrc/lsq_common.h
+++ b/leastsquaresoptim.jl_amd/csrc/lsq_common.h
@@ -345,6 +345,49 @@
     return true;
 }
 
+template <int NT>
+__device__ __forceinline__ bool grid_reduce2(double val_a, double val_b, double *part_a, double *part_b, unsigned *counter,
+                                             int nblocks, double *sh, double &tot_a, double &tot_b) {
+    __shared__ int s_last2;
+    const int b = blockIdx.x;
+    if (threadIdx.x == 0) {
+        __hip_atomic_store(&part_a[b], val_a, RLX_AGENT);
+        __hip_atomic_store(&part_b[b], val_b, RLX_AGENT);
+        asm volatile("s_waitcnt vmcnt(0)" ::: "memory");
+        const int g = b % LSQ_RGROUPS;
+        const int ngroups = nblocks < LSQ_RGROUPS ? nblocks : LSQ_RGROUPS;
+        const unsigned gsize = (unsigned)((nblocks - g + LSQ_RGROUPS - 1) / LSQ_RGROUPS);
+        int last = 0;
+        if (nblocks <= LSQ_RFLAT) {
+            if (__hip_atomic_fetch_add(counter, 1u, RLX_AGENT) == (unsigned)(nblocks - 1)) {
+                __hip_atomic_store(counter, 0u, RLX_AGENT);
+                last = 1;
+            }
+        } else if (__hip_atomic_fetch_add(counter + (1 + g) * LSQ_CTR_STRIDE, 1u, RLX_AGENT) == gsize - 1) {
+            __hip_atomic_store(counter + (1 + g) * LSQ_CTR_STRIDE, 0u, RLX_AGENT);
+            unsigned t2 = __hip_atomic_fetch_add(counter, 1u, RLX_AGENT);
+            if (t2 == (unsigned)(ngroups - 1)) {
+                __hip_atomic_store(counter, 0u, RLX_AGENT);
+                last = 1;
+            }
+        }
+        s_last2 = last;
+    }
+    __syncthreads();
+    if (!s_last2) return false;
+    if (threadIdx.x == 0) __builtin_amdgcn_fence(__ATOMIC_ACQUIRE, "agent");
+    __syncthreads();
+    double acc_a = 0.0, acc_b = 0.0;
+    for (int i = threadIdx.x; i < nblocks; i += NT) {
+        const double pa = __hip_atomic_load(&part_a[i], RLX_AGENT), pb = __hip_atomic_load(&part_b[i], RLX_AGENT);
+        acc_a += pa;
+        acc_b += pb;
+    }
+    tot_a = block_sum<NT>(acc_a, sh);
+    tot_b = block_sum<NT>(acc_b, sh);
+    return true;
+}
+
 struct LsqSlotPublish {
     const double *src = nullptr;
     int count = 0;
diff --git a/leastsquaresoptim.jl_amd/csrc/lsq_loop.h b/leastsquaresoptim.jl_amd/csrc/lsq_loop.h
--- a/leastsquaresoptim.jl_amd/csrc/lsq_loop.h
+++ b/leastsquaresoptim.jl_amd/csrc/lsq_loop.h
@@ -31,6 +31,6 @@
 int model_pair_tail(void *user, lsq_mat *J, const double *dx, const double *fcur, double *ftrial, const double *xt,
                     double *slot_pred, double *slot_trial, LsqSlotPublish pub, const int *skip, bool *done,
                     SpecGrad *sg = nullptr);
-void model_trial_buffers(void *user, const double *xt, double **t_out, double **s_out);
+void model_trial_buffers(void *user, const double *xt, double **t_out, double **s_out, double **pv_out, const double **pscale_out);
 
 int lsq_workspace_lsmr_path(const lsq_ctx *c, const lsq_mat *J);
diff --git a/leastsquaresoptim.jl_amd/csrc/lsq_lsmr3.h b/leastsquaresoptim.jl_amd/csrc/lsq_lsmr3.h
--- a/leastsquaresoptim.jl_amd/csrc/lsq_lsmr3.h
+++ b/leastsquaresoptim.jl_amd/csrc/lsq_lsmr3.h
@@ -210,6 +210,7 @@
     }
     double e_vt[NU], e_P[NU], e_dg[NU], e_ux[NU], e_h[NU], e_hb[NU], e_x[NU];
     double e_s[NU];
+    [[maybe_unused]] double e_sc[NU];
 #pragma unroll
     for (int k = 0; k < NU; ++k) {
         const int j = min((int)(blockIdx.x + k * gstride) * LSQ_BIG_NT + tid, n - 1);
@@ -220,7 +221,10 @@
         e_h[k] = a.h_in[j];
         e_hb[k] = a.hbar_in[j];
         e_x[k] = a.x_in[j];
-        if constexpr (STEP) e_s[k] = sd.x[j];
+        if constexpr (STEP) {
+            e_s[k] = sd.x[j];
+            e_sc[k] = sd.pv ? sd.pscale[j] : 0.0;
+        }
     }
     double aux = 0.0;
     double mx = 0.0, code = 0.0;
@@ -254,6 +258,12 @@
                 const double th = tanh(v);
                 sd.t_out[j] = th;
                 sd.s_out[j] = 1.0 - th * th;
+                if (sd.pv) {
+                    double2 ab;
+                    ab.x = dj * e_sc[k];
+                    ab.y = th;
+                    reinterpret_cast<double2 *>(sd.pv)[j] = ab;
+                }
             }
             double ad = fabs(dj);
             if (isnan(ad)) ad = INFINITY;
diff --git a/leastsquaresoptim.jl_amd/csrc/lsq_model.hip b/leastsquaresoptim.jl_amd/csrc/lsq_model.hip
--- a/leastsquaresoptim.jl_amd/csrc/lsq_model.hip
+++ b/leastsquaresoptim.jl_amd/csrc/lsq_model.hip
@@ -19,7 +19,10 @@
     double *d_b_perm = nullptr;
     double *d_perm[2] = {nullptr, nullptr};
     const double *perm_of[2] = {nullptr, nullptr};
+    double *d_pv = nullptr;
+    const double *pv_x = nullptr;
     long long pair_tails = 0;
+    long long pv_tails = 0;
 };
 static void model_perm_invalidate(lsq_model *md, const double *vec) {
     for (int k = 0; k < 2; ++k)
@@ -186,7 +189,7 @@
     lsq_ctx *c = md->ctx;
     lsq_mat *J = md->J;
     const bool have_tanh = md->tanh_x == x;
-    md->tanh_x = nullptr;
+    md->tanh_x = md->pv_x = nullptr;
     model_perm_invalidate(md, out);
     if (!have_tanh) {
         md->sfac_x = nullptr;
@@ -207,13 +210,22 @@
     return hipGetLastError() == hipSuccess ? 0 : 1;
 }
 
-void model_trial_buffers(void *user, const double *xt, double **t_out, double **s_out) {
-    lsq_model *md = (lsq_model *)user;
-    md->tanh_x = md->sfac_x = nullptr;
+static bool model_pair_applies(const lsq_model *md, const lsq_mat *J);
+static bool model_perm_ready(lsq_model *md);
+void model_trial_buffers(void *user, const double *xt, double **t_out, double **s_out, double **pv_out, const double **pscale_out) {
+    lsq_model *md = (lsq_model *)user;
+    md->tanh_x = md->sfac_x = md->pv_x = nullptr;
+    *pv_out = nullptr;
+    *pscale_out = nullptr;
     if ((md->J->kind == LSQ_MAT_CSC && md->J->srows.active) || md->J->kind == LSQ_MAT_DENSE) {
         *t_out = md->d_t;
         *s_out = md->d_sspec;
         md->tanh_x = md->sfac_x = xt;
+        if (model_pair_applies(md, md->J) && model_perm_ready(md) && md->d_pv) {
+            *pv_out = md->d_pv;
+            *pscale_out = md->J->d_colscale;
+            md->pv_x = xt;
+        }
     }
 }
 
@@ -222,7 +234,7 @@
     lsq_ctx *c = md->ctx;
     lsq_mat *J = md->J;
     *done = false;
-    md->tanh_x = md->sfac_x = nullptr;
+    md->tanh_x = md->sfac_x = md->pv_x = nullptr;
     if (!(J->kind == LSQ_MAT_CSC && J->srows.active) || J->n <= 0) return 0;
     LSQ_LAUNCH(k_tanh_sfac, dim3(ngrid(c, J->n)), dim3(LSQ_NT), 0, c->stream, J->n, x, md->d_t, md->d_sspec, c->d_partials,
                lsq_ctr(c, 0), d_nonfin);
@@ -233,7 +245,7 @@
 }
 void model_forget_point(void *user) {
     lsq_model *md = (lsq_model *)user;
-    md->tanh_x = md->sfac_x = nullptr;
+    md->tanh_x = md->sfac_x = md->pv_x = nullptr;
 }
 
 static bool model_pair_applies(const lsq_model *md, const lsq_mat *J) {
@@ -254,6 +266,12 @@
         return false;
     }
     md->d_b_perm = pb; md->d_perm[0] = p0; md->d_perm[1] = p1;
+    const size_t pvlen = (size_t)2 * (((size_t)md->J->n + 1) & ~(size_t)1);
+    if (getenv("LSQ_NO_PAIR_VECTOR")) md->d_pv = nullptr;
+    else if (hipMalloc(&md->d_pv, std::max<size_t>(pvlen, 2) * sizeof(double)) != hipSuccess) {
+        (void)hipGetLastError();
+        md->d_pv = nullptr;
+    }
     LSQ_LAUNCH(k_sell_perm_rows<0>, dim3(pgrid), dim3(LSQ_NT), 0, c->stream, sell_dev(S), S.wrows, S.nslices, (const double *)md->d_b,
                md->d_b_perm);
     return true;
@@ -269,7 +287,7 @@
     model_perm_invalidate(md, out);
     EpiResidualSq e{skip, 0, md->d_b, out, c->d_partials, lsq_ctr(c, ctr), d_out, pub};
     const bool have_tanh = md->tanh_x == x;
-    md->tanh_x = nullptr;
+    md->tanh_x = md->pv_x = nullptr;
     if (!have_tanh) {
         md->sfac_x = nullptr;
         LSQ_LAUNCH(k_tanh, dim3(ngrid(c, J->n)), dim3(LSQ_NT), 0, c->stream, J->n, x, md->d_t);
@@ -306,17 +324,19 @@
         md->perm_of[k] = fcur;
     }
     md->perm_of[1 - k] = ftrial;
-    md->tanh_x = nullptr;
+    const double *pv = md->pv_x == xt ? md->d_pv : nullptr;
+    md->tanh_x = md->pv_x = nullptr;
     const int grid = std::max(1, std::min(S.nblocks, c->num_cus));
     const bool spec = sg && sg->gate && md->sfac_x == xt;
     SellPairEpi e{skip, md->d_perm[k], md->d_b_perm, ftrial, md->d_perm[1 - k], c->d_partials, c->d_partials + 4096, lsq_ctr(c, 7),
                   slot_pred, slot_trial, pub, spec ? sg->gate : nullptr, spec ? sg->ssr : 0.0, MIN_STEP_QUALITY,
                   c->d_slots + SL_SSR, c->d_slots + SL_DX, c->d_slots + SL_GRAD, spec ? sg->xtol : 0.0, spec ? sg->ftol : 0.0,
                   spec ? sg->gtol : 0.0};
-    LSQ_LAUNCH(k_sell_rows_pair<0>, dim3(grid), dim3(LSQ_BIG_NT), lds, c->stream, sell_dev(S), S.wrows, J->m, dx, J->d_colscale,
-               (const double *)md->d_t, J->n, nxpad, e);
+    LSQ_LAUNCH(k_sell_rows_pair<0>, dim3(grid), dim3(LSQ_BIG_NT), lds, c->stream, sell_dev(S), S.wrows, J->m, pv, dx, J->d_colscale,
+               (const double *)md->d_t, J->n, e);
     *done = true;
     ++md->pair_tails;
+    if (pv) ++md->pv_tails;
     if (hipGetLastError() != hipSuccess) return 1;
     if (spec) {
         const int st = lsq_sparse_grad_colsum_spec(J, ftrial, sg->grad, md->d_sspec, sg->gate);
@@ -333,7 +353,7 @@
     else if (md->sfac_x == x) std::swap(md->d_s, md->d_sspec);
     else LSQ_LAUNCH(k_sfac, dim3(ngrid(c, J->n)), dim3(LSQ_NT), 0, c->stream, J->n, x, md->d_s);
     md->sfac_x = nullptr;
-    md->tanh_x = nullptr;
+    md->tanh_x = md->pv_x = nullptr;
     if (md->fused) {
         if (lsq_mat_set_colscale(J, md->d_s) != LSQ_OK) return 1;
         return hipGetLastError() == hipSuccess ? 0 : 1;
@@ -462,12 +482,21 @@
     return LSQ_OK;
 }
 
+extern "C" int lsq_model_pair_vector_tails(const lsq_model *md, long long *out) {
+    if (!md || !out) {
+        lsq_set_error("lsq_model_pair_vector_tails: null argument");
+        return LSQ_EARG;
+    }
+    *out = md->pv_tails;
+    return LSQ_OK;
+}
+
 extern "C" int lsq_model_destroy(lsq_model *md) {
     if (!md) return LSQ_OK;
     hipStreamSynchronize(md->ctx->stream);
     if (md->fused && md->J) lsq_mat_set_colscale(md->J, nullptr);
     hipFree(md->d_Acsc); hipFree(md->d_Acsr); hipFree(md->d_Ab); hipFree(md->d_b); hipFree(md->d_t); hipFree(md->d_s); hipFree(md->d_sspec);
-    hipFree(md->d_b_perm); hipFree(md->d_perm[0]); hipFree(md->d_perm[1]);
+    hipFree(md->d_b_perm); hipFree(md->d_perm[0]); hipFree(md->d_perm[1]); hipFree(md->d_pv);
     delete md;
     return LSQ_OK;
 }
diff --git a/leastsquaresoptim.jl_amd/csrc/lsq_optimize.hip b/leastsquaresoptim.jl_amd/csrc/lsq_optimize.hip
--- a/leastsquaresoptim.jl_amd/csrc/lsq_optimize.hip
+++ b/leastsquaresoptim.jl_amd/csrc/lsq_optimize.hip
@@ -149,18 +149,26 @@
 __global__ void __launch_bounds__(LSQ_NT)
 k_step(int n, const double *__restrict__ x, const double *__restrict__ dx, double *__restrict__ xt,
        double *partials, unsigned *counters, double *out_dx, double *out_nonfin, double *__restrict__ t_out,
-       double *__restrict__ s_out, const int *skip = nullptr) {
+       double *__restrict__ s_out, const int *skip = nullptr, double *__restrict__ pv = nullptr,
+       const double *__restrict__ pscale = nullptr) {
     __shared__ double sh[LSQ_NT / 64];
     if (skip && *skip) return;
     double mx = 0.0, code = 0.0;
     for (int i = blockIdx.x * LSQ_NT + threadIdx.x; i < n; i += gridDim.x * LSQ_NT) {
         double d = dx[i];
+        const double sc = pv ? pscale[i] : 0.0;
         double v = x[i] + -1.0 * d;
         xt[i] = v;
         if (t_out) {
             const double th = tanh(v);
             t_out[i] = th;
             s_out[i] = 1.0 - th * th;
+            if (pv) {
+                double2 ab;
+                ab.x = d * sc;
+                ab.y = th;
+                reinterpret_cast<double2 *>(pv)[i] = ab;
+            }
         }
         double a = fabs(d);
         if (isnan(a)) a = INFINITY;
@@ -517,10 +525,11 @@
 
 static int launch_step(lsq_ctx *c, bool model, void *user, int gn, int n, const double *x, const double *dx, double *xt,
                        const int *skip = nullptr) {
-    double *t_out = nullptr, *s_out = nullptr;
-    if (model) model_trial_buffers(user, xt, &t_out, &s_out);
+    double *t_out = nullptr, *s_out = nullptr, *pv = nullptr;
+    const double *pscale = nullptr;
+    if (model) model_trial_buffers(user, xt, &t_out, &s_out, &pv, &pscale);
     LSQ_LAUNCH(k_step, dim3(gn), dim3(LSQ_NT), 0, c->stream, n, x, dx, xt, c->d_partials, lsq_ctr(c, 5), c->d_slots + SL_DX,
-               c->d_slots + SL_NONFIN, t_out, s_out, skip);
+               c->d_slots + SL_NONFIN, t_out, s_out, skip, pv, pscale);
     LSQ_HIP(hipGetLastError());
     return LSQ_OK;
 }
@@ -738,7 +747,7 @@
             LsmrTail tail{guardable ? last_inner : 0, lm_tail, &tc, guardable};
             LsmrStepDesc sd{x, xt, nullptr, nullptr, c->d_partials, lsq_ctr(c, 5), c->d_slots + SL_DX, c->d_slots + SL_NONFIN};
             if (tail_ok && guardable) {
-                if (is_model) model_trial_buffers(user, xt, &sd.t_out, &sd.s_out);
+                if (is_model) model_trial_buffers(user, xt, &sd.t_out, &sd.s_out, &sd.pv, &sd.pscale);
                 tail.step = &sd;
                 tail.step_taken = &tc.step_taken;
             }
diff --git a/leastsquaresoptim.jl_amd/csrc/lsq_sell.h b/leastsquaresoptim.jl_amd/csrc/lsq_sell.h
--- a/leastsquaresoptim.jl_amd/csrc/lsq_sell.h
+++ b/leastsquaresoptim.jl_amd/csrc/lsq_sell.h
@@ -406,12 +406,12 @@
 }
 
 template <int U, bool CLAMP>
-__device__ __forceinline__ void sell_batch_sum2(SellBatch<U> &B, int p0, int np, int len, const double *xa, const double *xb,
-                                                double &sa, double &sb) {
+__device__ __forceinline__ void sell_batch_sum2(SellBatch<U> &B, int p0, int np, int len, const double2 *xab, double &sa, double &sb) {
 #pragma unroll
     for (int u = 0; u < U; ++u) {
         const unsigned i0 = B.c[u] & 0xffffu, i1 = B.c[u] >> 16;
-        double a0 = B.a[u].x * xa[i0], a1 = B.a[u].y * xa[i1], b0 = B.a[u].x * xb[i0], b1 = B.a[u].y * xb[i1];
+        const double2 x0 = xab[i0], x1 = xab[i1];
+        double a0 = B.a[u].x * x0.x, a1 = B.a[u].y * x1.x, b0 = B.a[u].x * x0.y, b1 = B.a[u].y * x1.y;
         asm volatile("" : "+v"(a0), "+v"(a1), "+v"(b0), "+v"(b1));
         const int j = 2 * (p0 + u);
         const bool pin = !CLAMP || p0 + u < np;
@@ -427,7 +427,7 @@
     }
 }
 __device__ __forceinline__ void sell_lane_sum2(const double *__restrict__ vp, const unsigned short *__restrict__ ip, int L, int len,
-                                               const double *xa, const double *xb, double &sa, double &sb, int lane) {
+                                               const double2 *xab, double &sa, double &sb, int lane) {
     const int np = L >> 1;
     int p0 = 0;
     SellTail tail;
@@ -437,24 +437,25 @@
     for (; p0 + 8 <= np; p0 += 8) {
         SellBatch<8> B;
         sell_batch_load<8, false>(B, vp, ip, p0, np);
-        sell_batch_sum2<8, false>(B, p0, np, len, xa, xb, sa, sb);
+        sell_batch_sum2<8, false>(B, p0, np, len, xab, sa, sb);
     }
     const int rem = np - p0;
     if (rem > 4) {
         SellBatch<8> B;
         sell_batch_load<8, true>(B, vp, ip, p0, np);
-        sell_batch_sum2<8, true>(B, p0, np, len, xa, xb, sa, sb);
+        sell_batch_sum2<8, true>(B, p0, np, len, xab, sa, sb);
     } else if (rem > 2) {
         SellBatch<4> B;
         sell_batch_load<4, true>(B, vp, ip, p0, np);
-        sell_batch_sum2<4, true>(B, p0, np, len, xa, xb, sa, sb);
+        sell_batch_sum2<4, true>(B, p0, np, len, xab, sa, sb);
     } else if (rem > 0) {
         SellBatch<2> B;
         sell_batch_load<2, true>(B, vp, ip, p0, np);
-        sell_batch_sum2<2, true>(B, p0, np, len, xa, xb, sa, sb);
+        sell_batch_sum2<2, true>(B, p0, np, len, xab, sa, sb);
     }
     if (L & 1) {
-        double pa = tail.a * xa[tail.c], pb = tail.a * xb[tail.c];
+        const double2 xt = xab[tail.c];
+        double pa = tail.a * xt.x, pb = tail.a * xt.y;
         asm volatile("" : "+v"(pa), "+v"(pb));
         const bool in = L - 1 < len;
         const double ta = sa + pa, tb = sb + pb;
@@ -489,17 +490,13 @@
         dst[i] = pos != LSQ_SELL_POS_MASK ? src[(size_t)w * wrows + pos] : 0.0;
     }
 }
-template <int = 0>
-__global__ void __launch_bounds__(LSQ_BIG_NT) k_sell_rows_pair(SellDev S, int wrows, int m, const double *__restrict__ xa,
-                                                               const double *__restrict__ sa_scale, const double *__restrict__ xb,
-                                                               int nx, int nxpad, SellPairEpi e) {
-    extern __shared__ __attribute__((aligned(16))) double smem[];
-    __shared__ double sh[LSQ_BIG_NT / 64];
-    double *la = smem, *lb = smem + nxpad;
-    constexpr int NW = LSQ_BIG_NT / 64;
-    const int tid = threadIdx.x, lane = tid & 63, wv = tid >> 6;
-    constexpr int XR = (LSQ_PAIR_X_MAX + LSQ_BIG_NT - 1) / LSQ_BIG_NT;
-    {
+template <int XR>
+__device__ __forceinline__ void sell_pair_stage(const double *__restrict__ pv, const double *__restrict__ xa,
+                                                const double *__restrict__ sa_scale, const double *__restrict__ xb, int nx,
+                                                double *lds, int tid) {
+    if (pv) {
+        sell_stage_dma<XR>(pv, lds, 2 * nx, tid);
+    } else {
         double ra[XR], rs[XR], rb[XR];
 #pragma unroll
         for (int q = 0; q < XR; ++q) {
@@ -508,30 +505,82 @@
             rs[q] = sa_scale ? sa_scale[i] : 1.0;
             rb[q] = xb[i];
         }
-        const int dflag = e.done ? *e.done : 0;
 #pragma unroll
         for (int q = 0; q < XR; ++q)
             if (tid + q * LSQ_BIG_NT < nx) {
-                la[tid + q * LSQ_BIG_NT] = ra[q] * rs[q];
-                lb[tid + q * LSQ_BIG_NT] = rb[q];
-            }
-        if (dflag) return;
-    }
+                double2 ab;
+                ab.x = ra[q] * rs[q];
+                ab.y = rb[q];
+                reinterpret_cast<double2 *>(lds)[tid + q * LSQ_BIG_NT] = ab;
+            }
+        sell_stage_wait();
+    }
+}
+__device__ __forceinline__ void sell_pair_restage(const double *__restrict__ pv, const double *__restrict__ xa,
+                                                  const double *__restrict__ sa_scale, const double *__restrict__ xb, int nx,
+                                                  double *lds, int tid) {
+    typedef const __attribute__((address_space(1))) void *gptr_t;
+    typedef __attribute__((address_space(3))) void *lptr_t;
+#pragma unroll 1
+    for (int i = tid; i < nx; i += LSQ_BIG_NT) {
+        if (pv) {
+            __builtin_amdgcn_global_load_lds((gptr_t)(pv + 2 * i), (lptr_t)(lds + 2 * i), 16, 0, 0);
+        } else {
+            double2 ab;
+            ab.x = xa[i] * (sa_scale ? sa_scale[i] : 1.0);
+            ab.y = xb[i];
+            reinterpret_cast<double2 *>(lds)[i] = ab;
+        }
+    }
+}
+template <int = 0>
+__global__ void __launch_bounds__(LSQ_BIG_NT) k_sell_rows_pair(SellDev S, int wrows, int m, const double *__restrict__ pv,
+                                                               const double *__restrict__ xa, const double *__restrict__ sa_scale,
+                                                               const double *__restrict__ xb, int nx, SellPairEpi e) {
+    extern __shared__ __attribute__((aligned(16))) double smem[];
+    __shared__ double sh[LSQ_BIG_NT / 64];
+    const double2 *lab = reinterpret_cast<const double2 *>(smem);
+    constexpr int NW = LSQ_BIG_NT / 64;
+    const int tid = threadIdx.x, lane = tid & 63, wv = tid >> 6;
+    constexpr int XR = (LSQ_PAIR_X_MAX + LSQ_BIG_NT - 1) / LSQ_BIG_NT;
+    static_assert(XR * LSQ_BIG_NT >= LSQ_PAIR_X_MAX, "one pair per chunk");
+    int dflag = 0;
+    double h_dx = 0.0, h_gr = 0.0;
     constexpr int G = LSQ_SELL_ROWS_MAX / 64 / NW;
     double acc_a = 0.0, acc_b = 0.0;
+    if ((int)blockIdx.x >= S.nblocks) return;
+    const SellSliceRef ref0 = sell_slice_ref(S, (int)blockIdx.x * S.spw + wv, ((int)blockIdx.x + 1) * S.spw, lane);
+    sell_pair_stage<XR>(pv, xa, sa_scale, xb, nx, smem, tid);
+    dflag = e.done ? *e.done : 0;
+    if (e.gate) {
+        h_dx = *e.slot_dx;
+        h_gr = *e.slot_gr;
+    }
     for (int w = blockIdx.x; w < S.nblocks; w += gridDim.x) {
         const int base = w * wrows, rows = min(wrows, m - base);
         const int s0 = w * S.spw, s1 = s0 + S.spw;
-        if (w != (int)blockIdx.x) {
+        const bool first = w == (int)blockIdx.x;
+        int s = s0 + wv;
+        SellSliceRef A;
+        A.sm = make_int2(0, 0);
+        A.inf = LSQ_SELL_POS_MASK;
+        if (!first) {
             __syncthreads();
-            for (int i = tid; i < nx; i += LSQ_BIG_NT) {
-                la[i] = xa[i] * (sa_scale ? sa_scale[i] : 1.0);
-                lb[i] = xb[i];
-            }
-        }
-        int s = s0 + wv;
-        SellSliceRef A = sell_slice_ref(S, s, s1, lane);
+            A = sell_slice_ref(S, s, s1, lane);
+            sell_pair_restage(pv, xa, sa_scale, xb, nx, smem, tid);
+        }
+        sell_stage_wait();
         __syncthreads();
+        if (first) {
+            int stop = dflag;
+            asm volatile("" : "+v"(stop));
+            if (stop) return;
+            int2 sm0 = ref0.sm;
+            unsigned inf0 = ref0.inf;
+            asm volatile("" : "+v"(sm0.x), "+v"(sm0.y), "+v"(inf0));
+            A.sm = sm0;
+            A.inf = inf0;
+        }
         double keep[G];
         unsigned kpos[G];
 #pragma unroll
@@ -547,7 +596,7 @@
                 const double fa = e.fa[pidx], fb = e.fb[pidx];
                 const size_t oa = (size_t)a.sm.x + lane * 2;
                 double sum_a = 0.0, sum_b = 0.0;
-                sell_lane_sum2(S.val + oa, S.idx16 + oa, a.sm.y, (int)(a.inf >> LSQ_SELL_POS_BITS), la, lb, sum_a, sum_b, lane);
+                sell_lane_sum2(S.val + oa, S.idx16 + oa, a.sm.y, (int)(a.inf >> LSQ_SELL_POS_BITS), lab, sum_a, sum_b, lane);
                 if (valid) {
                     const double r_a = sum_a - fa, r_b = sum_b - fb;
                     e.out_b_perm[pidx] = r_b;
@@ -565,16 +614,12 @@
             if (kpos[g] != LSQ_SELL_POS_MASK) smem[kpos[g]] = keep[g];
         __syncthreads();
         for (int i = tid; i < rows; i += LSQ_BIG_NT) e.out_b[base + i] = smem[i];
+        sell_stage_wait();
     }
     const double ba = block_sum<LSQ_BIG_NT>(acc_a, sh);
     const double bb = block_sum<LSQ_BIG_NT>(acc_b, sh);
-    if (tid == 0) __hip_atomic_store(&e.part_b[blockIdx.x], bb, RLX_AGENT);
-    double total_a = 0.0;
-    const bool last = grid_reduce<LSQ_BIG_NT>(ba, e.part_a, e.counter, gridDim.x, sh, [&](double t) { total_a = t; });
-    if (!last) return;
-    double pb = 0.0;
-    for (int i = tid; i < (int)gridDim.x; i += LSQ_BIG_NT) pb += __hip_atomic_load(&e.part_b[i], RLX_AGENT);
-    const double total_b = block_sum<LSQ_BIG_NT>(pb, sh);
+    double total_a = 0.0, total_b = 0.0;
+    if (!grid_reduce2<LSQ_BIG_NT>(ba, bb, e.part_a, e.part_b, e.counter, gridDim.x, sh, total_a, total_b)) return;
     if (tid == 0) {
         *e.slot_a = total_a;
         *e.slot_b = total_b;
@@ -582,8 +627,7 @@
             const double pred_red = fabs(e.ssr - total_a);
             const double rho = pred_red > 0 ? (e.ssr - total_b) / pred_red : 0.0;
             const bool acc = rho > e.min_quality;
-            const bool conv = (acc && fabs(total_b - e.ssr) <= e.ftol * (fabs(e.ssr) + e.ftol)) || *e.slot_dx <= e.xtol ||
-                              *e.slot_gr <= e.gtol;
+            const bool conv = (acc && fabs(total_b - e.ssr) <= e.ftol * (fabs(e.ssr) + e.ftol)) || h_dx <= e.xtol || h_gr <= e.gtol;
             const bool go = acc && !conv;
             *e.gate = go ? 0 : 1;
             *e.slot_gate = go ? 1.0 : 0.0;
diff --git a/leastsquaresoptim.jl_amd/csrc/lsq_solver.h b/leastsquaresoptim.jl_amd/csrc/lsq_solver.h
--- a/leastsquaresoptim.jl_amd/csrc/lsq_solver.h
+++ b/leastsquaresoptim.jl_amd/csrc/lsq_solver.h
@@ -174,6 +174,8 @@
     double *partials = nullptr;
     unsigned *counter = nullptr;
     double *out_dx = nullptr, *out_nonfin = nullptr;
+    double *pv = nullptr;
+    const double *pscale = nullptr;
 };
 struct LsmrTail {
     int predict = 0;
diff --git a/leastsquaresoptim.jl_amd/synthetic.py b/leastsquaresoptim.jl_amd/synthetic.py
--- a/leastsquaresoptim.jl_amd/synthetic.py
+++ b/leastsquaresoptim.jl_amd/synthetic.py
@@ -139,7 +139,7 @@
 
     def optimize(self, optimizer_kind, solver_kind, x_tol=1e-8, f_tol=1e-8, g_tol=1e-8, iterations=1000,
                  delta=None, trace=False, allreduce=None, fetch_x=True, row_allreduce=None, row_allreduce_user=None,
-                 global_rows=0):
+                 global_rows=0, lower=None, upper=None):
         if self._Jd is None:
             L = lib()
             self._Jd = _Handle(self.J)
@@ -147,7 +147,7 @@
         Jd = self._Jd
         st, res, tr = _run_native(self.ctx, optimizer_kind, solver_kind, Jd, self.x, self.fcur,
                                   self._fg[0], self._fg[1], self.model, x_tol, f_tol, g_tol,
-                                  iterations, delta, None, None, trace, self.n, allreduce=allreduce,
+                                  iterations, delta, lower, upper, trace, self.n, allreduce=allreduce,
                                   row_allreduce=row_allreduce, row_allreduce_user=row_allreduce_user, global_rows=global_rows)
         check(st)
         r = LeastSquaresResult()
@@ -179,9 +179,10 @@
         return r
 
     def paths(self):
-        rows, cols, lpath, pairs = C.c_int(), C.c_int(), C.c_int(), C.c_longlong()
+        rows, cols, lpath, pairs, pvs = C.c_int(), C.c_int(), C.c_int(), C.c_longlong(), C.c_longlong()
         check(lib().lsq_model_paths(self.model, C.byref(rows), C.byref(cols), C.byref(lpath), C.byref(pairs)))
-        return dict(sliced_rows=bool(rows.value), sliced_cols=bool(cols.value), pair_tails=pairs.value,
+        check(lib().lsq_model_pair_vector_tails(self.model, C.byref(pvs)))
+        return dict(sliced_rows=bool(rows.value), sliced_cols=bool(cols.value), pair_tails=pairs.value, pair_vector_tails=pvs.value,
                     lsmr_path={0: None, 1: "reference-order", 2: "four-launch", 3: "three-launch", 4: "general"}[lpath.value])
 
     def close(self):
```

Result: no change. 4344, median of 6 (+1.0%).
